# j-min/HiREST

Hardware: AMD Instinct MI355X
Metric: encoded frames/sec (EVA-CLIP-g/14 224^2) (higher is better)
Workload: dtype bf16

## Files before the change

hirest_amd/_lib.py:

```python
from __future__ import annotations

import ctypes as C
import os

HERE = os.path.dirname(os.path.abspath(__file__))
LIB_PATH = os.path.join(HERE, "lib", "libhirest_hip.so")
if os.environ.get("HIREST_LIB_VARIANT"):
    LIB_PATH = os.path.join(HERE, "lib", f"libhirest_hip.{os.environ['HIREST_LIB_VARIANT']}.so")

(EPI_BIAS_BF16, EPI_BIAS_GELU_BF16, EPI_BIAS_QGELU_BF16, EPI_BIAS_RESID_F32, EPI_BIAS_F32, EPI_PATCH_POS_F32,
 EPI_BIAS_RESID_LNSTATS_F32, EPI_LNFOLD_BF16, EPI_LNFOLD_GELU_BF16, EPI_BIAS_GELU_SPLIT2, EPI_BIAS_RESID2_LNSTATS) = range(11)

TOWER_NO_LNFOLD = 1
TOWER_NO_PRUNE = 2
TOWER_F32_RESIDUAL = 4
GEMM_REVERSE = 1
GEMM_X3 = 2
GEMM_X3_T128 = 4
ABI_VERSION = 4

ERRORS = {-1: "HIREST_E_BADARG", -2: "HIREST_E_SHAPE (unsupported shape)", -3: "HIREST_E_WORKSPACE (workspace too small)"}


class GemmArgs(C.Structure):
    _fields_ = [("struct_size", C.c_uint64),
                ("A", C.c_void_p), ("lda", C.c_int64), ("W", C.c_void_p), ("ldw", C.c_int64),
                ("bias", C.c_void_p), ("out", C.c_void_p), ("ldo", C.c_int64),
                ("M", C.c_int32), ("N", C.c_int32), ("K", C.c_int32), ("epilogue", C.c_int32),
                ("pos", C.c_void_p), ("patches_per_frame", C.c_int32), ("aux0", C.c_void_p), ("aux1", C.c_void_p), ("flags", C.c_int32)]

    @classmethod
    def make(cls, *fields):
        return cls(C.sizeof(cls), *fields)


F32_ENTRY = {"gemm": 0, "ws": 1, "layouts": 2, "ln": 3, "ln_colmax": 4, "rows_colmax": 5}


class GemmF32Query(C.Structure):
    _fields_ = [("struct_size", C.c_uint32)] + \
               [(n, C.c_int32) for n in ("entry", "M", "N", "K", "has_resid", "has_periodic", "has_ids", "has_ln_out", "has_workspace",
                                         "a_kmajor", "w_kmajor", "select_kernel", "ring_mode", "rows_ln_mode", "cus")]

    @classmethod
    def make(cls, entry, M, N, K, **fields):
        q = cls(C.sizeof(cls), F32_ENTRY[entry], M, N, K, select_kernel=-1, ring_mode=-1, rows_ln_mode=-1)
        for k, v in fields.items():
            setattr(q, k, int(v))
        return q


class BlockWeights(C.Structure):
    _fields_ = [(n, C.c_void_p) for n in ("ln1_g", "ln1_b", "qkv_w", "qkv_b", "proj_w", "proj_b",
                                          "ln2_g", "ln2_b", "fc1_w", "fc1_b", "fc2_w", "fc2_b",
                                          "qkv_wf", "qkv_bf", "qkv_s", "fc1_wf", "fc1_bf", "fc1_s")]


class VisionTower(C.Structure):
    _fields_ = [(n, C.c_int32) for n in ("image_size", "patch", "width", "heads", "head_dim", "mlp_dim",
                                         "layers", "embed_dim", "kpad", "act")] + \
               [("ln_eps", C.c_float)] + \
               [("patch_w", C.c_void_p), ("patch_b", C.c_void_p), ("cls", C.c_void_p), ("pos", C.c_void_p),
                ("blocks", C.POINTER(BlockWeights)),
                ("norm_g", C.c_void_p), ("norm_b", C.c_void_p), ("head_w", C.c_void_p), ("head_b", C.c_void_p),
                ("image_mean", C.c_void_p), ("image_std", C.c_void_p),
                ("ln_pre_g", C.c_void_p), ("ln_pre_b", C.c_void_p), ("out_all_tokens", C.c_int32)]


class TextTower(C.Structure):
    _fields_ = [(n, C.c_int32) for n in ("context", "vocab", "width", "heads", "layers", "embed_dim", "act")] + \
               [("ln_eps", C.c_float)] + \
               [("tok_emb", C.c_void_p), ("pos", C.c_void_p), ("blocks", C.POINTER(BlockWeights)),
                ("lnf_g", C.c_void_p), ("lnf_b", C.c_void_p), ("proj_w", C.c_void_p)]


class BlockWeightsF32(C.Structure):
    _fields_ = [(n, C.c_void_p) for n in ("ln1_g", "ln1_b", "qkv_w", "qkv_b", "proj_w", "proj_b",
                                          "ln2_g", "ln2_b", "fc1_w", "fc1_b", "fc2_w", "fc2_b")]


class VisionTowerF32(C.Structure):
    _fields_ = [(n, t) if n != "blocks" else (n, C.POINTER(BlockWeightsF32)) for n, t in VisionTower._fields_]


class TextTowerF32(C.Structure):
    _fields_ = [(n, t) if n != "blocks" else (n, C.POINTER(BlockWeightsF32)) for n, t in TextTower._fields_]


class BlockWeightsX3(C.Structure):
    _fields_ = [(n, C.c_void_p) for n in ("qkv_w2", "proj_w2", "fc1_w2", "fc2_w2")]


class VisionTowerX3(C.Structure):
    _fields_ = [("base", C.POINTER(VisionTowerF32)), ("blocks", C.POINTER(BlockWeightsX3))]


class CaptionLayer(C.Structure):
    _fields_ = [(n, C.c_void_p) for n in ("qkv_w", "qkv_b", "so_w", "so_b", "so_ln_g", "so_ln_b", "cq_w", "cq_b",
                                          "co_w", "co_b", "co_ln_g", "co_ln_b", "ff1_w", "ff1_b", "ff2_w", "ff2_b", "ff_ln_g", "ff_ln_b")]


class CaptionDecoder(C.Structure):
    _fields_ = [(n, C.c_int32) for n in ("layers", "heads", "hidden", "inter", "vocab_padded", "max_pos")] + \
               [(n, C.c_void_p) for n in ("word_emb", "pos_emb", "emb_ln_g", "emb_ln_b")] + \
               [("layer", C.POINTER(CaptionLayer))] + \
               [(n, C.c_void_p) for n in ("tr_w", "tr_b", "tr_ln_g", "tr_ln_b", "lm_w", "lm_b", "lm_w2")]


class WhisperLayer(C.Structure):
    _fields_ = [(n, C.c_void_p) for n in ("attn_ln_g", "attn_ln_b", "qkv_w", "qkv_b", "so_w", "so_b", "cross_ln_g", "cross_ln_b", "cq_w", "cq_b",
                                          "co_w", "co_b", "mlp_ln_g", "mlp_ln_b", "fc1_w", "fc1_b", "fc2_w", "fc2_b")]


class WhisperDecoder(C.Structure):
    _fields_ = [(n, C.c_int32) for n in ("layers", "heads", "hidden", "inter", "vocab_padded", "max_pos")] + \
               [(n, C.c_void_p) for n in ("tok_emb", "pos_emb")] + [("layer", C.POINTER(WhisperLayer))] + \
               [(n, C.c_void_p) for n in ("ln_g", "ln_b", "lm_b")]


class WhisperTailParams(C.Structure):
    _fields_ = [(n, C.c_int32) for n in ("n_vocab", "eot", "no_speech", "no_timestamps", "timestamp_begin", "max_initial_timestamp_index",
                                         "sample_begin", "blank", "suppress_blank", "timestamp_rules", "monotonic")] + \
               [("temperature", C.c_float), ("seed", C.c_uint32), ("serial", C.c_uint32), ("suppress_mask", C.c_void_p)]


WHISPER_ROW_STATE_WORDS = 8


class JointLayerX3(C.Structure):
    _fields_ = [(n, C.c_void_p) for n in ("qkv_w2", "qkv_b", "ao_w2", "ao_b", "ln1_g", "ln1_b", "fc1_w2", "fc1_b", "fc2_w2", "fc2_b", "ln2_g", "ln2_b")]


class JointEncoderX3(C.Structure):
    _fields_ = [("struct_size", C.c_uint64)] + [(n, C.c_int32) for n in ("layers", "heads", "width", "mlp_dim", "in_dim", "max_pos")] + \
               [("ln_eps", C.c_float), ("attn_shift", C.c_float)] + \
               [(n, C.c_void_p) for n in ("emb_w2", "emb_b", "pos", "emb_ln_g", "emb_ln_b")] + [("layer", C.POINTER(JointLayerX3))]


class ColsumItem(C.Structure):
    _fields_ = [("x", C.c_void_p), ("row_weight", C.c_void_p), ("row_select", C.c_void_p), ("out", C.c_void_p), ("ldx", C.c_int64),
                ("R", C.c_int32), ("C", C.c_int32), ("select_value", C.c_int32), ("reserved", C.c_int32)]


COLSUM_GROUP_MAX = 40


class SplitItem(C.Structure):
    _fields_ = [("x", C.c_void_p), ("out", C.c_void_p), ("ldx", C.c_int64), ("ldo", C.c_int64), ("rows", C.c_int32), ("cols", C.c_int32),
                ("transposed", C.c_int32), ("reserved", C.c_int32)]


class OptimItem(C.Structure):
    _fields_ = [("p", C.c_void_p), ("g", C.c_void_p), ("m", C.c_void_p), ("v", C.c_void_p), ("n", C.c_int64)]


OPTIM_GROUP_MAX = 64
OPTIM_CHUNK = 8192


class TrainBlock(C.Structure):
    _fields_ = [("struct_size", C.c_uint64)] + [(n, C.c_int32) for n in ("B", "T", "heads", "width", "mlp", "precision")] + \
               [("ln_eps", C.c_float), ("drop", C.c_float)] + [(n, C.c_uint32) for n in ("seed_attn", "seed_ao", "seed_out", "reserved")] + \
               [(n, C.c_void_p) for n in ("wqkv", "bqkv", "wo", "bo", "ln1_g", "ln1_b", "w1", "b1", "w2", "b2", "ln2_g", "ln2_b", "x",
                                          "qkv", "P", "cx", "a_pre", "aa", "hpre", "hh", "x_pre", "out", "x2", "out2",
                                          "wqkv2", "wo2", "w12", "w22", "wqkvT2", "woT2", "w1T2", "w2T2", "ws")] + [("ws_bytes", C.c_size_t)]


class TrainFusionBwd(C.Structure):
    _fields_ = [("struct_size", C.c_uint64)] + \
               [(n, C.c_int32) for n in ("B", "T", "E", "W", "vis_dim", "text_dim", "asr_dim", "boundary", "max_pos", "reserved")] + \
               [("drop", C.c_float), ("seed_emb", C.c_uint32)] + \
               [(n, C.c_void_p) for n in ("w_emb", "emb_ln_g", "t2_w", "asr1_w", "asr0_g", "norm_g",
                                          "x0", "f", "v", "tn", "tin", "a0", "asr2", "v0", "vis2", "t", "text", "mm32", "bm32", "n_valid", "dx",
                                          "g_emb_ln_g", "g_emb_ln_b", "g_pos", "g_w_emb", "g_b_emb", "g_mask", "g_bound", "g_t2_w", "g_t2_b", "g_t0_w", "g_t0_b",
                                          "g_asr1_w", "g_asr1_b", "g_asr0_g", "g_asr0_b", "g_norm_g", "g_norm_b", "g_vis_w", "g_vis_b", "g_text_w", "g_text_b")] + \
               [("items", C.POINTER(ColsumItem)), ("n_items", C.POINTER(C.c_int32)), ("max_items", C.c_int32), ("reserved2", C.c_int32),
                ("ws", C.c_void_p), ("ws_bytes", C.c_size_t), ("side_stream", C.c_void_p), ("side_ws", C.c_void_p), ("side_ws_bytes", C.c_size_t),
                ("scratch", C.c_void_p), ("scratch_bytes", C.c_size_t)]


class TrainBlockGrads(C.Structure):
    _fields_ = [("struct_size", C.c_uint64)] + \
               [(n, C.c_void_p) for n in ("dout", "dx", "g_wqkv", "g_wo", "g_w1", "g_w2", "g_bqkv", "g_bo", "g_b1", "g_b2", "g_ln1_g", "g_ln1_b",
                                          "g_ln2_g", "g_ln2_b")] + \
               [("items", C.POINTER(ColsumItem)), ("n_items", C.POINTER(C.c_int32)), ("max_items", C.c_int32), ("reserved", C.c_int32),
                ("side_stream", C.c_void_p), ("side_ws", C.c_void_p), ("side_ws_bytes", C.c_size_t), ("scratch", C.c_void_p),
                ("scratch_bytes", C.c_size_t)]


class JpegImage(C.Structure):
    _fields_ = [(n, C.c_int32) for n in ("width", "height", "ncomp", "hs", "vs", "restart_interval", "mcux", "mcuy", "supported",
                                         "reason")] + \
               [("scan_begin", C.c_int64), ("scan_end", C.c_int64), ("table_set", C.c_int32), ("reserved", C.c_int32),
                ("data_offset", C.c_int64), ("out_offset", C.c_int64), ("ws_offset", C.c_int64),
                ("plane_offset", C.c_int64)]


class JpegTables(C.Structure):
    _fields_ = [("qt", (C.c_uint16 * 64) * 3), ("huff_bits", (C.c_uint8 * 16) * 6), ("huff_vals", (C.c_uint8 * 256) * 6)]


JPEG_REASONS = {0: "ok", 1: "not a JPEG / malformed markers", 2: "progressive", 3: "arithmetic coding", 4: "lossless / hierarchical",
                5: "not 8-bit", 6: "colour space (CMYK / YCCK / RGB / component count)", 7: "sampling factors", 8: "multi-scan",
                9: "truncated (no EOI after the scan)", 10: "bad or missing tables", 11: "image size"}
JPEG_STATUS = {1: "bad Huffman code", 2: "more than 64 coefficients in a block", 4: "out of data", 8: "RSTn out of sequence",
               16: "unsupported"}


BATCH_GATHER_MAX = 8


class BatchGather(C.Structure):
    _fields_ = [("src", C.c_void_p), ("dst", C.c_void_p), ("row_of_example", C.c_void_p), ("words", C.c_int32), ("reserved", C.c_int32)]


class BatchArgs(C.Structure):
    _fields_ = [("struct_size", C.c_uint64), ("index", C.c_void_p)] + \
               [(n, C.c_int32) for n in ("B", "T", "D", "Da", "n_examples", "n_model_frames", "n_gather", "reserved")] + \
               [(n, C.c_void_p) for n in ("frames", "frame_off", "asr_rows", "sub_off", "sub_span", "ex_video", "ex_len", "ex_range",
                                          "bound_off", "bound_val", "vis", "asr", "vis_mask", "moment_mask", "prev_boundary_mask")] + \
               [("gather", BatchGather * BATCH_GATHER_MAX)]


class ProfRecord(C.Structure):
    _fields_ = [("kind", C.c_int32), ("tag", C.c_int32), ("d0", C.c_int64), ("d1", C.c_int64), ("d2", C.c_int64),
                ("ms", C.c_float)]


_SIGNATURES = {
    "hirest_profile_enable": (C.c_int, [C.c_int32]),
    "hirest_attention_debug_mode": (C.c_int, [C.c_int32]),
    "hirest_profile_collect": (C.c_int, [C.POINTER(ProfRecord), C.c_int32]),
    "hirest_abi_version": (C.c_int, []),
    "hirest_build_info": (C.c_char_p, []),
    "hirest_gemm_bf16": (C.c_int, [C.POINTER(GemmArgs), C.c_void_p]),
    "hirest_gemm_select_kernel": (C.c_int, [C.c_int32]),
    "hirest_gemm_debug_mode": (C.c_int, [C.c_int32]),
    "hirest_gemm_dispatch_name": (C.c_int, [C.POINTER(GemmArgs), C.c_char_p, C.c_int32]),
    "hirest_attention_select_kernel": (C.c_int, [C.c_int32]),
    "hirest_attention_set_skew": (C.c_int, [C.c_int32]),
    "hirest_attention_set_mapping": (C.c_int, [C.c_int32]),
    "hirest_attention_set_pace": (C.c_int, [C.c_int32]),
    "hirest_attention_x3_select_waves": (C.c_int, [C.c_int32]),
    "hirest_attention_x3_debug_trace": (C.c_int, [C.c_void_p]),
    "hirest_attention_set_stagger": (C.c_int, [C.c_int32]),
    "hirest_attention_debug_trace_read": (C.c_int, [C.c_void_p, C.c_int32]),
    "hirest_layernorm": (C.c_int, [C.c_void_p, C.c_int64, C.c_void_p, C.c_void_p, C.c_void_p, C.c_float,
                                   C.c_void_p, C.c_int64, C.c_int32, C.c_int32, C.c_int32, C.c_void_p]),
    "hirest_attention_bf16": (C.c_int, [C.c_void_p, C.c_void_p, C.c_int32, C.c_int32, C.c_int32, C.c_int32,
                                        C.c_float, C.c_int32, C.c_void_p]),
    "hirest_attention_bf16_rows": (C.c_int, [C.c_void_p, C.c_void_p, C.c_int32, C.c_int32, C.c_int32, C.c_int32,
                                             C.c_float, C.c_int32, C.c_int32, C.c_void_p]),
    "hirest_fold_layernorm": (C.c_int, [C.c_void_p, C.c_void_p, C.c_void_p, C.c_void_p, C.c_void_p, C.c_void_p, C.c_void_p, C.c_int32,
                                        C.c_int32, C.c_void_p]),
    "hirest_patchify": (C.c_int, [C.c_void_p, C.c_int32, C.c_int32, C.c_int32, C.c_int32, C.c_void_p, C.c_void_p,
                                  C.c_void_p, C.c_int32, C.c_void_p]),
    "hirest_rowstats_bf16": (C.c_int, [C.c_void_p, C.c_int64, C.c_void_p, C.c_void_p, C.c_float, C.c_int32, C.c_int32, C.c_void_p, C.c_void_p]),
    "hirest_rowstats_split_bf16": (C.c_int, [C.c_void_p, C.c_int64, C.c_void_p, C.c_void_p, C.c_void_p, C.c_float, C.c_int32, C.c_int32, C.c_void_p,
                                             C.c_void_p]),
    "hirest_combine_hi_lo_f32": (C.c_int, [C.c_void_p, C.c_void_p, C.c_int64, C.c_void_p, C.c_int64, C.c_int32, C.c_int32, C.c_void_p]),
    "hirest_ln_stats_finalize": (C.c_int, [C.c_void_p, C.c_int32, C.c_void_p, C.c_float, C.c_int32, C.c_int32, C.c_void_p, C.c_void_p]),
    "hirest_write_cls_rows": (C.c_int, [C.c_void_p, C.c_int64, C.c_void_p, C.c_void_p, C.c_int32, C.c_int32,
                                        C.c_int32, C.c_void_p]),
    "hirest_embed_tokens": (C.c_int, [C.c_void_p, C.c_void_p, C.c_void_p, C.c_void_p, C.c_void_p, C.c_int32,
                                      C.c_int32, C.c_int32, C.c_int32, C.c_void_p]),
    "hirest_f32_to_bf16": (C.c_int, [C.c_void_p, C.c_void_p, C.c_int64, C.c_void_p]),
    "hirest_pool_l2norm": (C.c_int, [C.c_void_p, C.c_void_p, C.c_int32, C.c_int32, C.c_int32, C.c_int32, C.c_void_p]),
    "hirest_pool_l2norm_varlen": (C.c_int, [C.c_void_p, C.c_void_p, C.c_void_p, C.c_int32, C.c_int32, C.c_void_p]),
    "hirest_similarity_f32": (C.c_int, [C.c_void_p, C.c_void_p, C.c_void_p, C.c_int32, C.c_int32, C.c_int32, C.c_void_p]),
    "hirest_topk_workspace_bytes": (C.c_int64, [C.c_int32, C.c_int32, C.c_int32]),
    "hirest_topk_f32_ws": (C.c_int, [C.c_void_p, C.c_void_p, C.c_int32, C.c_int32, C.c_int32, C.c_void_p, C.c_void_p, C.c_void_p,
                                     C.c_int64, C.c_void_p]),
    "hirest_topk_f32": (C.c_int, [C.c_void_p, C.c_void_p, C.c_int32, C.c_int32, C.c_int32, C.c_void_p, C.c_void_p,
                                  C.c_void_p]),
    "hirest_clip_score": (C.c_int, [C.c_void_p, C.c_int32, C.c_int32, C.c_void_p, C.c_int32, C.c_void_p, C.c_int32, C.c_int32,
                                    C.c_int32, C.c_void_p, C.c_void_p]),
    "hirest_bertscore_greedy": (C.c_int, [C.c_void_p, C.c_int64, C.c_int32, C.c_void_p, C.c_int32, C.c_void_p, C.c_void_p, C.c_void_p,
                                          C.c_int32, C.c_void_p, C.c_void_p]),
    "hirest_gemm_f32": (C.c_int, [C.c_void_p, C.c_int64, C.c_void_p, C.c_int64, C.c_void_p, C.c_void_p, C.c_int64, C.c_void_p,
                                  C.c_int32, C.c_void_p, C.c_int64, C.c_int32, C.c_int32, C.c_int32, C.c_int32, C.c_void_p]),
    "hirest_attention_f32": (C.c_int, [C.c_void_p, C.c_void_p, C.c_int32, C.c_int32, C.c_int32, C.c_int32, C.c_float,
                                       C.c_float, C.c_void_p]),
    "hirest_attention_f32_qkv": (C.c_int, [C.c_void_p, C.c_int64, C.c_void_p, C.c_void_p, C.c_int64, C.c_void_p, C.c_int32, C.c_int32,
                                           C.c_int32, C.c_int32, C.c_int32, C.c_float, C.c_float, C.c_float, C.c_void_p]),
    "hirest_gemm_f32_select_kernel": (C.c_int, [C.c_int32]),
    "hirest_gemm_f32_workspace_bytes": (C.c_size_t, [C.c_int32, C.c_int32, C.c_int32]),
    "hirest_gemm_f32_layouts_workspace_bytes": (C.c_size_t, [C.c_int32, C.c_int32, C.c_int32]),
    "hirest_gemm_f32_layouts": (C.c_int, [C.c_void_p, C.c_int64, C.c_int32, C.c_void_p, C.c_int64, C.c_int32, C.c_void_p, C.c_void_p, C.c_int64,
                                          C.c_void_p, C.c_int64, C.c_int32, C.c_int32, C.c_int32, C.c_int32, C.c_void_p, C.c_size_t, C.c_void_p]),
    "hirest_gemm_f32_ws": (C.c_int, [C.c_void_p, C.c_int64, C.c_void_p, C.c_int64, C.c_void_p, C.c_void_p, C.c_int64, C.c_void_p,
                                     C.c_int32, C.c_void_p, C.c_int64, C.c_int32, C.c_int32, C.c_int32, C.c_int32, C.c_void_p, C.c_size_t,
                                     C.c_void_p]),
    "hirest_attention_f32_decode": (C.c_int, [C.c_void_p, C.c_int64, C.c_void_p, C.c_void_p, C.c_int64, C.c_void_p, C.c_int32, C.c_void_p,
                                              C.c_void_p, C.c_int64, C.c_void_p, C.c_void_p, C.c_void_p, C.c_int32, C.c_int32, C.c_float,
                                              C.c_float, C.c_float, C.c_void_p]),
    "hirest_gemm_f32_ln": (C.c_int, [C.c_void_p, C.c_int64, C.c_void_p, C.c_void_p, C.c_void_p, C.c_void_p, C.c_void_p, C.c_float,
                                     C.c_void_p, C.c_int64, C.c_void_p, C.c_int64, C.c_void_p, C.c_void_p, C.c_int64, C.c_void_p,
                                     C.c_int64, C.c_int32, C.c_int32, C.c_int32, C.c_int32, C.c_void_p]),
    "hirest_caption_step_workspace_bytes": (C.c_size_t, [C.POINTER(CaptionDecoder), C.c_int32]),
    "hirest_beam_backtrack": (C.c_int, [C.c_void_p, C.c_void_p, C.c_void_p, C.c_void_p, C.c_int32, C.c_int32, C.c_int32, C.c_void_p, C.c_void_p]),
    "hirest_beam_advance": (C.c_int, [C.c_void_p, C.c_void_p, C.c_int32, C.c_int32, C.c_int32, C.c_int32, C.c_int32, C.c_int32,
                                      C.c_void_p, C.c_void_p, C.c_void_p, C.c_void_p, C.c_void_p, C.c_void_p, C.c_void_p, C.c_void_p,
                                      C.c_void_p]),
    "hirest_caption_decode_step": (C.c_int, [C.POINTER(CaptionDecoder), C.c_int32, C.c_int32, C.c_void_p, C.c_void_p,
                                             C.POINTER(C.c_void_p), C.POINTER(C.c_void_p), C.POINTER(C.c_void_p), C.c_int32,
                                             C.c_void_p, C.c_void_p, C.c_void_p, C.c_size_t, C.c_void_p]),
    "hirest_caption_decode_logits": (C.c_int, [C.POINTER(CaptionDecoder), C.c_int32, C.c_int32, C.c_void_p, C.c_void_p,
                                               C.POINTER(C.c_void_p), C.POINTER(C.c_void_p), C.POINTER(C.c_void_p), C.c_int32,
                                               C.c_void_p, C.c_void_p, C.c_size_t, C.c_void_p]),
    "hirest_caption_select": (C.c_int, [C.c_int32]),
    "hirest_gemm_f32_ln_colmax": (C.c_int, [C.c_void_p, C.c_int64, C.c_void_p, C.c_void_p, C.c_float, C.c_void_p, C.c_int64, C.c_void_p,
                                            C.c_void_p, C.c_int64, C.c_void_p, C.c_int32, C.c_int32, C.c_int32, C.c_void_p]),
    "hirest_gemm_f32_dispatch_name": (C.c_int, [C.POINTER(GemmF32Query), C.c_char_p, C.c_int32]),
    "hirest_gemm_f32_rows_ln_mode": (C.c_int, [C.c_int32]),
    "hirest_gemm_f32_ring_mode": (C.c_int, [C.c_int32]),
    "hirest_gemm_f32_rows_preferred": (C.c_int, [C.c_int32]),
    "hirest_gemm_f32_rows_colmax": (C.c_int, [C.c_void_p, C.c_int64, C.c_void_p, C.c_int64, C.c_void_p, C.c_void_p, C.c_int64, C.c_void_p,
                                              C.c_int32, C.c_int32, C.c_int32, C.c_void_p]),
    "hirest_caption_beam_step": (C.c_int, [C.POINTER(CaptionDecoder), C.c_int32, C.c_int32, C.c_int32, C.c_void_p, C.c_void_p,
                                           C.POINTER(C.c_void_p), C.POINTER(C.c_void_p), C.POINTER(C.c_void_p), C.c_int32, C.c_void_p,
                                           C.c_void_p, C.c_int32, C.c_int32, C.c_void_p, C.c_void_p, C.c_void_p, C.c_void_p, C.c_void_p,
                                           C.c_void_p, C.c_void_p, C.c_size_t, C.c_void_p, C.c_size_t, C.c_void_p]),
    "hirest_caption_beam_tail_workspace_bytes": (C.c_size_t, [C.c_int32, C.c_int32, C.c_int32]),
    "hirest_caption_beam_tail": (C.c_int, [C.c_void_p, C.c_int64, C.c_void_p, C.c_int32, C.c_int32, C.c_int32, C.c_int32, C.c_int32,
                                           C.c_int32, C.c_void_p, C.c_void_p, C.c_void_p, C.c_void_p, C.c_void_p, C.c_void_p,
                                           C.c_void_p, C.c_void_p, C.c_void_p, C.c_void_p, C.c_size_t, C.c_void_p]),
    "hirest_attention_f32_varlen": (C.c_int, [C.c_void_p, C.c_void_p, C.c_void_p, C.c_int32, C.c_int32, C.c_int32, C.c_int32, C.c_float,
                                              C.c_float, C.c_void_p]),
    "hirest_log_softmax_f32": (C.c_int, [C.c_void_p, C.c_int64, C.c_void_p, C.c_void_p, C.c_int64, C.c_int32, C.c_int32, C.c_void_p]),
    "hirest_joint_time_grid_f32": (C.c_int, [C.c_void_p, C.c_int32, C.c_int32, C.c_void_p, C.c_void_p]),
    "hirest_joint_time_features": (C.c_int, [C.c_void_p, C.c_void_p, C.c_void_p, C.c_void_p, C.c_int32, C.c_int32, C.c_int32,
                                             C.c_void_p]),
    "hirest_joint_base": (C.c_int, [C.c_void_p, C.c_void_p, C.c_void_p, C.c_void_p, C.c_void_p, C.c_int32, C.c_int32, C.c_int32,
                                    C.c_void_p]),
    "hirest_joint_mask_add": (C.c_int, [C.c_void_p, C.c_void_p, C.c_void_p, C.c_void_p, C.c_void_p, C.c_void_p, C.c_int64,
                                        C.c_int32, C.c_void_p]),
    "hirest_transpose_pad_f32": (C.c_int, [C.c_void_p, C.c_int64, C.c_int32, C.c_int32, C.c_void_p, C.c_int32, C.c_void_p]),
    "hirest_weighted_colsum_grouped_f32": (C.c_int, [C.c_void_p, C.c_int32, C.c_void_p]),
    "hirest_train_fusion_backward_scratch_bytes": (C.c_size_t, [C.POINTER(TrainFusionBwd)]),
    "hirest_train_fusion_backward": (C.c_int, [C.POINTER(TrainFusionBwd), C.c_void_p]),
    "hirest_train_block_forward_scratch_bytes": (C.c_size_t, [C.POINTER(TrainBlock)]),
    "hirest_train_block_forward": (C.c_int, [C.POINTER(TrainBlock), C.c_void_p, C.c_size_t, C.c_void_p]),
    "hirest_train_block_backward_scratch_bytes": (C.c_size_t, [C.POINTER(TrainBlock)]),
    "hirest_train_block_backward": (C.c_int, [C.POINTER(TrainBlock), C.POINTER(TrainBlockGrads), C.c_void_p]),
    "hirest_optim_partials_count": (C.c_int64, [C.c_void_p, C.c_int32]),
    "hirest_grad_sqnorm_grouped_f32": (C.c_int, [C.c_void_p, C.c_int32, C.c_void_p, C.c_void_p]),
    "hirest_clip_coef_f32": (C.c_int, [C.c_void_p, C.c_int64, C.c_float, C.c_void_p, C.c_void_p]),
    "hirest_adamw_grouped_f32": (C.c_int, [C.c_void_p, C.c_int32, C.c_void_p, C.c_float, C.c_float, C.c_float, C.c_float, C.c_float,
                                           C.c_float, C.c_float, C.c_void_p]),
    "hirest_grad_sqnorm_scaled_grouped_f32": (C.c_int, [C.c_void_p, C.c_int32, C.c_void_p, C.c_void_p, C.c_void_p]),
    "hirest_clip_coef_dev_f32": (C.c_int, [C.c_void_p, C.c_int64, C.c_void_p, C.c_void_p, C.c_void_p]),
    "hirest_optim_step_advance_f32": (C.c_int, [C.c_void_p, C.c_int32, C.c_void_p, C.c_void_p]),
    "hirest_adamw_capturable_grouped_f32": (C.c_int, [C.c_void_p, C.c_void_p, C.c_int32, C.c_void_p, C.c_void_p, C.c_double, C.c_void_p,
                                                      C.c_void_p, C.c_double, C.c_double, C.c_float, C.c_double, C.c_void_p]),
    "hirest_weighted_colsum_f32": (C.c_int, [C.c_void_p, C.c_int64, C.c_void_p, C.c_void_p, C.c_int32, C.c_int32, C.c_int32, C.c_void_p, C.c_void_p]),
    "hirest_scale_by_device_scalar_f32": (C.c_int, [C.c_void_p, C.c_void_p, C.c_int64, C.c_void_p]),
    "hirest_act_f32": (C.c_int, [C.c_void_p, C.c_void_p, C.c_int64, C.c_int32, C.c_void_p]),
    "hirest_act_bwd_f32": (C.c_int, [C.c_void_p, C.c_void_p, C.c_void_p, C.c_int64, C.c_int32, C.c_void_p]),
    "hirest_dropout_add_f32": (C.c_int, [C.c_void_p, C.c_void_p, C.c_void_p, C.c_int64, C.c_float, C.c_uint32, C.c_void_p]),
    "hirest_layernorm_bwd_f32": (C.c_int, [C.c_void_p, C.c_void_p, C.c_void_p, C.c_float, C.c_void_p, C.c_void_p, C.c_int32, C.c_int32, C.c_void_p]),
    "hirest_attention_train_select": (C.c_int, [C.c_int32]),
    "hirest_gemm_f32_strided": (C.c_int, [C.c_void_p, C.c_int64, C.c_int64, C.c_void_p, C.c_int64, C.c_int64, C.c_void_p, C.c_int64,
                                          C.c_int32, C.c_int32, C.c_int32, C.c_float, C.c_void_p]),
    "hirest_attention_train_fwd_f32": (C.c_int, [C.c_void_p, C.c_void_p, C.c_void_p, C.c_int32, C.c_int32, C.c_int32, C.c_int32, C.c_float,
                                                 C.c_float, C.c_float, C.c_uint32, C.c_void_p]),
    "hirest_attention_train_bwd_f32": (C.c_int, [C.c_void_p, C.c_void_p, C.c_void_p, C.c_void_p, C.c_void_p, C.c_int32, C.c_int32, C.c_int32,
                                                 C.c_int32, C.c_float, C.c_float, C.c_uint32, C.c_void_p]),
    "hirest_attention_train_fwd_qkv_f32": (C.c_int, [C.c_void_p, C.c_int64, C.c_void_p, C.c_void_p, C.c_int64, C.c_void_p, C.c_void_p, C.c_void_p,
                                                     C.c_int64, C.c_int32, C.c_int32, C.c_int32, C.c_int32, C.c_int32, C.c_float, C.c_float,
                                                     C.c_float, C.c_uint32, C.c_void_p]),
    "hirest_attention_train_bwd_qkv_f32": (C.c_int, [C.c_void_p, C.c_int64, C.c_void_p, C.c_void_p, C.c_int64, C.c_void_p, C.c_void_p, C.c_int64,
                                                     C.c_void_p, C.c_void_p, C.c_int64, C.c_void_p, C.c_void_p, C.c_int64, C.c_int32, C.c_int32,
                                                     C.c_int32, C.c_int32, C.c_int32, C.c_float, C.c_float, C.c_uint32, C.c_void_p]),
    "hirest_embedding_fwd_f32": (C.c_int, [C.c_void_p, C.c_void_p, C.c_void_p, C.c_void_p, C.c_int64, C.c_int32, C.c_int32, C.c_void_p]),
    "hirest_embedding_pos_fwd_f32": (C.c_int, [C.c_void_p, C.c_void_p, C.c_void_p, C.c_void_p, C.c_void_p, C.c_int64, C.c_int32, C.c_void_p]),
    "hirest_embedding_bwd_f32": (C.c_int, [C.c_void_p, C.c_void_p, C.c_void_p, C.c_int64, C.c_int32, C.c_void_p]),
    "hirest_ce_rows_f32": (C.c_int, [C.c_void_p, C.c_int64, C.c_void_p, C.c_int32, C.c_int32, C.c_float, C.c_int32, C.c_void_p, C.c_void_p, C.c_void_p]),
    "hirest_bce_masked_f32": (C.c_int, [C.c_void_p, C.c_void_p, C.c_void_p, C.c_int32, C.c_int32, C.c_float, C.c_void_p, C.c_void_p, C.c_void_p]),
    "hirest_joint_base_bwd_f32": (C.c_int, [C.c_void_p, C.c_void_p, C.c_void_p, C.c_void_p, C.c_void_p, C.c_int32, C.c_int32, C.c_int32, C.c_void_p]),
    "hirest_l2norm_bwd_f32": (C.c_int, [C.c_void_p, C.c_void_p, C.c_void_p, C.c_int32, C.c_int32, C.c_void_p]),
    "hirest_ce_masked_f32": (C.c_int, [C.c_void_p, C.c_void_p, C.c_void_p, C.c_int32, C.c_int32, C.c_float, C.c_void_p, C.c_void_p, C.c_void_p]),
    "hirest_heads_bwd_f32": (C.c_int, [C.c_void_p, C.c_int64, C.c_int32, C.c_int32, C.c_void_p, C.c_void_p, C.c_void_p, C.c_void_p, C.c_void_p]),
    "hirest_linear_heads": (C.c_int, [C.c_void_p, C.c_int64, C.c_int32, C.c_int32, C.c_void_p, C.c_void_p, C.c_void_p, C.c_void_p,
                                      C.c_void_p, C.c_void_p]),
    "hirest_masked_argmax": (C.c_int, [C.c_void_p, C.c_void_p, C.c_float, C.c_int32, C.c_int32, C.c_void_p, C.c_void_p]),
    "hirest_moment_valid_f32": (C.c_int, [C.c_void_p, C.c_void_p, C.c_void_p, C.c_void_p, C.c_void_p, C.c_int32, C.c_int32, C.c_float,
                                          C.c_void_p, C.c_void_p, C.c_void_p]),
    "hirest_lm_head_ce_workspace_bytes": (C.c_size_t, [C.c_int32, C.c_int32]),
    "hirest_lm_head_ce_f32": (C.c_int, [C.c_void_p, C.c_int64, C.c_void_p, C.c_int64, C.c_void_p, C.c_void_p, C.c_int32, C.c_int32,
                                        C.c_int32, C.c_int32, C.c_void_p, C.c_void_p, C.c_void_p, C.c_size_t, C.c_void_p]),
    "hirest_segmentation_step": (C.c_int, [C.c_void_p, C.c_void_p, C.c_void_p, C.c_int32, C.c_int32, C.c_double, C.c_void_p,
                                           C.c_void_p, C.c_int32, C.c_void_p, C.c_void_p]),
    "hirest_preprocess_plan_bytes": (C.c_int64, [C.c_int32, C.c_int32, C.c_int32]),
    "hirest_preprocess_plan": (C.c_int, [C.c_int32, C.c_int32, C.c_int32, C.c_void_p, C.c_int64]),
    "hirest_preprocess_workspace_bytes": (C.c_int64, [C.c_int32, C.c_int32, C.c_int32, C.c_int32]),
    "hirest_preprocess_u8": (C.c_int, [C.c_void_p, C.c_int32, C.c_int32, C.c_int32, C.c_int32, C.c_void_p, C.c_void_p,
                                       C.c_int32, C.c_void_p, C.c_void_p, C.c_void_p, C.c_int64, C.c_void_p]),
    "hirest_jpeg_parse": (C.c_int, [C.c_void_p, C.c_int64, C.POINTER(JpegImage), C.POINTER(JpegTables)]),
    "hirest_jpeg_workspace_bytes": (C.c_int64, [C.POINTER(JpegImage), C.c_int32]),
    "hirest_jpeg_decode": (C.c_int, [C.c_void_p, C.c_void_p, C.c_int32, C.c_void_p, C.c_void_p, C.c_void_p, C.c_void_p, C.c_void_p,
                                     C.c_int64, C.c_void_p]),
    "hirest_jpeg_decode_host": (C.c_int, [C.POINTER(JpegImage), C.POINTER(JpegTables), C.c_void_p, C.c_void_p, C.POINTER(C.c_int32)]),
    "hirest_jpeg_chunked_workspace_bytes": (C.c_int64, [C.c_int32]),
    "hirest_jpeg_decode_chunked": (C.c_int, [C.c_void_p, C.c_void_p, C.c_int32, C.c_void_p, C.c_void_p, C.c_void_p, C.c_void_p, C.c_void_p,
                                             C.c_int64, C.c_int64, C.c_void_p, C.c_int64, C.c_void_p]),
    "hirest_jpeg_decode_host_chunked": (C.c_int, [C.POINTER(JpegImage), C.POINTER(JpegTables), C.c_void_p, C.c_int64, C.c_void_p,
                                                  C.POINTER(C.c_int32), C.POINTER(C.c_int32)]),
    "hirest_interval_iou_f64": (C.c_int, [C.c_void_p, C.c_void_p, C.c_int64, C.c_void_p, C.c_void_p]),
    "hirest_step_bound_pr": (C.c_int, [C.c_void_p, C.c_void_p, C.c_void_p, C.c_void_p, C.c_int32, C.c_double, C.c_void_p,
                                       C.c_void_p, C.c_void_p, C.c_void_p]),
    "hirest_frame_to_timestamp": (C.c_int, [C.c_void_p, C.c_void_p, C.c_void_p, C.c_int32, C.c_int64, C.c_int64, C.c_void_p, C.c_void_p]),
    "hirest_timestamp_to_frame": (C.c_int, [C.c_void_p, C.c_void_p, C.c_void_p, C.c_int32, C.c_int64, C.c_int64, C.c_void_p, C.c_void_p]),
    "hirest_preprocess_moment_bounds": (C.c_int, [C.c_void_p, C.c_void_p, C.c_void_p, C.c_int32, C.c_void_p, C.c_void_p,
                                                  C.c_int32, C.c_void_p]),
    "hirest_cascade_moment_bounds": (C.c_int, [C.c_void_p, C.c_void_p, C.c_void_p, C.c_int32, C.c_int32, C.c_int32, C.c_void_p, C.c_void_p,
                                               C.c_void_p, C.c_void_p, C.c_void_p]),
    "hirest_cascade_boundaries": (C.c_int, [C.c_void_p, C.c_void_p, C.c_void_p, C.c_void_p, C.c_void_p, C.c_int32, C.c_int32, C.c_int32,
                                            C.c_void_p, C.c_void_p, C.c_void_p, C.c_void_p, C.c_void_p, C.c_void_p, C.c_void_p]),
    "hirest_cascade_trim_gather": (C.c_int, [C.c_void_p, C.c_void_p, C.c_void_p, C.c_void_p, C.c_int32, C.c_int32, C.c_int32, C.c_int32,
                                             C.c_int32, C.c_int32, C.c_void_p, C.c_void_p, C.c_void_p]),
    "hirest_batch_assemble": (C.c_int, [C.POINTER(BatchArgs), C.c_void_p]),
    "hirest_log_mel_workspace_bytes": (C.c_size_t, [C.c_int64, C.c_int64]),
    "hirest_log_mel": (C.c_int, [C.c_void_p, C.c_int64, C.c_int64, C.c_void_p, C.c_int32, C.c_void_p, C.c_void_p, C.c_void_p, C.c_size_t,
                                 C.c_void_p]),
    "hirest_mel_to_rows": (C.c_int, [C.c_void_p, C.c_void_p, C.c_int32, C.c_int32, C.c_int32, C.c_void_p]),
    "hirest_attention_f32_decode_inplace": (C.c_int, [C.c_void_p, C.c_int64, C.c_void_p, C.c_void_p, C.c_int64, C.c_int64, C.c_int32, C.c_int32,
                                                      C.c_void_p, C.c_void_p, C.c_int64, C.c_void_p, C.c_int32, C.c_int32, C.c_float, C.c_float,
                                                      C.c_float, C.c_void_p]),
    "hirest_attention_f32_cross_decode_workspace_bytes": (C.c_size_t, [C.c_int32, C.c_int32, C.c_int32]),
    "hirest_attention_f32_cross_decode": (C.c_int, [C.c_void_p, C.c_int64, C.c_void_p, C.c_int64, C.c_int64, C.c_int32, C.c_int32, C.c_void_p,
                                                    C.c_void_p, C.c_int64, C.c_int32, C.c_int32, C.c_float, C.c_void_p, C.c_size_t, C.c_void_p]),
    "hirest_whisper_step_tail": (C.c_int, [C.c_void_p, C.c_int64, C.c_int32, C.c_int32, C.c_int32, C.c_int32, C.POINTER(WhisperTailParams),
                                           C.c_void_p, C.c_void_p, C.c_void_p, C.c_void_p, C.c_void_p, C.c_void_p]),
    "hirest_whisper_gumbel_bits": (C.c_int, [C.c_uint32, C.c_uint32, C.c_int32, C.c_int32, C.c_void_p, C.c_void_p]),
    "hirest_whisper_step_workspace_bytes": (C.c_size_t, [C.POINTER(WhisperDecoder), C.c_int32, C.c_int32]),
    "hirest_whisper_decode_step": (C.c_int, [C.POINTER(WhisperDecoder), C.c_int32, C.c_int32, C.c_void_p, C.POINTER(C.c_void_p),
                                             C.POINTER(C.c_void_p), C.c_int32, C.POINTER(C.c_void_p), C.c_int32, C.c_int32, C.c_void_p,
                                             C.c_void_p, C.c_void_p, C.c_size_t, C.c_void_p]),
    "hirest_vision_workspace_bytes": (C.c_size_t, [C.POINTER(VisionTower), C.c_int32]),
    "hirest_vision_forward": (C.c_int, [C.POINTER(VisionTower), C.c_void_p, C.c_int32, C.c_int32, C.c_void_p,
                                        C.c_void_p, C.c_size_t, C.c_int32, C.c_void_p]),
    "hirest_vision_guard_offset": (C.c_size_t, [C.POINTER(VisionTower), C.c_int32]),
    "hirest_vision_workspace_bytes_f32": (C.c_size_t, [C.POINTER(VisionTowerF32), C.c_int32]),
    "hirest_vision_embed_f32": (C.c_int, [C.POINTER(VisionTowerF32), C.c_void_p, C.c_int32, C.c_int32, C.c_void_p, C.c_void_p, C.c_void_p]),
    "hirest_joint_encoder_x3_workspace_bytes": (C.c_size_t, [C.POINTER(JointEncoderX3), C.c_int32, C.c_int32]),
    "hirest_joint_encoder_x3_forward": (C.c_int, [C.POINTER(JointEncoderX3), C.c_void_p, C.c_int32, C.c_int32, C.c_void_p, C.c_void_p, C.c_size_t,
                                                  C.c_void_p]),
    "hirest_layernorm_f32_split2": (C.c_int, [C.c_void_p, C.c_int64, C.c_void_p, C.c_int32, C.c_void_p, C.c_void_p, C.c_float, C.c_void_p, C.c_int64,
                                              C.c_void_p, C.c_int64, C.c_int32, C.c_int32, C.c_void_p]),
    "hirest_split2_bf16": (C.c_int, [C.c_void_p, C.c_int64, C.c_void_p, C.c_int64, C.c_int64, C.c_int32, C.c_int32, C.c_void_p]),
    "hirest_split2_grouped_bf16": (C.c_int, [C.c_void_p, C.c_int32, C.c_void_p]),
    "hirest_split2_transposed_bf16": (C.c_int, [C.c_void_p, C.c_int64, C.c_void_p, C.c_int64, C.c_int32, C.c_int32, C.c_void_p]),
    "hirest_layernorm_split2": (C.c_int, [C.c_void_p, C.c_int64, C.c_void_p, C.c_void_p, C.c_float, C.c_void_p, C.c_int64, C.c_int32,
                                          C.c_int32, C.c_void_p]),
    "hirest_attention_x3_qkv": (C.c_int, [C.c_void_p, C.c_int64, C.c_void_p, C.c_void_p, C.c_int64, C.c_void_p, C.c_int32, C.c_int32, C.c_int32,
                                          C.c_int32, C.c_int32, C.c_float, C.c_void_p]),
    "hirest_attention_x3_qkv_split2": (C.c_int, [C.c_void_p, C.c_int64, C.c_void_p, C.c_void_p, C.c_int64, C.c_void_p, C.c_int32, C.c_int32,
                                                 C.c_int32, C.c_int32, C.c_int32, C.c_float, C.c_void_p]),
    "hirest_vision_x3_select_attention": (C.c_int, [C.c_int32]),
    "hirest_vision_workspace_bytes_x3": (C.c_size_t, [C.POINTER(VisionTowerX3), C.c_int32]),
    "hirest_vision_forward_x3": (C.c_int, [C.POINTER(VisionTowerX3), C.c_void_p, C.c_int32, C.c_int32, C.c_void_p, C.c_void_p, C.c_size_t,
                                           C.c_void_p]),
    "hirest_vision_forward_f32": (C.c_int, [C.POINTER(VisionTowerF32), C.c_void_p, C.c_int32, C.c_int32, C.c_void_p,
                                            C.c_void_p, C.c_size_t, C.c_void_p]),
    "hirest_text_workspace_bytes_f32": (C.c_size_t, [C.POINTER(TextTowerF32), C.c_int32]),
    "hirest_text_forward_f32": (C.c_int, [C.POINTER(TextTowerF32), C.c_void_p, C.c_int32, C.c_void_p, C.c_void_p,
                                          C.c_size_t, C.c_void_p]),
    "hirest_text_workspace_bytes": (C.c_size_t, [C.POINTER(TextTower), C.c_int32]),
    "hirest_text_forward": (C.c_int, [C.POINTER(TextTower), C.c_void_p, C.c_int32, C.c_void_p, C.c_void_p,
                                      C.c_size_t, C.c_void_p]),
}

EXPORTS = tuple(_SIGNATURES)
_lib = None


def load():
    global _lib
    if _lib is not None:
        return _lib
    if not os.path.isfile(LIB_PATH):
        raise RuntimeError(f"{LIB_PATH} is missing: build it with `python -m hirest_amd.build` "
                           "(hipcc --offload-arch=gfx950). There is no CPU fallback.")
    lib = C.CDLL(LIB_PATH)
    lib.hirest_abi_version.restype, lib.hirest_abi_version.argtypes = C.c_int, []
    if lib.hirest_abi_version() != ABI_VERSION:
        raise RuntimeError(f"libhirest_hip.so ABI version {lib.hirest_abi_version()} != binding {ABI_VERSION}: rebuild with "
                           "`python -m hirest_amd.build --force`")
    for name, (res, args) in _SIGNATURES.items():
        fn = getattr(lib, name)
        fn.restype, fn.argtypes = res, args
    if os.environ.get("HIREST_ATTENTION_KERNEL"):
        check(lib.hirest_attention_select_kernel(int(os.environ["HIREST_ATTENTION_KERNEL"])), "HIREST_ATTENTION_KERNEL")
    _lib = lib
    return lib


def check(code: int, what: str):
    if code == 0:
        return
    if code < 0:
        raise RuntimeError(f"{what}: {ERRORS.get(code, code)}")
    raise RuntimeError(f"{what}: HIP error {code}")
```

hirest_amd/csrc/attention.hip:

```cpp
#include "common.h"
#include <atomic>
#include "profile.h"

namespace {

template <int DH, int DP, int NT>
struct AttnCfg {
    static constexpr int NPAD = 16 * NT;
    static constexpr int KS = (NT + 1) / 2;
    static constexpr int KP = 32 * KS;
    static constexpr int KRS = DP * 2 + 16;
    static constexpr int VRS = KP * 2 + 16;
    static constexpr int LDS_BYTES = NPAD * KRS + DP * VRS;
};

template <int DH, int DP, int NT>
__global__ __launch_bounds__(512) void attention_kernel(const bf16_t* __restrict__ qkv, bf16_t* __restrict__ out,
                                                       int N, int H, float scale_log2e, int causal, int nq) {
    using C = AttnCfg<DH, DP, NT>;
    extern __shared__ __attribute__((aligned(16))) char smem[];
    char* Ks = smem;
    char* Vt = smem + C::NPAD * C::KRS;
    const int tid = threadIdx.x, lane = tid & 63, wave = tid >> 6;
    const int b = blockIdx.x / H, h = blockIdx.x - b * H;
    const int D = H * DH;
    const int64_t ld = 3 * (int64_t)D;
    const bf16_t* base = qkv + (int64_t)b * N * ld + h * DH;

    constexpr int KCH = DP / 8;
    for (int idx = tid; idx < C::NPAD * KCH; idx += 512) {
        const int key = idx / KCH, ch = idx - key * KCH;
        bf16x8 v = {0, 0, 0, 0, 0, 0, 0, 0};
        if (key < N && ch * 8 < DH) v = *reinterpret_cast<const bf16x8*>(base + (int64_t)key * ld + D + ch * 8);
        *reinterpret_cast<bf16x8*>(Ks + key * C::KRS + ch * 16) = v;
    }
    constexpr int VCH = DH / 8;
    for (int idx = tid; idx < C::KP * VCH; idx += 512) {
        const int ch = idx / C::KP, key = idx - ch * C::KP;
        bf16x8 v = {0, 0, 0, 0, 0, 0, 0, 0};
        if (key < N) v = *reinterpret_cast<const bf16x8*>(base + (int64_t)key * ld + 2 * D + ch * 8);
#pragma unroll
        for (int e = 0; e < 8; ++e) *reinterpret_cast<bf16_t*>(Vt + (ch * 8 + e) * C::VRS + key * 2) = v[e];
    }
    __syncthreads();

    const int g = lane >> 4, c16 = lane & 15;
    const int nqt = (nq + 15) >> 4;
    for (int qt = wave; qt < nqt; qt += 8) {
        const int q = qt * 16 + c16;
        const bool qvalid = q < N;
        bf16x8 qf[DP / 32];
#pragma unroll
        for (int kk = 0; kk < DP / 32; ++kk) {
            const int d = (kk * 4 + g) * 8;
            bf16x8 v = {0, 0, 0, 0, 0, 0, 0, 0};
            if (qvalid && d < DH) v = *reinterpret_cast<const bf16x8*>(base + (int64_t)q * ld + d);
            qf[kk] = v;
        }
        f32x4 st[NT];
#pragma unroll
        for (int t = 0; t < NT; ++t) {
            f32x4 acc = {0.f, 0.f, 0.f, 0.f};
#pragma unroll
            for (int kk = 0; kk < DP / 32; ++kk) {
                const bf16x8 kf = *reinterpret_cast<const bf16x8*>(Ks + (t * 16 + c16) * C::KRS + (kk * 4 + g) * 16);
                acc = __builtin_amdgcn_mfma_f32_16x16x32_bf16(kf, qf[kk], acc, 0, 0, 0);
            }
            st[t] = acc;
            if ((t & 1) == 1) __builtin_amdgcn_sched_barrier(0);
        }
        const int klimit = causal ? (q < N - 1 ? q : N - 1) : N - 1;
        float mx = -3.0e38f;
#pragma unroll
        for (int t = 0; t < NT; ++t)
#pragma unroll
            for (int i = 0; i < 4; ++i) {
                const int key = t * 16 + 4 * g + i;
                const float s = key <= klimit ? st[t][i] : -3.0e38f;
                st[t][i] = s;
                mx = fmaxf(mx, s);
            }
        mx = fmaxf(mx, __shfl_xor(mx, 16, 64));
        mx = fmaxf(mx, __shfl_xor(mx, 32, 64));
        float sum = 0.f;
#pragma unroll
        for (int t = 0; t < NT; ++t)
#pragma unroll
            for (int i = 0; i < 4; ++i) {
                const float pz = exp2f((st[t][i] - mx) * scale_log2e);
                st[t][i] = pz;
                sum += pz;
            }
        sum += __shfl_xor(sum, 16, 64);
        sum += __shfl_xor(sum, 32, 64);
        const float inv = 1.0f / sum;
        bf16x8 pf[C::KS];
#pragma unroll
        for (int s = 0; s < C::KS; ++s) {
#pragma unroll
            for (int i = 0; i < 4; ++i) {
                pf[s][i] = (bf16_t)st[2 * s][i];
                if (2 * s + 1 < NT) pf[s][4 + i] = (bf16_t)st[2 * s + 1][i];
                else pf[s][4 + i] = (bf16_t)0.f;
            }
        }
#pragma unroll 1
        for (int dt = 0; dt < DP / 16; ++dt) {
            f32x4 acc = {0.f, 0.f, 0.f, 0.f};
            const char* vrow = Vt + (dt * 16 + c16) * C::VRS + 8 * g;
#pragma unroll
            for (int s = 0; s < C::KS; ++s) {
                const bf16x4 lo = *reinterpret_cast<const bf16x4*>(vrow + s * 64);
                const bf16x4 hi = *reinterpret_cast<const bf16x4*>(vrow + s * 64 + 32);
                const bf16x8 vf = {lo[0], lo[1], lo[2], lo[3], hi[0], hi[1], hi[2], hi[3]};
                acc = __builtin_amdgcn_mfma_f32_16x16x32_bf16(vf, pf[s], acc, 0, 0, 0);
            }
            const int d = dt * 16 + 4 * g;
            if (q < nq && d < DH) {
                bf16x4 o;
#pragma unroll
                for (int i = 0; i < 4; ++i) o[i] = (bf16_t)(acc[i] * inv);
                *reinterpret_cast<bf16x4*>(out + ((int64_t)b * N + q) * D + h * DH + d) = o;
            }
        }
    }
}

template <int DH, int DP, int NT>
int launch(const bf16_t* qkv, bf16_t* out, int B, int N, int H, float scale, int causal, int nq, hipStream_t s) {
    using C = AttnCfg<DH, DP, NT>;
    static HirestDevCfg cfg;
    auto kern = attention_kernel<DH, DP, NT>;
    if (int e = hirest_configure(kern, C::LDS_BYTES, cfg)) return e;
    hipLaunchKernelGGL(kern, dim3(B * H), dim3(512), C::LDS_BYTES, s, qkv, out, N, H, scale * 1.44269504088896340736f, causal, nq);
    return hirest_launch_status();
}


template <int DH, int DP, int NT>
struct AttnCfg2 {
    static constexpr int NPAD = 16 * NT;
    static constexpr int KS = (NT + 1) / 2;
    static constexpr int KP = 32 * KS;
    static constexpr int RS = DP * 2;
    static constexpr int CPR = DP / 8;
    static constexpr int NK_INSTR = NPAD * CPR / 64;
    static constexpr int NV_INSTR = KP * CPR / 64;
    static constexpr int LDS_BYTES = (NPAD + KP) * RS;
};

__device__ __forceinline__ void wait_vm_le(int n) {
    switch (n) {
        case 0: asm volatile("s_waitcnt vmcnt(0)" ::: "memory"); break;
        case 1: asm volatile("s_waitcnt vmcnt(1)" ::: "memory"); break;
        case 2: asm volatile("s_waitcnt vmcnt(2)" ::: "memory"); break;
        case 3: asm volatile("s_waitcnt vmcnt(3)" ::: "memory"); break;
        case 4: asm volatile("s_waitcnt vmcnt(4)" ::: "memory"); break;
        case 5: asm volatile("s_waitcnt vmcnt(5)" ::: "memory"); break;
        case 6: asm volatile("s_waitcnt vmcnt(6)" ::: "memory"); break;
        case 7: asm volatile("s_waitcnt vmcnt(7)" ::: "memory"); break;
        default: asm volatile("s_waitcnt vmcnt(8)" ::: "memory"); break;
    }
}

template <int DH, int DP, int NT>
__global__ __launch_bounds__(512) void attention_kernel_v2(const bf16_t* __restrict__ qkv, bf16_t* __restrict__ out,
                                                          int N, int H, float scale_log2e, int causal, int nq) {
    using C = AttnCfg2<DH, DP, NT>;
    extern __shared__ __attribute__((aligned(16))) char smem[];
    char* Ks = smem;
    char* Vs = smem + C::NPAD * C::RS;
    const int tid = threadIdx.x, lane = tid & 63;
    const int wave = __builtin_amdgcn_readfirstlane(tid >> 6);
    const int b = blockIdx.x / H, h = blockIdx.x - b * H;
    const int D = H * DH;
    const int64_t ld = 3 * (int64_t)D;
    const bf16_t* base = qkv + (int64_t)b * N * ld + h * DH;

    int nv_mine = 0;
    for (int i = wave; i < C::NK_INSTR; i += 8) {
        const int ci = i * 64 + lane;
        int row = ci / C::CPR, c = ci - row * C::CPR;
        c = (c & ~3) | ((c & 3) ^ ((-(row >> 2)) & 3));
        row = row < N ? row : N - 1;
        c = c * 8 < DH ? c : DH / 8 - 1;
        glds16(base + (int64_t)row * ld + D + c * 8, Ks + i * 1024);
    }
    for (int i = wave; i < C::NV_INSTR; i += 8) {
        const int ci = i * 64 + lane;
        int row = ci / C::CPR, c = ci - row * C::CPR;
        row = row < N ? row : N - 1;
        c = c * 8 < DH ? c : DH / 8 - 1;
        glds16(base + (int64_t)row * ld + 2 * D + c * 8, Vs + i * 1024);
        ++nv_mine;
    }
    wait_vm_le(nv_mine);
    __builtin_amdgcn_s_barrier();

    const int g = lane >> 4, c16 = lane & 15;
    const int gk = g ^ ((-(c16 >> 2)) & 3);
    const int nqt = (nq + 15) >> 4;
    bool v_ready = false;
    for (int qt = wave; qt < nqt; qt += 8) {
        const int q = qt * 16 + c16;
        const bool qvalid = q < N;
        bf16x8 qf[DP / 32];
#pragma unroll
        for (int kk = 0; kk < DP / 32; ++kk) {
            const int d = (kk * 4 + g) * 8;
            bf16x8 v = {0, 0, 0, 0, 0, 0, 0, 0};
            if (qvalid && d < DH) v = *reinterpret_cast<const bf16x8*>(base + (int64_t)q * ld + d);
            qf[kk] = v;
        }
        f32x4 st[NT];
#pragma unroll
        for (int t = 0; t < NT; ++t) {
            f32x4 acc = {0.f, 0.f, 0.f, 0.f};
#pragma unroll
            for (int kk = 0; kk < DP / 32; ++kk) {
                const bf16x8 kf = *reinterpret_cast<const bf16x8*>(Ks + (t * 16 + c16) * C::RS + (kk * 4 + gk) * 16);
                acc = __builtin_amdgcn_mfma_f32_16x16x32_bf16(kf, qf[kk], acc, 0, 0, 0);
            }
            st[t] = acc;
            if ((t & 1) == 1) __builtin_amdgcn_sched_barrier(0);
        }
        const int klimit = causal ? (q < N - 1 ? q : N - 1) : N - 1;
        float mx = -3.0e38f;
#pragma unroll
        for (int t = 0; t < NT; ++t)
#pragma unroll
            for (int i = 0; i < 4; ++i) {
                const int key = t * 16 + 4 * g + i;
                const float sv = key <= klimit ? st[t][i] : -3.0e38f;
                st[t][i] = sv;
                mx = fmaxf(mx, sv);
            }
        mx = fmaxf(mx, __shfl_xor(mx, 16, 64));
        mx = fmaxf(mx, __shfl_xor(mx, 32, 64));
        float sum = 0.f;
#pragma unroll
        for (int t = 0; t < NT; ++t)
#pragma unroll
            for (int i = 0; i < 4; ++i) {
                const float pz = exp2f((st[t][i] - mx) * scale_log2e);
                st[t][i] = pz;
                sum += pz;
            }
        sum += __shfl_xor(sum, 16, 64);
        sum += __shfl_xor(sum, 32, 64);
        const float inv = 1.0f / sum;
        bf16x8 pf[C::KS];
#pragma unroll
        for (int s = 0; s < C::KS; ++s) {
#pragma unroll
            for (int i = 0; i < 4; ++i) {
                pf[s][i] = (bf16_t)st[2 * s][i];
                if (2 * s + 1 < NT) pf[s][4 + i] = (bf16_t)st[2 * s + 1][i];
                else pf[s][4 + i] = (bf16_t)0.f;
            }
        }
        if (!v_ready) {
            asm volatile("s_waitcnt vmcnt(0)" ::: "memory");
            __builtin_amdgcn_s_barrier();
            v_ready = true;
        }
        const char* vlane = Vs + (4 * g + (c16 >> 2)) * C::RS + (c16 & 3) * 8;
#pragma unroll 1
        for (int dt = 0; dt < DP / 16; ++dt) {
            f32x4 acc = {0.f, 0.f, 0.f, 0.f};
            const char* vrow = vlane + dt * 32;
#pragma unroll
            for (int s = 0; s < C::KS; ++s) {
                const bf16x4 lo = __builtin_amdgcn_ds_read_tr16_b64_v4bf16(
                    (__attribute__((address_space(3))) bf16x4*)(vrow + s * 32 * C::RS));
                const bf16x4 hi = __builtin_amdgcn_ds_read_tr16_b64_v4bf16(
                    (__attribute__((address_space(3))) bf16x4*)(vrow + (s * 32 + 16) * C::RS));
                const bf16x8 vf = {lo[0], lo[1], lo[2], lo[3], hi[0], hi[1], hi[2], hi[3]};
                acc = __builtin_amdgcn_mfma_f32_16x16x32_bf16(vf, pf[s], acc, 0, 0, 0);
            }
            const int d = dt * 16 + 4 * g;
            if (q < nq && d < DH) {
                bf16x4 o;
#pragma unroll
                for (int i = 0; i < 4; ++i) o[i] = (bf16_t)(acc[i] * inv);
                *reinterpret_cast<bf16x4*>(out + ((int64_t)b * N + q) * D + h * DH + d) = o;
            }
        }
    }
    if (!v_ready) {
        asm volatile("s_waitcnt vmcnt(0)" ::: "memory");
        __builtin_amdgcn_s_barrier();
    }
}


__device__ __forceinline__ void sleep_n(int n) {
    for (int i = 0; i < n; ++i) __builtin_amdgcn_s_sleep(1);
}
template <int NW, int CPR> struct ROWS_PER_PIECE_OK { static constexpr bool value = (NW * 64 % CPR == 0) && ((NW * 64 / CPR) % 8 == 0); };
__device__ __attribute__((aligned(16))) const unsigned short g_attn_ones[8] = {0x3F80, 0x3F80, 0x3F80, 0x3F80, 0x3F80, 0x3F80, 0x3F80, 0x3F80};
__device__ __attribute__((aligned(16))) const unsigned short g_attn_zeros[8] = {0, 0, 0, 0, 0, 0, 0, 0};
constexpr int ATTN_TRACE_STEPS = 64, ATTN_TRACE_WAVES = 12, ATTN_TRACE_SLOTS = 12;
__device__ long long g_attn_trace[ATTN_TRACE_STEPS * ATTN_TRACE_WAVES * ATTN_TRACE_SLOTS];
__device__ __forceinline__ float max3_raw(float a, float b, float c) {
    float r;
    asm("v_max3_f32 %0, %1, %2, %3" : "=v"(r) : "v"(a), "v"(b), "v"(c));
    return r;
}
typedef float f32x2_t __attribute__((ext_vector_type(2)));
template <int DH, int DP, int NT, bool FAST, bool DBG, int NW = 9, bool LEAN = false, bool PROD = false>
__global__ __launch_bounds__((NW + (PROD ? 1 : 0)) * 64) void attention_kernel_v3(const bf16_t* __restrict__ qkv, bf16_t* __restrict__ out,
                                                          int N, int H, float scale_log2e, int causal, int dbg_bits, int nq, int skew,
                                                          int B, int map, int pace, int stagger) {
    const int dbg = DBG ? dbg_bits : 0;
    using C = AttnCfg2<DH, DP, NT>;
    extern __shared__ __attribute__((aligned(16))) char smem[];
    char* Vs = smem + 2 * C::NPAD * C::RS;
    const int tid = threadIdx.x, lane = tid & 63;
    const int wave = __builtin_amdgcn_readfirstlane(tid >> 6);
    const int D = H * DH;
    const int64_t ld = 3 * (int64_t)D;
    int b0, bstep, h0, hstep, nsteps;
    if (map == 0) { b0 = blockIdx.x; bstep = 0; h0 = 0; hstep = 1; nsteps = H; }
    else {
        const int xcd = blockIdx.x & 7, slot = blockIdx.x >> 3, FL = (gridDim.x >> 3) / H;
        h0 = slot % H; hstep = 0; b0 = xcd * FL + slot / H; bstep = 8 * FL;
        nsteps = b0 < B ? (B - b0 + bstep - 1) / bstep : 0;
    }
    if (nsteps == 0) return;
    if (stagger > 0 && blockIdx.x < 256) sleep_n(((blockIdx.x >> 3) & 15) * stagger);
    auto sbase = [&](int st) { return qkv + (int64_t)(b0 + st * bstep) * N * ld + (h0 + st * hstep) * DH; };
    const int g = lane >> 4, c16 = lane & 15;
    const int gk = g ^ ((-(c16 >> 2)) & 3);
    const int nqt = (nq + 15) >> 4;

    const int ci0 = wave * 64 + lane;
    const int row0 = ci0 / C::CPR, col0 = ci0 - row0 * C::CPR;
    constexpr bool VSWAP = C::RS == 192;
    const int vlog = VSWAP ? ((((col0 >> 1) ^ ((row0 >> 2) & 1)) << 1) | (col0 & 1)) : col0;
    const int vc = vlog * 8 < DH ? vlog : DH / 8 - 1;
    static_assert(ROWS_PER_PIECE_OK<NW, C::CPR>::value, "a lane's rows must keep (row >> 2) & 1 from piece to piece");
    static_assert((NW * 64) % C::CPR == 0, "piece stride must be whole rows");
    constexpr int ROWS_PER_PIECE = NW * 64 / C::CPR;
    auto dma_k = [&](int h, char* dst) -> int {
        int n = 0;
        const bf16_t* src = sbase(h) + D;
        for (int i = wave, row = row0; i < C::NK_INSTR; i += NW, row += ROWS_PER_PIECE) {
            int kc = (col0 & ~3) | ((col0 & 3) ^ ((-(row >> 2)) & 3));
            const bool kpad = kc * 8 >= DH;
            kc = kpad ? DH / 8 - 1 : kc;
            const int r = row < N ? row : N - 1;
            const void* from = src + (int64_t)r * ld + kc * 8;
            if (LEAN && DP > DH) from = kpad ? (const void*)g_attn_zeros : from;
            glds16(from, dst + i * 1024);
            ++n;
        }
        return n;
    };
    constexpr bool SUM_IN_MFMA = LEAN && DP > DH;
    const bool vpad = SUM_IN_MFMA && vlog * 8 >= DH;
    auto dma_v = [&](int h) {
        const bf16_t* src = sbase(h) + 2 * D + vc * 8;
        for (int i = wave, row = row0; i < C::NV_INSTR; i += NW, row += ROWS_PER_PIECE) {
            const int r = row < N ? row : N - 1;
            const void* from = src + (int64_t)r * ld;
            if (SUM_IN_MFMA) from = vpad ? (const void*)g_attn_ones : from;
            glds16(from, Vs + i * 1024);
        }
    };
    auto load_q = [&](int h, int qtile, bf16x8 (&dst)[DP / 32]) {
        const int q = qtile * 16 + c16;
        const bf16_t* base = sbase(h);
        if (LEAN && DP > DH) {
            const bf16_t* row = base + (int64_t)(q < N ? q : N - 1) * ld;
#pragma unroll
            for (int kk = 0; kk < DP / 32; ++kk) {
                const int d = (kk * 4 + g) * 8;
                dst[kk] = *reinterpret_cast<const bf16x8*>(row + (d < DH ? d : DH - 8));
            }
            return;
        }
#pragma unroll
        for (int kk = 0; kk < DP / 32; ++kk) {
            const int d = (kk * 4 + g) * 8;
            bf16x8 v = {0, 0, 0, 0, 0, 0, 0, 0};
            if (qtile < nqt && q < N && d < DH) v = *reinterpret_cast<const bf16x8*>(base + (int64_t)q * ld + d);
            dst[kk] = v;
        }
    };

    if (PROD && wave == NW) {
        constexpr int PER = C::CPR / 4;
        static_assert(C::NK_INSTR % PER == 0 && C::NV_INSTR % PER == 0, "whole 16-row groups");
        int prow[PER], pkoff[PER], pvoff[PER];
        bool pkpad[PER], pvpad[PER];
#pragma unroll
        for (int j = 0; j < PER; ++j) {
            const int ci = j * 64 + lane, r = ci / C::CPR, c = ci - r * C::CPR;
            prow[j] = r;
            int kc = (c & ~3) | ((c & 3) ^ ((-(r >> 2)) & 3));
            pkpad[j] = kc * 8 >= DH;
            pkoff[j] = (pkpad[j] ? DH / 8 - 1 : kc) * 8;
            const int vl = VSWAP ? ((((c >> 1) ^ ((r >> 2) & 1)) << 1) | (c & 1)) : c;
            pvpad[j] = SUM_IN_MFMA && vl * 8 >= DH;
            pvoff[j] = (vl * 8 < DH ? vl : DH / 8 - 1) * 8;
        }
        auto issue_k = [&](int st, char* dst, int pace_units) {
            const bf16_t* src = sbase(st) + D;
            for (int it0 = 0; it0 < C::NK_INSTR / PER; ++it0) {
                const int it = map ? (it0 + h0) % (C::NK_INSTR / PER) : it0;
#pragma unroll
                for (int j = 0; j < PER; ++j) {
                    const int row = prow[j] + 16 * it, r = row < N ? row : N - 1;
                    const void* from = src + (int64_t)r * ld + pkoff[j];
                    if (LEAN && DP > DH) from = pkpad[j] ? (const void*)g_attn_zeros : from;
                    glds16(from, dst + (it * PER + j) * 1024);
                    if (pace_units > 0) sleep_n(pace_units);
                }
            }
        };
        auto issue_v = [&](int st) {
            const bf16_t* src = sbase(st) + 2 * D;
            for (int it0 = 0; it0 < C::NV_INSTR / PER; ++it0) {
                const int it = map ? (it0 + h0) % (C::NV_INSTR / PER) : it0;
#pragma unroll
                for (int j = 0; j < PER; ++j) {
                    const int row = prow[j] + 16 * it, r = row < N ? row : N - 1;
                    const void* from = src + (int64_t)r * ld + pvoff[j];
                    if (SUM_IN_MFMA) from = pvpad[j] ? (const void*)g_attn_ones : from;
                    glds16(from, Vs + (it * PER + j) * 1024);
                }
            }
        };
        issue_k(0, smem, 0);
        for (int h = 0; h < nsteps; ++h) {
            asm volatile("s_waitcnt vmcnt(0)" ::: "memory");
            __builtin_amdgcn_s_barrier();
            issue_v(h);
            asm volatile("s_waitcnt vmcnt(0)" ::: "memory");
            __builtin_amdgcn_s_barrier();
            if (h + 1 < nsteps) issue_k(h + 1, smem + ((h + 1) & 1) * (C::NPAD * C::RS), pace);
        }
        asm volatile("s_waitcnt vmcnt(0)" ::: "memory");
        return;
    }

    bf16x8 qa[DP / 32], qb[DP / 32];
    load_q(0, wave, qa);
    load_q(0, wave + NW, qb);
    if (!(dbg & 8) && !PROD) dma_k(0, smem);
    for (int h = 0; h < nsteps; ++h) {
        const char* Ks = smem + (h & 1) * (C::NPAD * C::RS);
        auto stamp = [&](int slot) {
            if (DBG && (dbg & 256) && blockIdx.x == 0 && h < ATTN_TRACE_STEPS) {
                const long long t = __builtin_readcyclecounter();
                if (lane == 0) g_attn_trace[(h * ATTN_TRACE_WAVES + wave) * ATTN_TRACE_SLOTS + slot] = t;
            }
        };
        stamp(10);
        asm volatile("s_waitcnt vmcnt(0)" ::: "memory");
#pragma unroll
        for (int kk = 0; kk < DP / 32; ++kk) { asm volatile("" : "+v"(qa[kk])); asm volatile("" : "+v"(qb[kk])); }
        if (!(dbg & 128)) __builtin_amdgcn_s_barrier();
        stamp(0);
        if (!(dbg & 8) && !PROD) dma_v(h);
        const int nk_next = (h + 1 < nsteps && !(dbg & 8) && !PROD) ? dma_k(h + 1, smem + ((h + 1) & 1) * (C::NPAD * C::RS)) : 0;
        bool v_ready = false;
        auto tile = [&](int qt, bf16x8 (&qf)[DP / 32], int ord) {
            stamp(1 + 4 * ord);
            const int q = qt * 16 + c16;
            const bool qvalid = q < N;
            f32x4 st[NT];
#pragma unroll
            for (int t = 0; t < NT; t += 2) {
                f32x4 a0 = {0.f, 0.f, 0.f, 0.f}, a1 = {0.f, 0.f, 0.f, 0.f};
                if (!(dbg & 1))
#pragma unroll
                for (int kk = 0; kk < DP / 32; ++kk) {
                    const bf16x8 k0 = *reinterpret_cast<const bf16x8*>(Ks + (t * 16 + c16) * C::RS + (kk * 4 + gk) * 16);
                    a0 = __builtin_amdgcn_mfma_f32_16x16x32_bf16(k0, qf[kk], a0, 0, 0, 0);
                    if (t + 1 < NT) {
                        const bf16x8 k1 = *reinterpret_cast<const bf16x8*>(Ks + ((t + 1) * 16 + c16) * C::RS + (kk * 4 + gk) * 16);
                        a1 = __builtin_amdgcn_mfma_f32_16x16x32_bf16(k1, qf[kk], a1, 0, 0, 0);
                    }
                }
                st[t] = a0;
                if (t + 1 < NT) st[t + 1] = a1;
                if ((t & 2) || !FAST) __builtin_amdgcn_sched_barrier(0);
            }
            if (h + 1 < nsteps && !(dbg & 32)) load_q(h + 1, qt, qf);
            stamp(2 + 4 * ord);
            const int klimit = causal ? (q < N - 1 ? q : N - 1) : N - 1;
            float mx = -3.0e38f;
            float sum = 0.f;
            bf16x8 pf[C::KS];
            if (LEAN) {
                float mxb = -3.0e38f;
#pragma unroll
                for (int t = 0; t < NT; ++t) {
                    if (!FAST || t == NT - 1) {
#pragma unroll
                        for (int i = 0; i < 4; ++i) st[t][i] = (t * 16 + 4 * g + i) <= klimit ? st[t][i] : -3.0e38f;
                    }
                    if (t & 1) { mxb = max3_raw(mxb, st[t][0], st[t][1]); mxb = max3_raw(mxb, st[t][2], st[t][3]); }
                    else { mx = max3_raw(mx, st[t][0], st[t][1]); mx = max3_raw(mx, st[t][2], st[t][3]); }
                }
                float pa = max3_raw(mx, mxb, mxb), pb = pa;
                lane_swap16(pa, pb); pa = max3_raw(pa, pb, pb); pb = pa; lane_swap32(pa, pb); mx = max3_raw(pa, pb, pb);
                const float nmc = -mx * scale_log2e;
                const f32x2_t sc2 = {scale_log2e, scale_log2e}, nm2 = {nmc, nmc};
                f32x2_t sum2 = {0.f, 0.f};
#pragma unroll
                for (int s2 = 0; s2 < C::KS; ++s2) {
#pragma unroll
                    for (int u = 0; u < 2; ++u) {
                        if (2 * s2 + u < NT) {
#pragma unroll
                            for (int ip = 0; ip < 2; ++ip) {
                                const f32x2_t sv = {st[2 * s2 + u][2 * ip], st[2 * s2 + u][2 * ip + 1]};
                                const f32x2_t e = __builtin_elementwise_fma(sv, sc2, nm2);
                                const f32x2_t p2 = (dbg & 2) ? e : f32x2_t{__builtin_amdgcn_exp2f(e[0]), __builtin_amdgcn_exp2f(e[1])};
                                if (!SUM_IN_MFMA) sum2 += p2;
                                pf[s2][4 * u + 2 * ip] = (bf16_t)p2[0];
                                pf[s2][4 * u + 2 * ip + 1] = (bf16_t)p2[1];
                            }
                        } else {
#pragma unroll
                            for (int i = 0; i < 4; ++i) pf[s2][4 + i] = (bf16_t)0.f;
                        }
                    }
                }
                if (!SUM_IN_MFMA) {
                    sum = sum2[0] + sum2[1];
                    float sa = sum, sb = sum; lane_swap16(sa, sb); sum = sa + sb; sa = sum; sb = sum; lane_swap32(sa, sb); sum = sa + sb;
                }
            } else {
#pragma unroll
            for (int t = 0; t < NT; ++t) {
                if (!FAST || t == NT - 1) {
#pragma unroll
                    for (int i = 0; i < 4; ++i) st[t][i] = (t * 16 + 4 * g + i) <= klimit ? st[t][i] : -3.0e38f;
                }
                mx = fmaxf(fmaxf(mx, fmaxf(st[t][0], st[t][1])), fmaxf(st[t][2], st[t][3]));
            }
            { float pa = mx, pb = mx; lane_swap16(pa, pb); mx = fmaxf(pa, pb); pa = mx; pb = mx; lane_swap32(pa, pb); mx = fmaxf(pa, pb); }
            const float nmc = -mx * scale_log2e;
#pragma unroll
            for (int s2 = 0; s2 < C::KS; ++s2) {
#pragma unroll
                for (int i = 0; i < 4; ++i) {
                    const float e0 = fmaf(st[2 * s2][i], scale_log2e, nmc);
                    const float p0 = (dbg & 2) ? e0 : __builtin_amdgcn_exp2f(e0);
                    sum += p0;
                    pf[s2][i] = (bf16_t)p0;
                    if (2 * s2 + 1 < NT) {
                        const float e1 = fmaf(st[2 * s2 + 1][i], scale_log2e, nmc);
                        const float p1 = (dbg & 2) ? e1 : __builtin_amdgcn_exp2f(e1);
                        sum += p1;
                        pf[s2][4 + i] = (bf16_t)p1;
                    } else {
                        pf[s2][4 + i] = (bf16_t)0.f;
                    }
                }
            }
            { float pa = sum, pb = sum; lane_swap16(pa, pb); sum = pa + pb; pa = sum; pb = sum; lane_swap32(pa, pb); sum = pa + pb; }
            }
            stamp(3 + 4 * ord);
            if (!v_ready) {
                if (!PROD) wait_vm_le(nk_next);
                if (!(dbg & 64)) __builtin_amdgcn_s_barrier();
                v_ready = true;
            }
            stamp(4 + 4 * ord);
            const char* vlane = Vs + (4 * g + (c16 >> 2)) * C::RS + (c16 & 3) * 8;
            const char* vl_e = vlane + ((VSWAP && (g & 1)) ? 32 : 0);
            const char* vl_o = vlane - ((VSWAP && (g & 1)) ? 32 : 0);
            f32x4 oacc[DP / 16];
#pragma unroll
            for (int dt = 0; dt < DP / 16; ++dt) oacc[dt] = f32x4{0.f, 0.f, 0.f, 0.f};
            if (!(dbg & 4))
#pragma unroll
            for (int s2 = 0; s2 < C::KS; ++s2) {
#pragma unroll
                for (int dt = 0; dt < DP / 16; ++dt) {
                    const char* vrow = ((dt & 1) ? vl_o : vl_e) + dt * 32 + s2 * 32 * C::RS;
                    const bf16x4 lo = __builtin_amdgcn_ds_read_tr16_b64_v4bf16((__attribute__((address_space(3))) bf16x4*)(vrow));
                    const bf16x4 hi = __builtin_amdgcn_ds_read_tr16_b64_v4bf16((__attribute__((address_space(3))) bf16x4*)(vrow + 16 * C::RS));
                    const bf16x8 vf = {lo[0], lo[1], lo[2], lo[3], hi[0], hi[1], hi[2], hi[3]};
                    oacc[dt] = __builtin_amdgcn_mfma_f32_16x16x32_bf16(vf, pf[s2], oacc[dt], 0, 0, 0);
                }
                if ((s2 & 1) || !FAST) __builtin_amdgcn_sched_barrier(0);
            }
            if (SUM_IN_MFMA) {
                float sa = oacc[DP / 16 - 1][0], sb = sa;
                lane_swap32(sa, sb);
                sum = sb;
            }
            const float inv = 1.0f / sum;
            static_assert((DP / 16) % 2 == 0 && DH % 8 == 0, "paired d tiles");
#pragma unroll
            for (int dp = 0; dp < DP / 32; ++dp) {
                union { bf16x4 v; unsigned u[2]; } e, o;
#pragma unroll
                for (int i = 0; i < 4; ++i) { e.v[i] = (bf16_t)(oacc[2 * dp][i] * inv); o.v[i] = (bf16_t)(oacc[2 * dp + 1][i] * inv); }
                const auto s0 = __builtin_amdgcn_permlane16_swap(e.u[0], o.u[0], false, false);
                const auto s1 = __builtin_amdgcn_permlane16_swap(e.u[1], o.u[1], false, false);
                union { bf16x8 v; unsigned u[4]; } w;
                w.u[0] = s0[0]; w.u[1] = s1[0]; w.u[2] = s0[1]; w.u[3] = s1[1];
                const int d = (2 * dp + (g & 1)) * 16 + (g >> 1) * 8;
                if (qvalid && q < nq && d < DH && !(dbg & 16)) *reinterpret_cast<bf16x8*>(out + ((int64_t)(b0 + h * bstep) * N + q) * D + (h0 + h * hstep) * DH + d) = w.v;
            }
        };
        if (skew > 0 && wave >= 4 && wave < 8) sleep_n(skew);
        if (wave < nqt) tile(wave, qa, 0);
        if (wave + NW < nqt) tile(wave + NW, qb, 1);
        stamp(9);
        if (!v_ready) {
            if (!PROD) wait_vm_le(nk_next);
            __builtin_amdgcn_s_barrier();
        }
    }
    asm volatile("s_waitcnt vmcnt(0)" ::: "memory");
}

std::atomic<int> g_attn_dbg{0};
std::atomic<int> g_attn_skew{12};
std::atomic<int> g_attn_stagger{16};
std::atomic<int> g_attn_pace{0};
std::atomic<int> g_attn_map{2};
std::atomic<int> g_attn_variant{7};

template <int DH, int DP, int NT, bool FAST, bool DBG, int NW = 9, bool LEAN = false, bool PROD = false>
int launch3_impl(const bf16_t* qkv, bf16_t* out, int B, int N, int H, float scale, int causal, int nq, hipStream_t s) {
    using C = AttnCfg2<DH, DP, NT>;
    constexpr int LDS = (2 * C::NPAD + C::KP) * C::RS;
    static_assert(LDS <= 163840, "K x2 + V must fit the CU's LDS");
    static HirestDevCfg cfg;
    auto kern = attention_kernel_v3<DH, DP, NT, FAST, DBG, NW, LEAN, PROD>;
    if (int e = hirest_configure(kern, LDS, cfg)) return e;
    const bool by_head = (g_attn_map == 1 || (g_attn_map == 2 && B < 256)) && H <= 32 && 32 % H == 0 && B >= 8 * (32 / H) * 4;
    const int grid = by_head ? 256 : B;
    hipLaunchKernelGGL(kern, dim3(grid), dim3((NW + (PROD ? 1 : 0)) * 64), LDS, s, qkv, out, N, H, scale * 1.44269504088896340736f, causal, g_attn_dbg, nq,
                       g_attn_skew, B, by_head ? 1 : 0, g_attn_pace, g_attn_stagger);
    return hirest_launch_status();
}

template <int DH, int DP, int NT, bool FAST>
int launch3(const bf16_t* qkv, bf16_t* out, int B, int N, int H, float scale, int causal, int nq, hipStream_t s) {
    if (g_attn_dbg && FAST && g_attn_variant == 6) return launch3_impl<DH, DP, NT, FAST, true, 9, true, true>(qkv, out, B, N, H, scale, causal, nq, s);
    if (g_attn_variant == 6) return launch3_impl<DH, DP, NT, FAST, false, 9, true, true>(qkv, out, B, N, H, scale, causal, nq, s);
    if (g_attn_dbg && FAST && g_attn_variant == 7) return launch3_impl<DH, DP, NT, FAST, true, 9, false, true>(qkv, out, B, N, H, scale, causal, nq, s);
    if (g_attn_variant == 7) return launch3_impl<DH, DP, NT, FAST, false, 9, false, true>(qkv, out, B, N, H, scale, causal, nq, s);
    if (g_attn_dbg && FAST && g_attn_variant == 5) return launch3_impl<DH, DP, NT, FAST, true, 9, true>(qkv, out, B, N, H, scale, causal, nq, s);
    if (g_attn_dbg && FAST) return launch3_impl<DH, DP, NT, FAST, true>(qkv, out, B, N, H, scale, causal, nq, s);
    if (g_attn_variant == 4) return launch3_impl<DH, DP, NT, FAST, false, 12>(qkv, out, B, N, H, scale, causal, nq, s);
    if (g_attn_variant == 5) return launch3_impl<DH, DP, NT, FAST, false, 9, true>(qkv, out, B, N, H, scale, causal, nq, s);
    return launch3_impl<DH, DP, NT, FAST, false>(qkv, out, B, N, H, scale, causal, nq, s);
}


template <int DH, int DP, int NT>
int launch2(const bf16_t* qkv, bf16_t* out, int B, int N, int H, float scale, int causal, int nq, hipStream_t s) {
    using C = AttnCfg2<DH, DP, NT>;
    static HirestDevCfg cfg;
    auto kern = attention_kernel_v2<DH, DP, NT>;
    if (int e = hirest_configure(kern, C::LDS_BYTES, cfg)) return e;
    hipLaunchKernelGGL(kern, dim3(B * H), dim3(512), C::LDS_BYTES, s, qkv, out, N, H, scale * 1.44269504088896340736f, causal, nq);
    return hirest_launch_status();
}

}

extern "C" int hirest_attention_debug_mode(int32_t bits) { g_attn_dbg = bits; return 0; }

extern "C" int hirest_attention_set_skew(int32_t units) {
    if (units < 0 || units > 64) return HIREST_E_BADARG;
    g_attn_skew = units;
    return 0;
}

extern "C" int hirest_attention_debug_trace_read(int64_t* dst, int32_t n) {
    if (!dst || n <= 0 || n > ATTN_TRACE_STEPS * ATTN_TRACE_WAVES * ATTN_TRACE_SLOTS) return HIREST_E_BADARG;
    return (int)hipMemcpyFromSymbol(dst, HIP_SYMBOL(g_attn_trace), sizeof(long long) * n);
}

extern "C" int hirest_attention_set_stagger(int32_t units) {
    if (units < 0 || units > 64) return HIREST_E_BADARG;
    g_attn_stagger = units;
    return 0;
}

extern "C" int hirest_attention_set_pace(int32_t units) {
    if (units < 0 || units > 64) return HIREST_E_BADARG;
    g_attn_pace = units;
    return 0;
}

extern "C" int hirest_attention_set_mapping(int32_t by_head) {
    if (by_head < 0 || by_head > 2) return HIREST_E_BADARG;
    g_attn_map = by_head;
    return 0;
}

extern "C" int hirest_attention_select_kernel(int32_t which) {
    if (which < 1 || which > 7) return HIREST_E_BADARG;
    g_attn_variant = which;
    return 0;
}

extern "C" int hirest_attention_bf16(const hirest_bf16* qkv, hirest_bf16* out, int32_t B, int32_t N, int32_t H,
                                     int32_t dh, float scale, int32_t causal, void* stream) {
    return hirest_attention_bf16_rows(qkv, out, B, N, H, dh, scale, causal, N, stream);
}

extern "C" int hirest_attention_bf16_rows(const hirest_bf16* qkv, hirest_bf16* out, int32_t B, int32_t N, int32_t H,
                                          int32_t dh, float scale, int32_t causal, int32_t q_rows, void* stream) {
    if (!qkv || !out || B <= 0 || N <= 0 || H <= 0 || q_rows <= 0 || q_rows > N) return HIREST_E_BADARG;
    const int nq = q_rows;
    hipStream_t s = reinterpret_cast<hipStream_t>(stream);
    const bf16_t* q = reinterpret_cast<const bf16_t*>(qkv);
    bf16_t* o = reinterpret_cast<bf16_t*>(out);
    HirestProfScope prof(HIREST_PROF_ATTENTION, causal, (int64_t)B * H, N, dh, s);
    if (g_attn_variant >= 3 && N > 80 && N <= 272 && B >= 64) {
        const bool fast = !causal && N > 256;
        if (dh == 88) return fast ? launch3<88, 96, 17, true>(q, o, B, N, H, scale, causal, nq, s)
                                  : launch3<88, 96, 17, false>(q, o, B, N, H, scale, causal, nq, s);
        if (dh == 64) return fast ? launch3<64, 64, 17, true>(q, o, B, N, H, scale, causal, nq, s)
                                  : launch3<64, 64, 17, false>(q, o, B, N, H, scale, causal, nq, s);
    }
    if (g_attn_variant >= 2) {
        if (dh == 88) {
            if (N <= 80) return launch2<88, 96, 5>(q, o, B, N, H, scale, causal, nq, s);
            if (N <= 272) return launch2<88, 96, 17>(q, o, B, N, H, scale, causal, nq, s);
        } else if (dh == 64) {
            if (N <= 80) return launch2<64, 64, 5>(q, o, B, N, H, scale, causal, nq, s);
            if (N <= 272) return launch2<64, 64, 17>(q, o, B, N, H, scale, causal, nq, s);
        }
        return HIREST_E_SHAPE;
    }
    if (dh == 88) {
        if (N <= 80) return launch<88, 96, 5>(q, o, B, N, H, scale, causal, nq, s);
        if (N <= 272) return launch<88, 96, 17>(q, o, B, N, H, scale, causal, nq, s);
    } else if (dh == 64) {
        if (N <= 80) return launch<64, 64, 5>(q, o, B, N, H, scale, causal, nq, s);
        if (N <= 272) return launch<64, 64, 17>(q, o, B, N, H, scale, causal, nq, s);
    }
    return HIREST_E_SHAPE;
}
```

hirest_amd/csrc/tower.hip:

```cpp
#include "common.h"

namespace {

inline size_t align256(size_t v) { return (v + 255) & ~(size_t)255; }

struct Regions {
    size_t x, h, big, eot, xb, xl, cls, part, stats, guard, total;
};

Regions plan(int64_t M, int D, int wide, int B, bool lnfold = false) {
    Regions r;
    size_t off = 0;
    r.x = off; off += align256((size_t)M * D * 4);
    r.h = off; off += align256((size_t)M * D * 2);
    r.big = off; off += align256((size_t)M * wide * 2);
    r.eot = off; off += align256((size_t)B * 4);
    r.xb = r.xl = r.cls = r.part = r.stats = r.guard = off;
    if (lnfold) {
        r.xb = off; off += align256((size_t)M * D * 2);
        r.xl = off; off += align256((size_t)M * D * 2);
        r.cls = off; off += 2 * align256((size_t)B * D * 2);
        r.part = off; off += align256((size_t)M * ((D + 63) / 64) * 8);
        r.stats = off; off += align256((size_t)M * 8);
        r.guard = off; off += 256;
    }
    r.total = off;
    return r;
}

inline bool vision_lnfold(const hirest_vision_tower* t, int B) {
    if (!t->blocks || !t->blocks[0].qkv_wf || t->act != 0 || t->ln_pre_g || B < 64) return false;
    const int T = (t->image_size / t->patch) * (t->image_size / t->patch) + 1;
    const int64_t M = (int64_t)B * T;
    return t->width >= 256 && t->width <= 1536 && t->width % 8 == 0 && M * t->width >= (int64_t)2048 * 1024;
}

inline int vision_wide(const hirest_vision_tower* t) {
    int w = 3 * t->width;
    if (t->mlp_dim > w) w = t->mlp_dim;
    if (t->kpad > w) w = t->kpad;
    return w;
}

#define CHECK(expr) do { int _e = (expr); if (_e != 0) return _e; } while (0)

int gemm(const void* A, int64_t lda, const void* W, int64_t ldw, const float* bias, void* out, int64_t ldo, int M, int N,
         int K, int epi, void* stream, const float* pos = nullptr, int P = 0, void* aux0 = nullptr, void* aux1 = nullptr,
         int flags = 0) {
    hirest_gemm_args a;
    a.struct_size = sizeof(a);
    a.A = reinterpret_cast<const hirest_bf16*>(A); a.lda = lda;
    a.W = reinterpret_cast<const hirest_bf16*>(W); a.ldw = ldw;
    a.bias = bias; a.out = out; a.ldo = ldo; a.M = M; a.N = N; a.K = K; a.epilogue = epi;
    a.pos = pos; a.patches_per_frame = P; a.aux0 = aux0; a.aux1 = aux1; a.flags = flags;
    return hirest_gemm_bf16(&a, stream);
}

int run_block(const hirest_block_weights& w, float* x, hirest_bf16* h, hirest_bf16* big, int B, int T, int D, int heads,
              int dh, int Dm, float eps, int act, int causal, void* stream) {
    const int M = B * T;
    CHECK(hirest_layernorm(x, D, nullptr, w.ln1_g, w.ln1_b, eps, h, D, 0, M, D, stream));
    CHECK(gemm(h, D, w.qkv_w, D, w.qkv_b, big, 3 * D, M, 3 * D, D, HIREST_EPI_BIAS_BF16, stream));
    CHECK(hirest_attention_bf16(big, h, B, T, heads, dh, 1.0f / sqrtf((float)dh), causal, stream));
    CHECK(gemm(h, D, w.proj_w, D, w.proj_b, x, D, M, D, D, HIREST_EPI_BIAS_RESID_F32, stream));
    CHECK(hirest_layernorm(x, D, nullptr, w.ln2_g, w.ln2_b, eps, h, D, 0, M, D, stream));
    CHECK(gemm(h, D, w.fc1_w, D, w.fc1_b, big, Dm, M, Dm, D,
               act == 1 ? HIREST_EPI_BIAS_QGELU_BF16 : HIREST_EPI_BIAS_GELU_BF16, stream));
    CHECK(gemm(big, Dm, w.fc2_w, Dm, w.fc2_b, x, D, M, D, Dm, HIREST_EPI_BIAS_RESID_F32, stream));
    return 0;
}

int run_block_lnfold(const hirest_block_weights& w, float* x, hirest_bf16* h, hirest_bf16* big, hirest_bf16* xb, float* part,
                     float* stats, float* guard, int B, int T, int D, int heads, int dh, int Dm, float eps, void* stream,
                     hirest_bf16* xl = nullptr) {
    const int M = B * T, G = (D + 63) / 64;
    void* res = xl ? static_cast<void*>(xl) : static_cast<void*>(x);
    const int epi_res = xl ? HIREST_EPI_BIAS_RESID2_LNSTATS : HIREST_EPI_BIAS_RESID_LNSTATS_F32;
    CHECK(gemm(xb, D, w.qkv_wf, D, w.qkv_bf, big, 3 * D, M, 3 * D, D, HIREST_EPI_LNFOLD_BF16, stream, nullptr, 0, stats,
               const_cast<float*>(w.qkv_s)));
    CHECK(hirest_attention_bf16(big, h, B, T, heads, dh, 1.0f / sqrtf((float)dh), 0, stream));
    CHECK(gemm(h, D, w.proj_w, D, w.proj_b, res, D, M, D, D, epi_res, stream, nullptr, 0, xb, part));
    CHECK(hirest_ln_stats_finalize(part, G, stats, eps, M, D, guard, stream));
    CHECK(gemm(xb, D, w.fc1_wf, D, w.fc1_bf, big, Dm, M, Dm, D, HIREST_EPI_LNFOLD_GELU_BF16, stream, nullptr, 0, stats,
               const_cast<float*>(w.fc1_s)));
    CHECK(gemm(big, Dm, w.fc2_w, Dm, w.fc2_b, res, D, M, D, Dm, epi_res, stream, nullptr, 0, xb, part, HIREST_GEMM_REVERSE));
    CHECK(hirest_ln_stats_finalize(part, G, stats, eps, M, D, guard, stream));
    return 0;
}

int run_block_lnfold_cls(const hirest_block_weights& w, float* x, hirest_bf16* h, hirest_bf16* big, hirest_bf16* xb, float* part,
                         float* stats, float* guard, int B, int T, int D, int heads, int dh, int Dm, float eps, void* stream,
                         hirest_bf16* xl = nullptr, hirest_bf16* cls_hi = nullptr, hirest_bf16* cls_lo = nullptr) {
    const int M = B * T, G = (D + 63) / 64;
    const int64_t TD = (int64_t)T * D;
    CHECK(gemm(xb, D, w.qkv_wf, D, w.qkv_bf, big, 3 * D, M, 3 * D, D, HIREST_EPI_LNFOLD_BF16, stream, nullptr, 0, stats,
               const_cast<float*>(w.qkv_s)));
    CHECK(hirest_attention_bf16_rows(big, h, B, T, heads, dh, 1.0f / sqrtf((float)dh), 0, 1, stream));
    if (xl) {
        hipStream_t s = reinterpret_cast<hipStream_t>(stream);
        if (hipMemcpy2DAsync(cls_hi, (size_t)D * 2, xb, (size_t)TD * 2, (size_t)D * 2, B, hipMemcpyDeviceToDevice, s) != hipSuccess ||
            hipMemcpy2DAsync(cls_lo, (size_t)D * 2, xl, (size_t)TD * 2, (size_t)D * 2, B, hipMemcpyDeviceToDevice, s) != hipSuccess)
            return hirest_launch_status();
        CHECK(gemm(h, TD, w.proj_w, D, w.proj_b, cls_lo, D, B, D, D, HIREST_EPI_BIAS_RESID2_LNSTATS, stream, nullptr, 0, cls_hi, part));
        CHECK(hirest_ln_stats_finalize(part, G, stats, eps, B, D, guard, stream));
        CHECK(gemm(cls_hi, D, w.fc1_wf, D, w.fc1_bf, big, Dm, B, Dm, D, HIREST_EPI_LNFOLD_GELU_BF16, stream, nullptr, 0, stats,
                   const_cast<float*>(w.fc1_s)));
        CHECK(gemm(big, Dm, w.fc2_w, Dm, w.fc2_b, cls_lo, D, B, D, Dm, HIREST_EPI_BIAS_RESID2_LNSTATS, stream, nullptr, 0, cls_hi, part));
        return 0;
    }
    CHECK(gemm(h, TD, w.proj_w, D, w.proj_b, x, TD, B, D, D, HIREST_EPI_BIAS_RESID_LNSTATS_F32, stream, nullptr, 0, xb, part));
    CHECK(hirest_ln_stats_finalize(part, G, stats, eps, B, D, guard, stream));
    CHECK(gemm(xb, D, w.fc1_wf, D, w.fc1_bf, big, Dm, B, Dm, D, HIREST_EPI_LNFOLD_GELU_BF16, stream, nullptr, 0, stats,
               const_cast<float*>(w.fc1_s)));
    CHECK(gemm(big, Dm, w.fc2_w, Dm, w.fc2_b, x, TD, B, D, Dm, HIREST_EPI_BIAS_RESID_LNSTATS_F32, stream, nullptr, 0, xb, part));
    return 0;
}

}

extern "C" int hirest_abi_version(void) { return HIREST_ABI_VERSION; }

extern "C" const char* hirest_build_info(void) {
    return "hirest_hip gfx950 (CDNA4) | gemm pq256 (persistent ping-pong, 2 phases per K step, 16x16x32 bf16 MFMA) / p256 / t128 + LDS-DMA | "
           "bf16x3 split-operand GEMM + attention | attention 16x16x32 bf16 MFMA + tr16 reads | " __VERSION__;
}

extern "C" size_t hirest_vision_workspace_bytes(const hirest_vision_tower* t, int32_t B) {
    if (!t || B <= 0) return 0;
    const int T = (t->image_size / t->patch) * (t->image_size / t->patch) + 1;
    return plan((int64_t)B * T, t->width, vision_wide(t), B, vision_lnfold(t, B)).total;
}

extern "C" size_t hirest_vision_guard_offset(const hirest_vision_tower* t, int32_t B) {
    if (!t || B <= 0 || !vision_lnfold(t, B)) return (size_t)-1;
    const int T = (t->image_size / t->patch) * (t->image_size / t->patch) + 1;
    return plan((int64_t)B * T, t->width, vision_wide(t), B, true).guard;
}

extern "C" int hirest_vision_forward(const hirest_vision_tower* t, const void* frames, int32_t in_dtype, int32_t B,
                                     float* out, void* workspace, size_t workspace_bytes, int32_t flags, void* stream) {
    if (!t || !frames || !out || !workspace || B <= 0 || !t->blocks) return HIREST_E_BADARG;
    if (t->width != t->heads * t->head_dim || t->image_size % t->patch != 0) return HIREST_E_SHAPE;
    const int G = t->image_size / t->patch, P = G * G, T = P + 1, D = t->width;
    const bool can_fold = vision_lnfold(t, B), lnfold = can_fold && !(flags & HIREST_TOWER_NO_LNFOLD);
    const Regions r = plan((int64_t)B * T, D, vision_wide(t), B, can_fold);
    if (workspace_bytes < r.total) return HIREST_E_WORKSPACE;
    char* ws = reinterpret_cast<char*>(workspace);
    float* x = reinterpret_cast<float*>(ws + r.x);
    hirest_bf16* h = reinterpret_cast<hirest_bf16*>(ws + r.h);
    hirest_bf16* big = reinterpret_cast<hirest_bf16*>(ws + r.big);

    CHECK(hirest_patchify(frames, in_dtype, B, t->image_size, t->patch, t->image_mean, t->image_std, big, t->kpad, stream));
    CHECK(gemm(big, t->kpad, t->patch_w, t->kpad, t->patch_b, x, D, B * P, D, t->kpad, HIREST_EPI_PATCH_POS_F32, stream,
               t->pos, P));
    CHECK(hirest_write_cls_rows(x, D, t->cls, t->pos, B, T, D, stream));
    if (t->ln_pre_g)
        CHECK(hirest_layernorm(x, D, nullptr, t->ln_pre_g, t->ln_pre_b, t->ln_eps, x, D, 1, B * T, D, stream));
    int64_t cls_ldx = (int64_t)T * D;
    if (lnfold) {
        hirest_bf16* xb = reinterpret_cast<hirest_bf16*>(ws + r.xb);
        float* part = reinterpret_cast<float*>(ws + r.part);
        float* stats = reinterpret_cast<float*>(ws + r.stats);
        float* guard = reinterpret_cast<float*>(ws + r.guard);
        if (hipMemsetAsync(guard, 0, 256, reinterpret_cast<hipStream_t>(stream)) != hipSuccess) return hirest_launch_status();
        const bool prune = !t->out_all_tokens && !(flags & HIREST_TOWER_NO_PRUNE);
        hirest_bf16* xl = ((flags & HIREST_TOWER_F32_RESIDUAL) || (prune && t->layers == 1)) ? nullptr : reinterpret_cast<hirest_bf16*>(ws + r.xl);
        hirest_bf16* cls_hi = reinterpret_cast<hirest_bf16*>(ws + r.cls);
        hirest_bf16* cls_lo = reinterpret_cast<hirest_bf16*>(ws + r.cls + align256((size_t)B * D * 2));
        CHECK(hirest_rowstats_split_bf16(x, D, xb, xl, stats, t->ln_eps, B * T, D, guard, stream));
        for (int l = 0; l < t->layers; ++l) {
            if (prune && l == t->layers - 1) {
                CHECK(run_block_lnfold_cls(t->blocks[l], x, h, big, xb, part, stats, guard, B, T, D, t->heads, t->head_dim, t->mlp_dim,
                                           t->ln_eps, stream, xl, cls_hi, cls_lo));
            } else {
                CHECK(run_block_lnfold(t->blocks[l], x, h, big, xb, part, stats, guard, B, T, D, t->heads, t->head_dim, t->mlp_dim,
                                       t->ln_eps, stream, xl));
            }
        }
        if (xl && !prune) CHECK(hirest_combine_hi_lo_f32(xb, xl, D, x, D, B * T, D, stream));
        if (xl && prune) {
            CHECK(hirest_combine_hi_lo_f32(cls_hi, cls_lo, D, x, D, B, D, stream));
            cls_ldx = D;
        }
    } else {
        for (int l = 0; l < t->layers; ++l)
            CHECK(run_block(t->blocks[l], x, h, big, B, T, D, t->heads, t->head_dim, t->mlp_dim, t->ln_eps, t->act, 0, stream));
    }
    if (t->out_all_tokens) {
        CHECK(hirest_layernorm(x, D, nullptr, t->norm_g, t->norm_b, t->ln_eps, h, D, 0, B * T, D, stream));
        CHECK(gemm(h, D, t->head_w, D, t->head_b, out, t->embed_dim, B * T, t->embed_dim, D, HIREST_EPI_BIAS_F32, stream));
        return 0;
    }
    CHECK(hirest_layernorm(x, cls_ldx, nullptr, t->norm_g, t->norm_b, t->ln_eps, h, D, 0, B, D, stream));
    CHECK(gemm(h, D, t->head_w, D, t->head_b, out, t->embed_dim, B, t->embed_dim, D, HIREST_EPI_BIAS_F32, stream));
    return 0;
}

extern "C" size_t hirest_text_workspace_bytes(const hirest_text_tower* t, int32_t B) {
    if (!t || B <= 0) return 0;
    return plan((int64_t)B * t->context, t->width, 4 * t->width, B).total;
}

extern "C" int hirest_text_forward(const hirest_text_tower* t, const int64_t* tokens, int32_t B, float* out,
                                   void* workspace, size_t workspace_bytes, void* stream) {
    if (!t || !tokens || !out || !workspace || B <= 0 || !t->blocks) return HIREST_E_BADARG;
    if (t->width % t->heads != 0) return HIREST_E_SHAPE;
    const int L = t->context, D = t->width, dh = D / t->heads;
    const Regions r = plan((int64_t)B * L, D, 4 * D, B);
    if (workspace_bytes < r.total) return HIREST_E_WORKSPACE;
    char* ws = reinterpret_cast<char*>(workspace);
    float* x = reinterpret_cast<float*>(ws + r.x);
    hirest_bf16* h = reinterpret_cast<hirest_bf16*>(ws + r.h);
    hirest_bf16* big = reinterpret_cast<hirest_bf16*>(ws + r.big);
    int32_t* eot = reinterpret_cast<int32_t*>(ws + r.eot);

    CHECK(hirest_embed_tokens(tokens, t->tok_emb, t->pos, x, eot, B, L, D, t->vocab, stream));
    for (int l = 0; l < t->layers; ++l)
        CHECK(run_block(t->blocks[l], x, h, big, B, L, D, t->heads, dh, 4 * D, t->ln_eps, t->act, 1, stream));
    CHECK(hirest_layernorm(x, D, eot, t->lnf_g, t->lnf_b, t->ln_eps, h, D, 0, B, D, stream));
    CHECK(gemm(h, D, t->proj_w, D, nullptr, out, t->embed_dim, B, t->embed_dim, D, HIREST_EPI_BIAS_F32, stream));
    return 0;
}
```

hirest_amd/eva_clip.py:

```python
from __future__ import annotations

import ctypes as C
import json
import math
import os
from contextlib import contextmanager
from copy import deepcopy
from operator import attrgetter
from typing import Dict, Optional, Tuple

import numpy as np
import torch
from torch import nn

from . import _lib, ops, synth

OPENAI_DATASET_MEAN = (0.48145466, 0.4578275, 0.40821073)
OPENAI_DATASET_STD = (0.26862954, 0.26130258, 0.27577711)

TOWER_PRECISIONS = ("fp32", "bf16x3", "bf16")
_NO_GUARD = (1 << 64) - 1

_MODEL_CONFIGS: Dict[str, dict] = {"EVA_CLIP_g_14": synth.EVA_CLIP_G_14, "EVA_CLIP_tiny_test": synth.EVA_CLIP_TINY,
                                   "EVA_CLIP_tiny_e1024_test": dict(synth.EVA_CLIP_TINY, embed_dim=1024)}


def list_models():
    return list(_MODEL_CONFIGS.keys())


def add_model_config(path):
    paths = [os.path.join(path, f) for f in os.listdir(path)] if os.path.isdir(path) else [path]
    for p in paths:
        if p.endswith(".json"):
            cfg = json.load(open(p))
            if all(k in cfg for k in ("embed_dim", "vision_cfg", "text_cfg")):
                _MODEL_CONFIGS[os.path.splitext(os.path.basename(p))[0]] = cfg


def get_model_config(model_name):
    return deepcopy(_MODEL_CONFIGS[model_name]) if model_name in _MODEL_CONFIGS else None


class _Leaf(nn.Module):

    def __init__(self, **shapes):
        super().__init__()
        for name, shape in shapes.items():
            self.register_parameter(name, nn.Parameter(torch.zeros(shape), requires_grad=True))


def _linear(out_f, in_f, bias=True):
    return _Leaf(weight=(out_f, in_f), bias=(out_f,)) if bias else _Leaf(weight=(out_f, in_f))


def _norm(d):
    return _Leaf(weight=(d,), bias=(d,))


def _struct(struct, /, **fields):
    names = [n for n, _ in struct._fields_]
    if sorted(fields) != sorted(names):
        raise TypeError(f"{struct.__name__}: fields {sorted(set(fields) ^ set(names))} missing or unknown")
    return struct(**fields)


@contextmanager
def _precision_scope(towers):
    old = [t.precision for t, _ in towers]
    try:
        for t, p in towers:
            if p is not None:
                t.precision = p
        yield
    finally:
        for (t, _), p in zip(towers, old):
            t.precision = p


def _fold_rows(lin, weight, norm):
    return tuple((f"{lin}_{out}", f"fold{i}", (weight, f"{lin}_b", norm)) for i, out in enumerate(("wf", "bf", "s")))


_NO_FOLD = tuple((f, None, None) for f in ("qkv_wf", "qkv_bf", "qkv_s", "fc1_wf", "fc1_bf", "fc1_s"))
_RESBLOCK = (("ln1_g", "f32", "ln_1.weight"), ("ln1_b", "f32", "ln_1.bias"),
             ("qkv_w", "w", "attn.in_proj_weight"), ("qkv_b", "f32", "attn.in_proj_bias"),
             ("proj_w", "w", "attn.out_proj.weight"), ("proj_b", "f32", "attn.out_proj.bias"),
             ("ln2_g", "f32", "ln_2.weight"), ("ln2_b", "f32", "ln_2.bias"),
             ("fc1_w", "w", "mlp.c_fc.weight"), ("fc1_b", "f32", "mlp.c_fc.bias"),
             ("fc2_w", "w", "mlp.c_proj.weight"), ("fc2_b", "f32", "mlp.c_proj.bias"))


class _Tower(nn.Module):
    _TABLES: Dict[str, tuple] = {}
    _what = "tower"
    fold_layernorm = False

    def __init__(self):
        super().__init__()
        self._prepared = None
        self._workspace = None
        self.precision = "bf16"

    def _apply(self, fn, *a, **k):
        self._prepared = None
        self._workspace = None
        return super()._apply(fn, *a, **k)

    def _load_from_state_dict(self, *a, **k):
        self._prepared = None
        return super()._load_from_state_dict(*a, **k)

    def invalidate(self):
        self._prepared = None

    def _ws(self, nbytes: int, device) -> torch.Tensor:
        if self._workspace is None or self._workspace.numel() < nbytes or self._workspace.device != device:
            self._workspace = torch.empty(nbytes, dtype=torch.uint8, device=device)
        return self._workspace

    @staticmethod
    def _f32(p: torch.Tensor) -> torch.Tensor:
        return p.detach().float().contiguous()

    def _prepared_for(self, kind: str, device) -> dict:
        cache = self._prepared
        if cache is None or any(p["device"] != device for p in cache.values()):
            cache = self._prepared = {}
        if kind not in cache:
            if device.type != "cuda":
                raise RuntimeError(f"hirest_amd: the {self._what} runs on MI355X only (no CPU fallback); move the model to a GPU")
            desc_cls, rows, block_cls, block_rows = self._TABLES[kind]
            keep = []
            blocks = (block_cls * self.layers)()
            for i, b in enumerate(self._blocks()):
                blocks[i] = _struct(block_cls, **self._pointers(b, block_rows, kind, device, keep))
            if kind == "x3":
                base = self._prepared_for("fp32", device)
                keep.append(base)
                scalars = {"base": C.pointer(base["desc"])}
            else:
                scalars = self._scalars()
            desc = _struct(desc_cls, blocks=blocks, **scalars, **self._pointers(self, rows, kind, device, keep))
            cache[kind] = {"device": device, "desc": desc, "blocks": blocks, "keep": keep}
        return cache[kind]

    def _pointers(self, owner, rows, kind, device, keep) -> dict:
        cast = ops.to_bf16 if kind == "bf16" else (lambda t: t)
        fold = self.fold_layernorm and not self.quick_gelu
        done, folded = {}, {}
        for field, form, src in rows:
            if form is None or (form.startswith("fold") and not fold):
                t = None
            elif form == "const":
                t = torch.tensor(getattr(self, src), dtype=torch.float32, device=device)
            elif form.startswith("fold"):
                if src not in folded:
                    weight, bias, norm = src
                    folded[src] = self._fold(self._f32(attrgetter(weight)(owner)), done[bias], attrgetter(norm)(owner), device)
                t = folded[src][int(form[4:])]
            else:
                p = attrgetter(src)(owner)
                if form == "qkv_bias":
                    t = torch.cat([p.q_bias.detach().float(), torch.zeros(self.width, device=device), p.v_bias.detach().float()])
                elif form == "patch":
                    K = p[0].numel()
                    t = torch.zeros((self.width, self._scalars()["kpad"]), dtype=torch.float32, device=device)
                    t[:, :K] = p.detach().float().reshape(self.width, K)
                    t = cast(t)
                else:
                    t = self._f32(p.detach().float().t() if form == "wT" else p)
                    t = ops.split2(t) if form == "split" else t if form == "f32" else cast(t)
            done[field] = t
        keep.extend(t for t in done.values() if t is not None)
        return {f: None if t is None else t.data_ptr() for f, t in done.items()}

    def _fold(self, w32, bias, norm, device):
        N, K = w32.shape
        wf = torch.empty((N, K), dtype=torch.bfloat16, device=device)
        bf = torch.empty((N,), dtype=torch.float32, device=device)
        cs = torch.empty((N,), dtype=torch.float32, device=device)
        _lib.check(_lib.load().hirest_fold_layernorm(w32.data_ptr(), self._f32(norm.weight).data_ptr(), self._f32(norm.bias).data_ptr(),
                                                     bias.data_ptr(), wf.data_ptr(), bf.data_ptr(), cs.data_ptr(), N, K,
                                                     ops.stream_ptr()), "hirest_fold_layernorm")
        return wf, bf, cs

    @staticmethod
    def _call_size(B: int, limit, near_equal: bool) -> int:
        limit = max(1, int(limit))
        return -(-B // -(-B // limit)) if near_equal else min(B, limit)

    def _run_calls(self, B: int, limit, near_equal: bool, ws_bytes, call, device):
        if B <= 0:
            return []
        step = self._call_size(B, limit, near_equal)
        ws = self._ws(ws_bytes(step), device)
        spans = [(s, min(step, B - s)) for s in range(0, B, step)]
        for s, n in spans:
            call(s, n, ws)
        return spans


class VisionTower(_Tower):
    _what = "vision tower"
    _FIELDS = (("patch_w", "patch", "patch_embed.proj.weight"), ("patch_b", "f32", "patch_embed.proj.bias"),
               ("cls", "f32", "cls_token"), ("pos", "f32", "pos_embed"), ("norm_g", "f32", "norm.weight"), ("norm_b", "f32", "norm.bias"),
               ("head_w", "w", "head.weight"), ("head_b", "f32", "head.bias"),
               ("image_mean", "const", "image_mean"), ("image_std", "const", "image_std"), ("ln_pre_g", None, None), ("ln_pre_b", None, None))
    _BLOCK = (("ln1_g", "f32", "norm1.weight"), ("ln1_b", "f32", "norm1.bias"),
              ("qkv_w", "w", "attn.qkv.weight"), ("qkv_b", "qkv_bias", "attn"),
              ("proj_w", "w", "attn.proj.weight"), ("proj_b", "f32", "attn.proj.bias"),
              ("ln2_g", "f32", "norm2.weight"), ("ln2_b", "f32", "norm2.bias"),
              ("fc1_w", "w", "mlp.fc1.weight"), ("fc1_b", "f32", "mlp.fc1.bias"),
              ("fc2_w", "w", "mlp.fc2.weight"), ("fc2_b", "f32", "mlp.fc2.bias"))
    _TABLES = {"bf16": (_lib.VisionTower, _FIELDS, _lib.BlockWeights,
                        _BLOCK + _fold_rows("qkv", "attn.qkv.weight", "norm1") + _fold_rows("fc1", "mlp.fc1.weight", "norm2")),
               "fp32": (_lib.VisionTowerF32, _FIELDS, _lib.BlockWeightsF32, _BLOCK),
               "x3": (_lib.VisionTowerX3, (), _lib.BlockWeightsX3, tuple((f + "2", "split", src) for f, form, src in _BLOCK if form == "w"))}

    def __init__(self, image_size, patch_size, width, layers, heads, mlp_ratio, embed_dim, quick_gelu=False):
        super().__init__()
        self.image_size, self.patch_size, self.width, self.layers, self.heads = image_size, patch_size, width, layers, heads
        self.mlp_dim = int(width * mlp_ratio)
        self.embed_dim = self.num_classes = embed_dim
        self.quick_gelu = quick_gelu
        self.num_tokens = (image_size // patch_size) ** 2 + 1
        D, Dm = width, self.mlp_dim
        self.cls_token = nn.Parameter(torch.zeros(1, 1, D))
        self.pos_embed = nn.Parameter(torch.zeros(1, self.num_tokens, D))
        self.patch_embed = nn.Module()
        self.patch_embed.proj = _Leaf(weight=(D, 3, patch_size, patch_size), bias=(D,))
        blocks = []
        for _ in range(layers):
            b = nn.Module()
            b.norm1, b.norm2 = _norm(D), _norm(D)
            b.attn = _Leaf(q_bias=(D,), v_bias=(D,))
            b.attn.qkv = _linear(3 * D, D, bias=False)
            b.attn.proj = _linear(D, D)
            b.mlp = nn.Module()
            b.mlp.fc1, b.mlp.fc2 = _linear(Dm, D), _linear(D, Dm)
            blocks.append(b)
        self.blocks = nn.ModuleList(blocks)
        self.norm = _norm(D)
        self.head = _linear(embed_dim, D)
        self.image_mean, self.image_std = OPENAI_DATASET_MEAN, OPENAI_DATASET_STD
        self.max_frames_per_call = 1024
        self.max_frames_per_call_f32 = 256
        self.max_frames_per_call_x3 = 1024
        self.fold_layernorm = True
        self.fold_guard_ratio = 4.0
        self.last_fold_ratio = 0.0
        self.fold_fallbacks = 0
        self.prune_last_block = True
        self.f32_residual = os.environ.get("HIREST_F32_RESIDUAL", "0") == "1"

    def _blocks(self):
        return self.blocks

    def _scalars(self):
        P = self.patch_size
        return dict(image_size=self.image_size, patch=P, width=self.width, heads=self.heads, head_dim=self.width // self.heads,
                    mlp_dim=self.mlp_dim, layers=self.layers, embed_dim=self.embed_dim, kpad=(3 * P * P + 63) // 64 * 64,
                    act=1 if self.quick_gelu else 0, ln_eps=1e-6,
                    out_all_tokens=0)

    _EXACT = {"fp32": ("fp32", "hirest_vision_workspace_bytes_f32", "hirest_vision_forward_f32", "max_frames_per_call_f32", False),
              "bf16x3": ("x3", "hirest_vision_workspace_bytes_x3", "hirest_vision_forward_x3", "max_frames_per_call_x3", True)}

    def _forward_exact(self, image: torch.Tensor) -> torch.Tensor:
        kind, ws_bytes, fwd, limit, near_equal = self._EXACT[self.precision]
        desc = C.byref(self._prepared_for(kind, image.device)["desc"])
        lib = _lib.load()
        out = torch.empty((image.shape[0], self.embed_dim), dtype=torch.float32, device=image.device)
        code = ops._IN_DTYPES[image.dtype]

        def call(s, n, ws):
            _lib.check(getattr(lib, fwd)(desc, image[s:s + n].data_ptr(), code, n, out[s:s + n].data_ptr(), ws.data_ptr(), ws.numel(),
                                         ops.stream_ptr()), fwd)
        self._run_calls(image.shape[0], getattr(self, limit), near_equal, lambda n: getattr(lib, ws_bytes)(desc, n), call, image.device)
        return out

    @torch.no_grad()
    @ops.on_tensor_device
    def forward(self, image: torch.Tensor) -> torch.Tensor:
        if image.dtype == torch.uint8:
            H, W = image.shape[1], image.shape[2]
        else:
            H, W = image.shape[-2], image.shape[-1]
            if image.dtype not in (torch.float32, torch.bfloat16):
                image = image.float()
        assert H == self.image_size and W == self.image_size, \
            f"Input image size ({H}*{W}) doesn't match model ({self.image_size}*{self.image_size})."
        image = image.contiguous()
        if self.precision in self._EXACT:
            return self._forward_exact(image)
        desc = C.byref(self._prepared_for("bf16", image.device)["desc"])
        lib = _lib.load()
        B = image.shape[0]
        out = torch.empty((B, self.embed_dim), dtype=torch.float32, device=image.device)
        if B == 0:
            return out
        step = self._call_size(B, self.max_frames_per_call, True)
        code = ops._IN_DTYPES[image.dtype]
        self.last_fold_ratio = 0.0
        flags = (0 if self.prune_last_block else _lib.TOWER_NO_PRUNE) | (_lib.TOWER_F32_RESIDUAL if self.f32_residual else 0)
        goff = lib.hirest_vision_guard_offset(desc, step) if self.fold_guard_ratio is not None else _NO_GUARD
        guards = torch.zeros(-(-B // step), dtype=torch.float32, device=image.device) if goff != _NO_GUARD else None

        def call(s, n, ws, extra=0):
            _lib.check(lib.hirest_vision_forward(desc, image[s:s + n].data_ptr(), code, n, out[s:s + n].data_ptr(),
                                                 ws.data_ptr(), ws.numel(), flags | extra, ops.stream_ptr()), "hirest_vision_forward")

        def guarded(s, n, ws):
            call(s, n, ws)
            if guards is not None:
                g = lib.hirest_vision_guard_offset(desc, n)
                if g != _NO_GUARD:
                    guards[s // step:s // step + 1].copy_(ws[g:g + 4].view(torch.float32))
        spans = self._run_calls(B, self.max_frames_per_call, True, lambda n: lib.hirest_vision_workspace_bytes(desc, n), guarded, image.device)
        if guards is not None:
            ratios = guards.cpu().tolist()
            self.last_fold_ratio = max(ratios)
            for (s, n), ratio in zip(spans, ratios):
                if not ratio <= self.fold_guard_ratio:
                    self.fold_fallbacks += 1
                    call(s, n, self._workspace, _lib.TOWER_NO_LNFOLD)
        return out


class TextTower(_Tower):
    _what = "text tower"
    _FIELDS = (("tok_emb", "f32", "token_embedding.weight"), ("pos", "f32", "positional_embedding"),
               ("lnf_g", "f32", "ln_final.weight"), ("lnf_b", "f32", "ln_final.bias"), ("proj_w", "wT", "text_projection"))
    _TABLES = {"bf16": (_lib.TextTower, _FIELDS, _lib.BlockWeights, _RESBLOCK + _NO_FOLD),
               "fp32": (_lib.TextTowerF32, _FIELDS, _lib.BlockWeightsF32, _RESBLOCK)}

    def __init__(self, vocab_size, width, layers, heads, context_length, embed_dim, quick_gelu=False):
        super().__init__()
        self.vocab_size, self.width, self.layers, self.heads = vocab_size, width, layers, heads
        self.context_length, self.embed_dim, self.quick_gelu = context_length, embed_dim, quick_gelu
        D = width
        self.token_embedding = _Leaf(weight=(vocab_size, D))
        self.positional_embedding = nn.Parameter(torch.zeros(context_length, D))
        self.transformer = nn.Module()
        blocks = []
        for _ in range(layers):
            b = nn.Module()
            b.ln_1, b.ln_2 = _norm(D), _norm(D)
            b.attn = _Leaf(in_proj_weight=(3 * D, D), in_proj_bias=(3 * D,))
            b.attn.out_proj = _linear(D, D)
            b.mlp = nn.Module()
            b.mlp.c_fc, b.mlp.c_proj = _linear(4 * D, D), _linear(D, 4 * D)
            blocks.append(b)
        self.transformer.resblocks = nn.ModuleList(blocks)
        self.ln_final = _norm(D)
        self.text_projection = nn.Parameter(torch.zeros(D, embed_dim))
        self.logit_scale = nn.Parameter(torch.ones([]) * math.log(1 / 0.07))
        self.max_rows_per_call = 1024

    def _blocks(self):
        return self.transformer.resblocks

    def _scalars(self):
        return dict(context=self.context_length, vocab=self.vocab_size, width=self.width, heads=self.heads, layers=self.layers,
                    embed_dim=self.embed_dim, act=1 if self.quick_gelu else 0, ln_eps=1e-5)

    @torch.no_grad()
    @ops.on_tensor_device
    def forward(self, text: torch.Tensor) -> torch.Tensor:
        if text.dim() != 2 or text.shape[1] != self.context_length:
            raise RuntimeError(f"encode_text expects [B,{self.context_length}] token ids, got {tuple(text.shape)}")
        f32 = self.precision == "fp32"
        desc = C.byref(self._prepared_for("fp32" if f32 else "bf16", text.device)["desc"])
        lib = _lib.load()
        text = text.to(torch.int64).contiguous()
        out = torch.empty((text.shape[0], self.embed_dim), dtype=torch.float32, device=text.device)
        ws_bytes, fwd = (lib.hirest_text_workspace_bytes_f32, lib.hirest_text_forward_f32) if f32 else \
            (lib.hirest_text_workspace_bytes, lib.hirest_text_forward)

        def call(s, n, ws):
            _lib.check(fwd(desc, text[s:s + n].data_ptr(), n, out[s:s + n].data_ptr(), ws.data_ptr(), ws.numel(), ops.stream_ptr()),
                       "hirest_text_forward_f32" if f32 else "hirest_text_forward")
        self._run_calls(text.shape[0], self.max_rows_per_call, False, lambda n: ws_bytes(desc, n), call, text.device)
        return out


class EVA_CLIP(nn.Module):

    def __init__(self, embed_dim: int, vision_cfg: dict, text_cfg: dict, quick_gelu: bool = False):
        super().__init__()
        v, t = dict(vision_cfg), dict(text_cfg)
        self.visual = VisionTower(v.get("image_size", 224), v.get("patch_size", 16), v.get("width", 768),
                                  v.get("layers", 12), v.get("width", 768) // v.get("head_width", 64),
                                  v.get("mlp_ratio", 4.0), embed_dim)
        self.text = TextTower(t.get("vocab_size", 49408), t.get("width", 512), t.get("layers", 12), t.get("heads", 8),
                              t.get("context_length", 77), embed_dim, quick_gelu)
        self.output_dtype = torch.float32

    def set_precision(self, precision: str):
        if precision not in TOWER_PRECISIONS:
            raise ValueError(f"precision must be one of {TOWER_PRECISIONS}, got {precision!r}")
        self.visual.precision = precision
        self.text.precision = "fp32" if precision == "bf16x3" else precision
        return self

    def precision_scope(self, visual: Optional[str] = None, text: Optional[str] = None):
        for precision in (visual, text):
            if precision is not None and precision not in TOWER_PRECISIONS:
                raise ValueError(f"precision must be one of {TOWER_PRECISIONS}, got {precision!r}")
        return _precision_scope(((self.visual, visual), (self.text, "fp32" if text == "bf16x3" else text)))

    @torch.no_grad()
    def init_random_(self, seed: int = 0):
        gen = torch.Generator(device=next(self.parameters()).device)
        gen.manual_seed(seed)
        for name, p in self.named_parameters():
            std, mean = synth._init_rule(name, tuple(p.shape))
            if std == 0.0:
                p.fill_(mean)
            else:
                p.normal_(mean, std, generator=gen)
        self.visual.invalidate()
        self.text.invalidate()
        return self

    def encode_image(self, image):
        return self.visual(image).to(self.output_dtype)

    def encode_text(self, text):
        return self.text(text).to(self.output_dtype)

    def forward(self, image, text):
        if image is None:
            return self.encode_text(text)
        elif text is None:
            return self.encode_image(image)
        img = self.visual(image)
        txt = self.text(text)
        img_n = ops.pool_l2norm(img.unsqueeze(1)).to(self.output_dtype)
        txt_n = ops.pool_l2norm(txt.unsqueeze(1)).to(self.output_dtype)
        return img_n, txt_n, self.text.logit_scale.exp()


def load_state_dict(checkpoint_path: str, map_location: str = "cpu", model_key="model|module|state_dict"):
    if isinstance(checkpoint_path, str) and checkpoint_path.startswith("synth:"):
        raise RuntimeError("synthetic checkpoints are resolved in create_model")
    checkpoint = torch.load(checkpoint_path, map_location=map_location)
    state_dict = checkpoint
    for mk in model_key.split("|"):
        if isinstance(checkpoint, dict) and mk in checkpoint:
            state_dict = checkpoint[mk]
            break
    if next(iter(state_dict.items()))[0].startswith("module"):
        state_dict = {k[7:]: v for k, v in state_dict.items()}
    return state_dict


def load_checkpoint(model, checkpoint_path, model_key="model|module|state_dict", strict=True):
    sd = load_state_dict(checkpoint_path, model_key=model_key)
    return model.load_state_dict(sd, strict=strict)


def create_model(model_name: str, pretrained: str = "", precision: str = "fp32",
                 device: torch.device = torch.device("cpu"), force_quick_gelu: bool = False):
    model_name = model_name.replace("/", "-")
    if model_name not in _MODEL_CONFIGS:
        raise RuntimeError(f"Model config for {model_name} not found.")
    cfg = deepcopy(_MODEL_CONFIGS[model_name])
    if force_quick_gelu:
        cfg["quick_gelu"] = True
    synthetic = isinstance(pretrained, str) and pretrained.startswith("synth:")
    if not synthetic and not os.path.isfile(pretrained):
        raise FileNotFoundError(f"[Errno 2] No such file or directory: '{pretrained}'")
    model = EVA_CLIP(**cfg)
    if isinstance(pretrained, str) and pretrained.startswith("synth:"):
        model.load_state_dict(synth.eva_clip_state_dict(cfg, int(pretrained.split(":", 1)[1])), strict=True)
    else:
        load_checkpoint(model, pretrained)
    device = torch.device(device)
    model.to(device=device)
    env = os.environ.get("HIREST_PRECISION", "").strip().lower()
    if env and env not in TOWER_PRECISIONS:
        raise ValueError(f"HIREST_PRECISION={env!r}: expected one of {TOWER_PRECISIONS}")
    if env and precision != "fp32" and precision != env:
        import warnings
        warnings.warn(f"hirest_amd: HIREST_PRECISION={env} ignored: create_model was called with precision={precision!r}")
        env = ""
    if env:
        model.set_precision(env)
    elif precision == "fp32":
        model.set_precision("fp32")
    elif precision in TOWER_PRECISIONS:
        model.set_precision(precision)
    elif precision in ("bf16", "amp", "amp_bf16", "amp_bfloat16", "fp16"):
        model.set_precision("bf16")
    else:
        raise ValueError(f"unknown precision {precision!r} (fp32 | bf16 | amp | fp16)")
    if precision == "fp16":
        assert device.type != "cpu"
        model.output_dtype = torch.float16
    model.visual.image_mean = OPENAI_DATASET_MEAN
    model.visual.image_std = OPENAI_DATASET_STD
    return model


class ImageTransform:

    def __init__(self, image_size: int, mean=None, std=None):
        if isinstance(image_size, (list, tuple)):
            image_size = image_size[0]
        self.size = int(image_size)
        mean = mean or OPENAI_DATASET_MEAN
        std = std or OPENAI_DATASET_STD
        mean = (mean,) * 3 if not isinstance(mean, (list, tuple)) else mean
        std = (std,) * 3 if not isinstance(std, (list, tuple)) else std
        self.mean = np.asarray(mean, dtype=np.float32).reshape(3, 1, 1)
        self.std = np.asarray(std, dtype=np.float32).reshape(3, 1, 1)

    def __call__(self, img):
        from PIL import Image
        w, h = img.size
        s = self.size
        if not ((w <= h and w == s) or (h <= w and h == s)):
            if w < h:
                nw, nh = s, int(s * h / w)
            else:
                nh, nw = s, int(s * w / h)
            img = img.resize((nw, nh), Image.BICUBIC)
            w, h = nw, nh
        left, top = int(round((w - s) / 2.0)), int(round((h - s) / 2.0))
        img = img.crop((left, top, left + s, top + s)).convert("RGB")
        a = np.asarray(img, dtype=np.float32).transpose(2, 0, 1) / 255.0
        return torch.from_numpy((a - self.mean) / self.std)


def image_transform(image_size: int, mean: Optional[Tuple[float, ...]] = None, std: Optional[Tuple[float, ...]] = None):
    return ImageTransform(image_size, mean, std)


def build_eva_model_and_transforms(model_name: str, pretrained: str = "", precision: str = "fp32",
                                   device: torch.device = torch.device("cpu"), force_quick_gelu: bool = False,
                                   image_mean: Optional[Tuple[float, ...]] = None,
                                   image_std: Optional[Tuple[float, ...]] = None):
    model = create_model(model_name, pretrained, precision, device, force_quick_gelu=force_quick_gelu)
    image_mean = image_mean or getattr(model.visual, "image_mean", None)
    image_std = image_std or getattr(model.visual, "image_std", None)
    preprocess = image_transform(model.visual.image_size, mean=image_mean, std=image_std)
    return model, preprocess
```

include/hirest_hip.h:

```cpp
#ifndef HIREST_HIP_H
#define HIREST_HIP_H

#include <stddef.h>
#include <stdint.h>

#ifdef __cplusplus
extern "C" {
#endif

#define HIREST_ABI_VERSION 4

#define HIREST_E_BADARG   (-1)
#define HIREST_E_SHAPE    (-2)
#define HIREST_E_WORKSPACE (-3)

typedef uint16_t hirest_bf16;

int hirest_abi_version(void);
const char* hirest_build_info(void);

enum hirest_epilogue {
    HIREST_EPI_BIAS_BF16 = 0,
    HIREST_EPI_BIAS_GELU_BF16 = 1,
    HIREST_EPI_BIAS_QGELU_BF16 = 2,
    HIREST_EPI_BIAS_RESID_F32 = 3,
    HIREST_EPI_BIAS_F32 = 4,
    HIREST_EPI_PATCH_POS_F32 = 5,
    HIREST_EPI_BIAS_RESID_LNSTATS_F32 = 6,
    HIREST_EPI_LNFOLD_BF16 = 7,
    HIREST_EPI_LNFOLD_GELU_BF16 = 8,
    HIREST_EPI_BIAS_GELU_SPLIT2 = 9,
    HIREST_EPI_BIAS_RESID2_LNSTATS = 10
};

typedef struct hirest_gemm_args {
    uint64_t struct_size;
    const hirest_bf16* A;  int64_t lda;
    const hirest_bf16* W;  int64_t ldw;
    const float* bias;
    void* out;             int64_t ldo;
    int32_t M, N, K;
    int32_t epilogue;
    const float* pos;
    int32_t patches_per_frame;
    void* aux0;
    void* aux1;
    int32_t flags;
} hirest_gemm_args;
enum { HIREST_GEMM_REVERSE = 1,
       HIREST_GEMM_X3 = 2,
       HIREST_GEMM_X3_T128 = 4
     };

int hirest_gemm_bf16(const hirest_gemm_args* args, void* stream);
int hirest_gemm_select_kernel(int32_t which);
int hirest_gemm_debug_mode(int32_t bits);
int hirest_gemm_dispatch_name(const hirest_gemm_args* args, char* out, int32_t out_len);

int hirest_layernorm(const float* x, int64_t ldx, const int32_t* row_index,
                     const float* gamma, const float* beta, float eps,
                     void* out, int64_t ldo, int32_t out_is_f32,
                     int32_t rows, int32_t D, void* stream);

int hirest_attention_bf16(const hirest_bf16* qkv, hirest_bf16* out,
                          int32_t B, int32_t N, int32_t H, int32_t dh,
                          float scale, int32_t causal, void* stream);
int hirest_attention_bf16_rows(const hirest_bf16* qkv, hirest_bf16* out,
                               int32_t B, int32_t N, int32_t H, int32_t dh,
                               float scale, int32_t causal, int32_t q_rows, void* stream);
int hirest_attention_select_kernel(int32_t which);
int hirest_attention_set_mapping(int32_t by_head);
int hirest_attention_set_pace(int32_t units);
int hirest_attention_set_stagger(int32_t units);
int hirest_attention_set_skew(int32_t units);
int hirest_attention_debug_mode(int32_t bits);
int hirest_attention_debug_trace_read(int64_t* dst, int32_t n);

int hirest_patchify(const void* frames, int32_t in_dtype, int32_t B, int32_t S, int32_t P,
                    const float* mean3, const float* std3,
                    hirest_bf16* patches, int32_t Kpad, void* stream);

int hirest_fold_layernorm(const float* W, const float* gamma, const float* beta, const float* bias, hirest_bf16* Wf,
                          float* bias_out, float* colsum_out, int32_t N, int32_t K, void* stream);
int hirest_write_cls_rows(float* x, int64_t ldx, const float* cls, const float* pos0,
                          int32_t B, int32_t tokens_per_frame, int32_t D, void* stream);

int hirest_rowstats_bf16(const float* x, int64_t ldx, hirest_bf16* xb, float* stats, float eps, int32_t rows, int32_t D,
                         float* guard, void* stream);
int hirest_rowstats_split_bf16(const float* x, int64_t ldx, hirest_bf16* xb, hirest_bf16* xlo, float* stats, float eps, int32_t rows,
                               int32_t D, float* guard, void* stream);
int hirest_combine_hi_lo_f32(const hirest_bf16* hi, const hirest_bf16* lo, int64_t ld_in, float* out, int64_t ldo, int32_t rows,
                             int32_t D, void* stream);
int hirest_ln_stats_finalize(const float* partials, int32_t groups, float* stats, float eps, int32_t rows, int32_t D,
                             float* guard, void* stream);

int hirest_embed_tokens(const int64_t* tokens, const float* tok_emb, const float* pos,
                        float* x, int32_t* eot_row, int32_t B, int32_t L, int32_t D,
                        int32_t vocab, void* stream);

int hirest_f32_to_bf16(const float* in, hirest_bf16* out, int64_t n, void* stream);

int hirest_pool_l2norm(const float* frame_embeds, float* out, int32_t V, int32_t F, int32_t E,
                       int32_t normalize_frames_first, void* stream);
int hirest_pool_l2norm_varlen(const float* rows, const int32_t* seg_off, float* out, int32_t V, int32_t E, void* stream);

int hirest_similarity_f32(const float* text_n, const float* video_n, float* scores,
                          int32_t Q, int32_t V, int32_t E, void* stream);

int hirest_topk_f32(const float* scores, const int32_t* tie_rank, int32_t Q, int32_t V, int32_t k,
                    int32_t* out_index, float* out_score, void* stream);
int64_t hirest_topk_workspace_bytes(int32_t Q, int32_t V, int32_t k);
int hirest_topk_f32_ws(const float* scores, const int32_t* tie_rank, int32_t Q, int32_t V, int32_t k,
                       int32_t* out_index, float* out_score, void* workspace, int64_t workspace_bytes, void* stream);
int hirest_clip_score(const void* img_rows, int32_t img_dtype, int32_t U, const void* txt_rows, int32_t txt_dtype,
                      const int32_t* sel, int32_t C, int32_t K, int32_t E, float* out, void* stream);

#define HIREST_BERTSCORE_MAX_TOKENS 1024
int hirest_bertscore_greedy(const float* states, int64_t ld, int32_t D, const int32_t* seq_off, int32_t n_seq,
                            const float* tok_weight, const int32_t* cand_seq, const int32_t* ref_seq, int32_t n_pairs,
                            float* out , void* stream);

typedef struct hirest_block_weights {
    const float* ln1_g; const float* ln1_b;
    const hirest_bf16* qkv_w; const float* qkv_b;
    const hirest_bf16* proj_w; const float* proj_b;
    const float* ln2_g; const float* ln2_b;
    const hirest_bf16* fc1_w; const float* fc1_b;
    const hirest_bf16* fc2_w; const float* fc2_b;
    const hirest_bf16* qkv_wf; const float* qkv_bf; const float* qkv_s;
    const hirest_bf16* fc1_wf; const float* fc1_bf; const float* fc1_s;
} hirest_block_weights;

typedef struct hirest_vision_tower {
    int32_t image_size, patch, width, heads, head_dim, mlp_dim, layers, embed_dim;
    int32_t kpad;
    int32_t act;
    float ln_eps;
    const hirest_bf16* patch_w;
    const float* patch_b;
    const float* cls;
    const float* pos;
    const hirest_block_weights* blocks;
    const float* norm_g; const float* norm_b;
    const hirest_bf16* head_w;
    const float* head_b;
    const float* image_mean; const float* image_std;
    const float* ln_pre_g; const float* ln_pre_b;
    int32_t out_all_tokens;
} hirest_vision_tower;

size_t hirest_vision_workspace_bytes(const hirest_vision_tower* t, int32_t B);
enum { HIREST_TOWER_NO_LNFOLD = 1,
       HIREST_TOWER_NO_PRUNE = 2,
       HIREST_TOWER_F32_RESIDUAL = 4 };
int hirest_vision_forward(const hirest_vision_tower* t, const void* frames, int32_t in_dtype,
                          int32_t B, float* out, void* workspace, size_t workspace_bytes,
                          int32_t flags, void* stream);
size_t hirest_vision_guard_offset(const hirest_vision_tower* t, int32_t B);

typedef struct hirest_text_tower {
    int32_t context, vocab, width, heads, layers, embed_dim;
    int32_t act;
    float ln_eps;
    const float* tok_emb;
    const float* pos;
    const hirest_block_weights* blocks;
    const float* lnf_g; const float* lnf_b;
    const hirest_bf16* proj_w;
} hirest_text_tower;

size_t hirest_text_workspace_bytes(const hirest_text_tower* t, int32_t B);
int hirest_text_forward(const hirest_text_tower* t, const int64_t* tokens, int32_t B, float* out,
                        void* workspace, size_t workspace_bytes, void* stream);

typedef struct hirest_block_weights_f32 {
    const float* ln1_g; const float* ln1_b;
    const float* qkv_w; const float* qkv_b;
    const float* proj_w; const float* proj_b;
    const float* ln2_g; const float* ln2_b;
    const float* fc1_w; const float* fc1_b;
    const float* fc2_w; const float* fc2_b;
} hirest_block_weights_f32;

typedef struct hirest_vision_tower_f32 {
    int32_t image_size, patch, width, heads, head_dim, mlp_dim, layers, embed_dim;
    int32_t kpad;
    int32_t act;
    float ln_eps;
    const float* patch_w;
    const float* patch_b; const float* cls; const float* pos;
    const hirest_block_weights_f32* blocks;
    const float* norm_g; const float* norm_b;
    const float* head_w; const float* head_b;
    const float* image_mean; const float* image_std;
    const float* ln_pre_g; const float* ln_pre_b;
    int32_t out_all_tokens;
} hirest_vision_tower_f32;

typedef struct hirest_text_tower_f32 {
    int32_t context, vocab, width, heads, layers, embed_dim;
    int32_t act;
    float ln_eps;
    const float* tok_emb; const float* pos;
    const hirest_block_weights_f32* blocks;
    const float* lnf_g; const float* lnf_b;
    const float* proj_w;
} hirest_text_tower_f32;

size_t hirest_vision_workspace_bytes_f32(const hirest_vision_tower_f32* t, int32_t B);
int hirest_vision_forward_f32(const hirest_vision_tower_f32* t, const void* frames, int32_t in_dtype, int32_t B, float* out,
                              void* workspace, size_t workspace_bytes, void* stream);
int hirest_vision_embed_f32(const hirest_vision_tower_f32* t, const void* frames, int32_t in_dtype, int32_t B, float* x, float* rows,
                            void* stream);
size_t hirest_text_workspace_bytes_f32(const hirest_text_tower_f32* t, int32_t B);
int hirest_text_forward_f32(const hirest_text_tower_f32* t, const int64_t* tokens, int32_t B, float* out,
                            void* workspace, size_t workspace_bytes, void* stream);

typedef struct hirest_block_weights_x3 {
    const hirest_bf16* qkv_w2;
    const hirest_bf16* proj_w2;
    const hirest_bf16* fc1_w2;
    const hirest_bf16* fc2_w2;
} hirest_block_weights_x3;

typedef struct hirest_vision_tower_x3 {
    const hirest_vision_tower_f32* base;
    const hirest_block_weights_x3* blocks;
} hirest_vision_tower_x3;

int hirest_split2_bf16(const float* x, int64_t ldx, hirest_bf16* out, int64_t ldo, int64_t rows, int32_t D, int32_t act, void* stream);
int hirest_split2_transposed_bf16(const float* x, int64_t ldx, hirest_bf16* out, int64_t ldo, int32_t rows, int32_t cols, void* stream);
#define HIREST_SPLIT_GROUP_MAX 16
typedef struct hirest_split_item {
    const float* x; hirest_bf16* out;
    int64_t ldx, ldo;
    int32_t rows, cols, transposed, reserved;
} hirest_split_item;
int hirest_split2_grouped_bf16(const hirest_split_item* items, int32_t count, void* stream);
int hirest_layernorm_split2(const float* x, int64_t ldx, const float* gamma, const float* beta, float eps, hirest_bf16* out, int64_t ldo,
                            int32_t rows, int32_t D, void* stream);
int hirest_attention_x3_qkv(const float* q, int64_t ldq, const float* k, const float* v, int64_t ldkv, float* out, int32_t B, int32_t Tq,
                            int32_t Tk, int32_t H, int32_t dh, float scale, void* stream);
int hirest_attention_x3_qkv_split2(const float* q, int64_t ldq, const float* k, const float* v, int64_t ldkv, hirest_bf16* out2, int32_t B,
                                   int32_t Tq, int32_t Tk, int32_t H, int32_t dh, float scale, void* stream);
int hirest_attention_x3_select_waves(int32_t waves);
int hirest_attention_x3_debug_trace(int64_t* device_buffer);
int hirest_vision_x3_select_attention(int32_t which);
size_t hirest_vision_workspace_bytes_x3(const hirest_vision_tower_x3* t, int32_t B);
int hirest_vision_forward_x3(const hirest_vision_tower_x3* t, const void* frames, int32_t in_dtype, int32_t B, float* out,
                             void* workspace, size_t workspace_bytes, void* stream);

int hirest_gemm_f32(const float* A, int64_t lda, const float* W, int64_t ldw, const float* bias,
                    const float* resid, int64_t ldr, const float* periodic, int32_t period,
                    float* out, int64_t ldo, int32_t M, int32_t N, int32_t K, int32_t act, void* stream);
size_t hirest_gemm_f32_workspace_bytes(int32_t M, int32_t N, int32_t K);
int hirest_gemm_f32_ws(const float* A, int64_t lda, const float* W, int64_t ldw, const float* bias, const float* resid, int64_t ldr,
                       const float* periodic, int32_t period, float* out, int64_t ldo, int32_t M, int32_t N, int32_t K, int32_t act,
                       void* workspace, size_t workspace_bytes, void* stream);
size_t hirest_gemm_f32_layouts_workspace_bytes(int32_t M, int32_t N, int32_t K);
int hirest_gemm_f32_layouts(const float* A, int64_t lda, int32_t a_kmajor, const float* W, int64_t ldw, int32_t w_kmajor,
                            const float* bias, const float* resid, int64_t ldr, float* out, int64_t ldo, int32_t M, int32_t N,
                            int32_t K, int32_t act, void* workspace, size_t workspace_bytes, void* stream);
int hirest_gemm_f32_select_kernel(int32_t which);
int hirest_gemm_f32_ring_mode(int32_t mode);
int hirest_gemm_f32_ln(const float* X, int64_t ldx, const int32_t* ids, const float* table, const float* pos_row,
                       const float* gamma, const float* beta, float eps, float* ln_out, int64_t ldl, const float* W, int64_t ldw,
                       const float* bias, const float* resid, int64_t ldr, float* out, int64_t ldo, int32_t M, int32_t N, int32_t K,
                       int32_t act, void* stream);
int hirest_gemm_f32_ln_colmax(const float* X, int64_t ldx, const float* gamma, const float* beta, float eps, const float* W, int64_t ldw,
                              const float* bias, float* out, int64_t ldo, float* colmax, int32_t M, int32_t N, int32_t K, void* stream);
int hirest_gemm_f32_rows_ln_mode(int32_t mode);
int hirest_gemm_f32_rows_preferred(int32_t M);
int hirest_gemm_f32_rows_colmax(const float* A, int64_t lda, const float* W, int64_t ldw, const float* bias, float* out, int64_t ldo,
                                float* colmax, int32_t M, int32_t N, int32_t K, void* stream);
#define HIREST_F32_ENTRY_GEMM 0
#define HIREST_F32_ENTRY_WS 1
#define HIREST_F32_ENTRY_LAYOUTS 2
#define HIREST_F32_ENTRY_LN 3
#define HIREST_F32_ENTRY_LN_COLMAX 4
#define HIREST_F32_ENTRY_ROWS_COLMAX 5
typedef struct hirest_gemm_f32_query {
    uint32_t struct_size;
    int32_t entry;
    int32_t M, N, K;
    int32_t has_resid, has_periodic;
    int32_t has_ids, has_ln_out;
    int32_t has_workspace;
    int32_t a_kmajor, w_kmajor;
    int32_t select_kernel, ring_mode, rows_ln_mode;
    int32_t cus;
} hirest_gemm_f32_query;
int hirest_gemm_f32_dispatch_name(const hirest_gemm_f32_query* query, char* out, int32_t out_len);
int hirest_attention_f32(const float* qkv, float* out, int32_t B, int32_t T, int32_t H, int32_t dh,
                         float scale, float add_const, void* stream);
int hirest_attention_f32_qkv(const float* q, int64_t ldq, const float* k, const float* v, int64_t ldkv, float* out,
                             int32_t B, int32_t Tq, int32_t Tk, int32_t H, int32_t dh, float scale, float add_const,
                             float causal_penalty, void* stream);
int hirest_attention_f32_varlen(const float* qkv, float* out, const int32_t* seq_off, int32_t B, int32_t max_len, int32_t H,
                                int32_t dh, float scale, float add_const, void* stream);
int hirest_log_softmax_f32(const float* x, int64_t ldx, const float* row_add, float* out, int64_t ldo, int32_t rows,
                           int32_t V, void* stream);
int hirest_joint_time_features(const int32_t* n_valid, const float* w1, const float* b1, float* tin,
                               int32_t B, int32_t T, int32_t E, void* stream);
int hirest_joint_time_grid_f32(const int32_t* n_valid, int32_t B, int32_t T, float* grid, void* stream);
int hirest_joint_base(const float* v, const float* text_proj, const float* asr, const float* temporal, float* base,
                      int32_t B, int32_t T, int32_t E, void* stream);
int hirest_joint_mask_add(const float* base, const int32_t* moment_mask, const int32_t* boundary_mask,
                          const float* mask_embed, const float* boundary_embed, float* f, int64_t rows, int32_t E,
                          void* stream);
int hirest_linear_heads(const float* x, int64_t rows, int32_t D, int32_t nheads, const float* w0, const float* w1,
                        const float* w2, const float* bias3, float* logits, void* stream);
typedef struct hirest_caption_layer {
    const float* qkv_w; const float* qkv_b;
    const float* so_w; const float* so_b; const float* so_ln_g; const float* so_ln_b;
    const float* cq_w; const float* cq_b;
    const float* co_w; const float* co_b; const float* co_ln_g; const float* co_ln_b;
    const float* ff1_w; const float* ff1_b;
    const float* ff2_w; const float* ff2_b; const float* ff_ln_g; const float* ff_ln_b;
} hirest_caption_layer;
typedef struct hirest_caption_decoder {
    int32_t layers, heads, hidden, inter, vocab_padded, max_pos;
    const float* word_emb; const float* pos_emb; const float* emb_ln_g; const float* emb_ln_b;
    const hirest_caption_layer* layer;
    const float* tr_w; const float* tr_b; const float* tr_ln_g; const float* tr_ln_b;
    const float* lm_w; const float* lm_b;
    const hirest_bf16* lm_w2;
} hirest_caption_decoder;
size_t hirest_caption_step_workspace_bytes(const hirest_caption_decoder* d, int32_t R);
int hirest_caption_decode_step(const hirest_caption_decoder* d, int32_t R, int32_t position, const int32_t* last_ids,
                               const int32_t* parent_rows, const float* const* kv_in, float* const* kv_out,
                               const float* const* enc_kv, int32_t F, const float* row_add, float* logp,
                               void* workspace, size_t workspace_bytes, void* stream);

int hirest_attention_f32_decode(const float* q, int64_t ldq, const float* k_hist, const float* v_hist, int64_t ld_hist,
                                const int32_t* parent, int32_t t_hist, const float* k_new, const float* v_new, int64_t ld_new,
                                float* k_out, float* v_out, float* out, int32_t R, int32_t H, float scale, float add_const,
                                float causal_penalty, void* stream);
int hirest_caption_select(int32_t mode);
int hirest_caption_decode_logits(const hirest_caption_decoder* d, int32_t R, int32_t position, const int32_t* last_ids,
                                 const int32_t* parent_rows, const float* const* kv_in, float* const* kv_out,
                                 const float* const* enc_kv, int32_t F, float* logits, void* workspace, size_t workspace_bytes,
                                 void* stream);
size_t hirest_caption_beam_tail_workspace_bytes(int32_t B, int32_t beam, int32_t vocab);
int hirest_caption_beam_tail(const float* logits, int64_t ldx, const float* row_add, int32_t B, int32_t beam, int32_t vocab,
                             int32_t step, int32_t max_steps, int32_t eos_id, float* scores, int32_t* tokens, int32_t* backptr,
                             int32_t* n_steps, int32_t* done, int32_t* next_ids, int32_t* next_parents, float* next_add,
                             int32_t* done_host, void* workspace, size_t workspace_bytes, void* stream);

int hirest_caption_beam_step(const hirest_caption_decoder* d, int32_t B, int32_t beam, int32_t position, int32_t* ids, int32_t* parent_rows,
                             const float* const* kv_in, float* const* kv_out, const float* const* enc_kv, int32_t F, float* row_add,
                             float* logits, int32_t max_steps, int32_t eos_id, float* scores, int32_t* tokens, int32_t* backptr,
                             int32_t* n_steps, int32_t* done, int32_t* done_host, void* workspace, size_t workspace_bytes,
                             void* tail_workspace, size_t tail_workspace_bytes, void* stream);

int hirest_beam_advance(const float* val, const int32_t* idx, int32_t B, int32_t beam, int32_t vocab, int32_t step, int32_t max_steps,
                        int32_t eos_id, float* scores, int32_t* tokens, int32_t* backptr, int32_t* n_steps, int32_t* done,
                        int32_t* next_ids, int32_t* next_parents, float* next_add, void* stream);
int hirest_beam_backtrack(const float* scores, const int32_t* tokens, const int32_t* backptr, const int32_t* n_steps, int32_t B,
                          int32_t beam, int32_t max_steps, int32_t* out, void* stream);

int hirest_gemm_f32_strided(const float* A, int64_t sam, int64_t sak, const float* B, int64_t sbn, int64_t sbk, float* C, int64_t ldc,
                            int32_t M, int32_t N, int32_t K, float alpha, void* stream);
int hirest_transpose_pad_f32(const float* in, int64_t ld_in, int32_t R, int32_t C, float* out, int32_t Rp, void* stream);
int hirest_weighted_colsum_f32(const float* x, int64_t ldx, const float* row_weight, const int32_t* row_select,
                               int32_t select_value, int32_t R, int32_t C, float* out, void* stream);
#define HIREST_COLSUM_GROUP_MAX 40
typedef struct hirest_colsum_item {
    const float*   x;
    const float*   row_weight;
    const int32_t* row_select;
    float*         out;
    int64_t        ldx;
    int32_t        R, C, select_value, reserved;
} hirest_colsum_item;
int hirest_weighted_colsum_grouped_f32(const hirest_colsum_item* items, int32_t count, void* stream);
int hirest_act_f32(const float* pre, float* y, int64_t n, int32_t act, void* stream);
int hirest_scale_by_device_scalar_f32(float* x, const float* scalar, int64_t n, void* stream);
int hirest_act_bwd_f32(const float* pre, const float* dy, float* dx, int64_t n, int32_t act, void* stream);
int hirest_dropout_add_f32(const float* x, const float* resid, float* y, int64_t n, float p, uint32_t seed, void* stream);
int hirest_layernorm_bwd_f32(const float* x, const float* dy, const float* gamma, float eps, float* dx, float* dyxhat,
                             int32_t R, int32_t D, void* stream);
int hirest_attention_train_fwd_f32(const float* qkv, float* P, float* ctx, int32_t B, int32_t T, int32_t H, int32_t dh,
                                   float scale, float add_const, float drop_p, uint32_t seed, void* stream);
int hirest_attention_train_bwd_f32(const float* qkv, const float* P, const float* dctx, float* dS, float* dqkv, int32_t B,
                                   int32_t T, int32_t H, int32_t dh, float scale, float drop_p, uint32_t seed, void* stream);
int hirest_attention_train_select(int32_t which);
int hirest_attention_train_fwd_qkv_f32(const float* q, int64_t ldq, const float* k, const float* v, int64_t ldkv,
                                       const float* mask_add, float* P, float* ctx, int64_t ldctx, int32_t B, int32_t Tq, int32_t Tk,
                                       int32_t H, int32_t dh, float scale, float add_const, float drop_p, uint32_t seed, void* stream);
int hirest_attention_train_bwd_qkv_f32(const float* q, int64_t ldq, const float* k, const float* v, int64_t ldkv, const float* P,
                                       const float* dctx, int64_t ldctx, float* dS, float* dq, int64_t lddq, float* dk, float* dv,
                                       int64_t lddkv, int32_t B, int32_t Tq, int32_t Tk, int32_t H, int32_t dh, float scale,
                                       float drop_p, uint32_t seed, void* stream);
int hirest_embedding_fwd_f32(const int32_t* ids, const float* table, const float* pos, float* out, int64_t rows, int32_t T,
                             int32_t D, void* stream);
int hirest_embedding_pos_fwd_f32(const int32_t* ids, const int32_t* pos_ids, const float* table, const float* pos, float* out,
                                 int64_t rows, int32_t D, void* stream);
int hirest_embedding_bwd_f32(const int32_t* ids, const float* dx, float* dtable_accum, int64_t rows, int32_t D, void* stream);
int hirest_ce_rows_f32(const float* logits, int64_t ld, const int32_t* target, int32_t R, int32_t V, float weight, int32_t n_valid,
                       float* loss_accum, float* dlogits, void* stream);
int hirest_bce_masked_f32(const float* logits, const int32_t* target, const int32_t* mask, int32_t B, int32_t T, float weight,
                          float* loss_accum, float* dlogits, void* stream);
int hirest_joint_base_bwd_f32(const float* dbase, const float* v, const float* tn, float* dv, float* dtn, int32_t B, int32_t T,
                              int32_t E, void* stream);
int hirest_l2norm_bwd_f32(const float* t, const float* dtn, float* dt, int32_t B, int32_t E, void* stream);
int hirest_ce_masked_f32(const float* logits, const int32_t* mask, const int32_t* target, int32_t B, int32_t T, float weight,
                         float* loss_accum, float* dlogits, void* stream);
int hirest_heads_bwd_f32(const float* dlogits, int64_t rows, int32_t D, int32_t nheads, const float* w0, const float* w1,
                         const float* w2, float* dfeats, void* stream);

int hirest_masked_argmax(const float* logits, const int32_t* mask, float fill, int32_t B, int32_t T, int32_t* out,
                         void* stream);
int hirest_moment_valid_f32(const float* logits, const int32_t* vis_mask, const int32_t* moment_mask, const int32_t* start_target,
                            const int32_t* end_target, int32_t B, int32_t T, float fill, int32_t* pred , float* loss,
                            void* stream);
size_t hirest_lm_head_ce_workspace_bytes(int32_t R, int32_t V);
int hirest_lm_head_ce_f32(const float* h, int64_t ldh, const float* W, int64_t ldw, const float* bias, const int32_t* target, int32_t R,
                          int32_t V, int32_t K, int32_t n_valid, float* nll, float* loss, void* workspace, size_t workspace_bytes,
                          void* stream);
int hirest_segmentation_step(const float* logits, int32_t* moment_mask, int32_t* boundary_mask, int32_t B, int32_t T,
                             double threshold, int32_t* steps, int32_t* nsteps, int32_t max_steps, float* probs_out,
                             void* stream);

int64_t hirest_preprocess_plan_bytes(int32_t in_h, int32_t in_w, int32_t size);
int hirest_preprocess_plan(int32_t in_h, int32_t in_w, int32_t size, void* host_plan, int64_t plan_bytes);
int64_t hirest_preprocess_workspace_bytes(int32_t in_h, int32_t in_w, int32_t size, int32_t B);
int hirest_preprocess_u8(const uint8_t* frames, int32_t B, int32_t in_h, int32_t in_w, int32_t size,
                         const void* plan_dev, void* out, int32_t out_kind, const float* mean3, const float* std3,
                         void* workspace, int64_t workspace_bytes, void* stream);

enum hirest_jpeg_reason {
    HIREST_JPEG_OK = 0, HIREST_JPEG_NOT_JPEG = 1, HIREST_JPEG_PROGRESSIVE = 2, HIREST_JPEG_ARITHMETIC = 3,
    HIREST_JPEG_LOSSLESS = 4,
    HIREST_JPEG_PRECISION = 5,
    HIREST_JPEG_COLOR = 6,
    HIREST_JPEG_SAMPLING = 7, HIREST_JPEG_MULTI_SCAN = 8,
    HIREST_JPEG_TRUNCATED = 9,
    HIREST_JPEG_BAD_TABLES = 10, HIREST_JPEG_SIZE = 11
};
#define HIREST_JPEG_ST_BAD_CODE 1
#define HIREST_JPEG_ST_COEF_OVERRUN 2
#define HIREST_JPEG_ST_OUT_OF_DATA 4
#define HIREST_JPEG_ST_BAD_RESTART 8
#define HIREST_JPEG_ST_UNSUPPORTED 16

typedef struct {
    int32_t width, height, ncomp, hs, vs;
    int32_t restart_interval, mcux, mcuy;
    int32_t supported, reason;
    int64_t scan_begin, scan_end;
    int32_t table_set, reserved;
    int64_t data_offset, out_offset;
    int64_t ws_offset, plane_offset;
} hirest_jpeg_image;

typedef struct {
    uint16_t qt[3][64];
    uint8_t huff_bits[6][16];
    uint8_t huff_vals[6][256];
} hirest_jpeg_tables;

int hirest_jpeg_parse(const uint8_t* data, int64_t size, hirest_jpeg_image* img, hirest_jpeg_tables* tables);
int64_t hirest_jpeg_workspace_bytes(hirest_jpeg_image* imgs, int32_t n);
int hirest_jpeg_decode(const hirest_jpeg_image* imgs_host, const hirest_jpeg_image* imgs_dev, int32_t n,
                       const hirest_jpeg_tables* tables_dev, const uint8_t* data, uint8_t* out, int32_t* status,
                       void* workspace, int64_t workspace_bytes, void* stream);
int hirest_jpeg_decode_host(const hirest_jpeg_image* img, const hirest_jpeg_tables* tables, const uint8_t* data,
                            uint8_t* out, int32_t* status);
int64_t hirest_jpeg_chunked_workspace_bytes(int32_t n);
int hirest_jpeg_decode_chunked(const hirest_jpeg_image* imgs_host, const hirest_jpeg_image* imgs_dev, int32_t n,
                               const hirest_jpeg_tables* tables_dev, const uint8_t* data, uint8_t* out, int32_t* status,
                               void* workspace, int64_t workspace_bytes, int64_t chunk_bytes, void* chunk_workspace,
                               int64_t chunk_workspace_bytes, void* stream);
int hirest_jpeg_decode_host_chunked(const hirest_jpeg_image* img, const hirest_jpeg_tables* tables, const uint8_t* data,
                                    int64_t chunk_bytes, uint8_t* out, int32_t* status, int32_t* rounds_out);

int hirest_interval_iou_f64(const double* a, const double* b, int64_t n, double* iou, void* stream);
int hirest_step_bound_pr(const double* refs, const int32_t* ref_off, const double* preds, const int32_t* pred_off,
                         int32_t V, double tiou, double* recall, double* precision, double* best_iou, void* stream);
int hirest_preprocess_moment_bounds(const double* preds, const int32_t* pred_off, const double* gt_minmax, int32_t V,
                                    double* out, int32_t* out_count, int32_t max_out, void* stream);

int hirest_frame_to_timestamp(const int64_t* frame, const double* duration, const int32_t* n_frames, int32_t n_frames_all,
                              int64_t per_video, int64_t n, int64_t* timestamp, void* stream);
int hirest_timestamp_to_frame(const double* t, const double* duration, const int32_t* n_frames, int32_t n_frames_all,
                              int64_t per_video, int64_t n, int64_t* frame, void* stream);

int hirest_cascade_moment_bounds(const int32_t* pred_frames, const double* duration, const int32_t* n_frames, int32_t n_frames_all,
                                 int32_t B, int32_t T, int64_t* bounds_ts, int32_t* bound_frames, int32_t* moment_mask,
                                 int32_t* boundary_mask, void* stream);
int hirest_cascade_boundaries(const int32_t* steps, const int32_t* nsteps, const int32_t* bound_frames, const double* duration,
                              const int32_t* n_frames, int32_t n_frames_all, int32_t B, int32_t iters, int32_t* n_bounds,
                              int32_t* bounds, int64_t* step_ts, int32_t* step_frames, int32_t* step_sample, int32_t* offsets,
                              void* stream);
int hirest_cascade_trim_gather(const float* vis, const float* asr, const int32_t* step_frames, const int32_t* step_sample, int32_t S,
                               int32_t B, int32_t T, int32_t D, int32_t Da, int32_t F, float* out_vis, float* out_asr, void* stream);

enum hirest_prof_kind { HIREST_PROF_GEMM = 0, HIREST_PROF_ATTENTION = 1, HIREST_PROF_LAYERNORM = 2 };
typedef struct hirest_prof_record {
    int32_t kind;
    int32_t tag;
    int64_t d0, d1, d2;
    float ms;
} hirest_prof_record;
int hirest_profile_enable(int32_t on);
int hirest_profile_collect(hirest_prof_record* out, int32_t max_records);

typedef struct hirest_joint_layer_x3 {
    const hirest_bf16* qkv_w2; const float* qkv_b;
    const hirest_bf16* ao_w2;  const float* ao_b;
    const float* ln1_g; const float* ln1_b;
    const hirest_bf16* fc1_w2; const float* fc1_b;
    const hirest_bf16* fc2_w2; const float* fc2_b;
    const float* ln2_g; const float* ln2_b;
} hirest_joint_layer_x3;
typedef struct hirest_joint_encoder_x3 {
    uint64_t struct_size;
    int32_t layers, heads, width, mlp_dim, in_dim, max_pos;
    float ln_eps, attn_shift;
    const hirest_bf16* emb_w2; const float* emb_b;
    const float* pos;
    const float* emb_ln_g; const float* emb_ln_b;
    const hirest_joint_layer_x3* layer;
} hirest_joint_encoder_x3;
size_t hirest_joint_encoder_x3_workspace_bytes(const hirest_joint_encoder_x3* e, int32_t B, int32_t T);
int hirest_joint_encoder_x3_forward(const hirest_joint_encoder_x3* e, const float* f, int32_t B, int32_t T, float* out,
                                    void* workspace, size_t workspace_bytes, void* stream);
int hirest_layernorm_f32_split2(const float* x, int64_t ldx, const float* add, int32_t period, const float* gamma, const float* beta, float eps,
                                float* out32, int64_t ldo32, hirest_bf16* out2, int64_t ldo2, int32_t rows, int32_t D, void* stream);


typedef struct hirest_train_block {
    uint64_t struct_size;
    int32_t B, T, heads, width, mlp, precision;
    float ln_eps, drop;
    uint32_t seed_attn, seed_ao, seed_out, reserved;
    const float *wqkv, *bqkv;
    const float *wo, *bo, *ln1_g, *ln1_b;
    const float *w1, *b1, *w2, *b2, *ln2_g, *ln2_b;
    const float* x;
    float *qkv, *P, *cx, *a_pre, *aa, *hpre, *hh, *x_pre, *out;
    const hirest_bf16* x2; hirest_bf16* out2;
    const hirest_bf16 *wqkv2, *wo2, *w12, *w22;
    const hirest_bf16 *wqkvT2, *woT2, *w1T2, *w2T2;
    void* ws; size_t ws_bytes;
} hirest_train_block;
typedef struct hirest_train_block_grads {
    uint64_t struct_size;
    const float* dout;
    float* dx;
    float *g_wqkv, *g_wo, *g_w1, *g_w2;
    float *g_bqkv, *g_bo, *g_b1, *g_b2, *g_ln1_g, *g_ln1_b, *g_ln2_g, *g_ln2_b;
    hirest_colsum_item* items; int32_t* n_items; int32_t max_items, reserved;
    void* side_stream; void* side_ws; size_t side_ws_bytes;
    void* scratch; size_t scratch_bytes;
} hirest_train_block_grads;
typedef struct hirest_train_fusion_bwd {
    uint64_t struct_size;
    int32_t B, T, E, W, vis_dim, text_dim, asr_dim, boundary, max_pos, reserved;
    float drop; uint32_t seed_emb;
    const float *w_emb, *emb_ln_g, *t2_w, *asr1_w, *asr0_g, *norm_g;
    const float *x0, *f, *v, *tn, *tin, *a0, *asr2, *v0, *vis2, *t, *text;
    const int32_t *mm32, *bm32, *n_valid;
    const float* dx;
    float *g_emb_ln_g, *g_emb_ln_b, *g_pos, *g_w_emb, *g_b_emb, *g_mask, *g_bound, *g_t2_w, *g_t2_b, *g_t0_w, *g_t0_b,
          *g_asr1_w, *g_asr1_b, *g_asr0_g, *g_asr0_b, *g_norm_g, *g_norm_b, *g_vis_w, *g_vis_b, *g_text_w, *g_text_b;
    hirest_colsum_item* items; int32_t* n_items; int32_t max_items, reserved2;
    void* ws; size_t ws_bytes;
    void* side_stream; void* side_ws; size_t side_ws_bytes;
    void* scratch; size_t scratch_bytes;
} hirest_train_fusion_bwd;
size_t hirest_train_fusion_backward_scratch_bytes(const hirest_train_fusion_bwd* f);
int hirest_train_fusion_backward(const hirest_train_fusion_bwd* f, void* stream);
size_t hirest_train_block_forward_scratch_bytes(const hirest_train_block* b);
int hirest_train_block_forward(const hirest_train_block* b, void* scratch, size_t scratch_bytes, void* stream);
size_t hirest_train_block_backward_scratch_bytes(const hirest_train_block* b);
int hirest_train_block_backward(const hirest_train_block* b, const hirest_train_block_grads* g, void* stream);

#define HIREST_OPTIM_GROUP_MAX 64
#define HIREST_OPTIM_CHUNK 8192
typedef struct hirest_optim_item {
    float*       p;
    const float* g;
    float*       m;
    float*       v;
    int64_t      n;
} hirest_optim_item;
int64_t hirest_optim_partials_count(const hirest_optim_item* items, int32_t count);
int hirest_grad_sqnorm_grouped_f32(const hirest_optim_item* items, int32_t count, float* partials, void* stream);
int hirest_clip_coef_f32(const float* partials, int64_t count, float max_norm, float* norm_coef, void* stream);
int hirest_adamw_grouped_f32(const hirest_optim_item* items, int32_t count, const float* coef, float decay, float one_minus_beta1,
                             float beta2, float one_minus_beta2, float step_size, float bc2_sqrt, float eps, void* stream);
int hirest_grad_sqnorm_scaled_grouped_f32(const hirest_optim_item* items, int32_t count, const float* grad_scale, float* partials,
                                          void* stream);
int hirest_clip_coef_dev_f32(const float* partials, int64_t count, const float* max_norm, float* norm_coef, void* stream);
int hirest_optim_step_advance_f32(float* const* steps, int32_t count, const float* found_inf, void* stream);
int hirest_adamw_capturable_grouped_f32(const hirest_optim_item* items, float* const* steps, int32_t count, const float* coef,
                                        const float* lr_ptr, double lr, const float* grad_scale, const float* found_inf,
                                        double beta1, double beta2, float eps, double weight_decay, void* stream);

#define HIREST_BATCH_GATHER_MAX 8
typedef struct hirest_batch_gather {
    const void* src;
    void*       dst;
    const int32_t* row_of_example;
    int32_t words, reserved;
} hirest_batch_gather;
typedef struct hirest_batch_args {
    uint64_t struct_size;
    const int32_t* index;
    int32_t B, T, D, Da, n_examples, n_model_frames, n_gather, reserved;
    const float*   frames;
    const int64_t* frame_off;
    const float*   asr_rows;
    const int64_t* sub_off;
    const int32_t* sub_span;
    const int32_t* ex_video;
    const int32_t* ex_len;
    const int32_t* ex_range;
    const int32_t* bound_off;
    const int32_t* bound_val;
    float*   vis;
    float*   asr;
    int64_t *vis_mask, *moment_mask, *prev_boundary_mask;
    hirest_batch_gather gather[HIREST_BATCH_GATHER_MAX];
} hirest_batch_args;
int hirest_batch_assemble(const hirest_batch_args* a, void* stream);

size_t hirest_log_mel_workspace_bytes(int64_t n, int64_t padding);
int hirest_log_mel(const float* audio, int64_t n, int64_t padding, const float* filters, int32_t n_mels, const double* tables,
                   float* out, void* workspace, size_t workspace_bytes, void* stream);
int hirest_mel_to_rows(const float* mel, float* rows, int32_t B, int32_t n_mels, int32_t T, void* stream);

int hirest_attention_f32_decode_inplace(const float* q, int64_t ldq, float* k_cache, float* v_cache, int64_t ld_cache, int64_t row_stride,
                                        int32_t t, int32_t T_max, const float* k_new, const float* v_new, int64_t ld_new, float* out,
                                        int32_t R, int32_t H, float scale, float add_const, float causal_penalty, void* stream);
size_t hirest_attention_f32_cross_decode_workspace_bytes(int32_t R, int32_t H, int32_t Tk);
int hirest_attention_f32_cross_decode(const float* q, int64_t ldq, const float* kv, int64_t ldkv, int64_t window_stride, int32_t n_windows,
                                      int32_t Tk, const int32_t* row_window, float* out, int64_t ldo, int32_t R, int32_t H, float scale,
                                      void* workspace, size_t workspace_bytes, void* stream);

typedef struct hirest_whisper_row_state {
    int32_t n_sampled;
    int32_t last, penult;
    int32_t last_timestamp;
    int32_t completed;
    float   sum_logprobs;
    float   no_speech_prob;
    float   last_logprob;
} hirest_whisper_row_state;
typedef struct hirest_whisper_tail_params {
    int32_t n_vocab;
    int32_t eot, no_speech;
    int32_t no_timestamps, timestamp_begin, max_initial_timestamp_index;
    int32_t sample_begin;
    int32_t blank, suppress_blank;
    int32_t timestamp_rules;
    int32_t monotonic;
    float   temperature;
    uint32_t seed, serial;
    const uint32_t* suppress_mask;
} hirest_whisper_tail_params;
int hirest_whisper_step_tail(const float* logits, int64_t ldx, int32_t R, int32_t V, int32_t step, int32_t T_max,
                             const hirest_whisper_tail_params* params, hirest_whisper_row_state* state, int32_t* next_ids, int32_t* tokens,
                             float* logprobs, int32_t* done_host, void* stream);
int hirest_whisper_gumbel_bits(uint32_t seed, uint32_t serial, int32_t R, int32_t V, uint32_t* out, void* stream);

typedef struct hirest_whisper_layer {
    const float* attn_ln_g; const float* attn_ln_b;
    const float* qkv_w; const float* qkv_b;
    const float* so_w; const float* so_b;
    const float* cross_ln_g; const float* cross_ln_b;
    const float* cq_w; const float* cq_b;
    const float* co_w; const float* co_b;
    const float* mlp_ln_g; const float* mlp_ln_b;
    const float* fc1_w; const float* fc1_b; const float* fc2_w; const float* fc2_b;
} hirest_whisper_layer;
typedef struct hirest_whisper_decoder {
    int32_t layers, heads, hidden, inter, vocab_padded, max_pos;
    const float* tok_emb;
    const float* pos_emb;
    const hirest_whisper_layer* layer;
    const float* ln_g; const float* ln_b;
    const float* lm_b;
} hirest_whisper_decoder;
size_t hirest_whisper_step_workspace_bytes(const hirest_whisper_decoder* d, int32_t R, int32_t Tk);
int hirest_whisper_decode_step(const hirest_whisper_decoder* d, int32_t R, int32_t position, const int32_t* ids, float* const* self_k,
                               float* const* self_v, int32_t T_max, const float* const* cross_kv, int32_t n_windows, int32_t Tk,
                               const int32_t* row_window, float* logits, void* workspace, size_t workspace_bytes, void* stream);

#ifdef __cplusplus
}
#endif
#endif
```

Baseline: 2158.

## Permute QKV weight rows into per-head interleaved layout for attention

Reorders the rows of the QKV projection weights, biases and folded scales on the host so the QKV GEMM writes Q, K and V for each head next to each other. The attention kernels now take a layout descriptor (head stride plus K and V offsets) instead of assuming planar Q|K|V, and the tower forward passes a flag to select it. When this layout is active, the v3 kernel's auto mapping also picks the by-head block schedule regardless of batch size. The aim is better locality for the per-head K/V loads; the cost is an extra one-time weight permutation and a larger configuration surface.

```diff
diff --git a/hirest_amd/_lib.py b/hirest_amd/_lib.py
--- a/hirest_amd/_lib.py
+++ b/hirest_amd/_lib.py
@@ -14,6 +14,8 @@
 TOWER_NO_LNFOLD = 1
 TOWER_NO_PRUNE = 2
 TOWER_F32_RESIDUAL = 4
+TOWER_QKV_BY_HEAD = 8
+QKV_PLANAR, QKV_BY_HEAD = 0, 1
 GEMM_REVERSE = 1
 GEMM_X3 = 2
 GEMM_X3_T128 = 4
@@ -251,6 +253,8 @@
                                         C.c_float, C.c_int32, C.c_void_p]),
     "hirest_attention_bf16_rows": (C.c_int, [C.c_void_p, C.c_void_p, C.c_int32, C.c_int32, C.c_int32, C.c_int32,
                                              C.c_float, C.c_int32, C.c_int32, C.c_void_p]),
+    "hirest_attention_bf16_layout": (C.c_int, [C.c_void_p, C.c_void_p, C.c_int32, C.c_int32, C.c_int32, C.c_int32,
+                                               C.c_float, C.c_int32, C.c_int32, C.c_int32, C.c_void_p]),
     "hirest_fold_layernorm": (C.c_int, [C.c_void_p, C.c_void_p, C.c_void_p, C.c_void_p, C.c_void_p, C.c_void_p, C.c_void_p, C.c_int32,
                                         C.c_int32, C.c_void_p]),
     "hirest_patchify": (C.c_int, [C.c_void_p, C.c_int32, C.c_int32, C.c_int32, C.c_int32, C.c_void_p, C.c_void_p,
diff --git a/hirest_amd/csrc/attention.hip b/hirest_amd/csrc/attention.hip
--- a/hirest_amd/csrc/attention.hip
+++ b/hirest_amd/csrc/attention.hip
@@ -3,6 +3,8 @@
 #include "profile.h"
 
 namespace {
+
+struct QkvLayout { int hs, ko, vo; };
 
 template <int DH, int DP, int NT>
 struct AttnCfg {
@@ -16,7 +18,7 @@
 
 template <int DH, int DP, int NT>
 __global__ __launch_bounds__(512) void attention_kernel(const bf16_t* __restrict__ qkv, bf16_t* __restrict__ out,
-                                                       int N, int H, float scale_log2e, int causal, int nq) {
+                                                       int N, int H, float scale_log2e, int causal, int nq, QkvLayout lay) {
     using C = AttnCfg<DH, DP, NT>;
     extern __shared__ __attribute__((aligned(16))) char smem[];
     char* Ks = smem;
@@ -25,20 +27,20 @@
     const int b = blockIdx.x / H, h = blockIdx.x - b * H;
     const int D = H * DH;
     const int64_t ld = 3 * (int64_t)D;
-    const bf16_t* base = qkv + (int64_t)b * N * ld + h * DH;
+    const bf16_t* base = qkv + (int64_t)b * N * ld + h * lay.hs;
 
     constexpr int KCH = DP / 8;
     for (int idx = tid; idx < C::NPAD * KCH; idx += 512) {
         const int key = idx / KCH, ch = idx - key * KCH;
         bf16x8 v = {0, 0, 0, 0, 0, 0, 0, 0};
-        if (key < N && ch * 8 < DH) v = *reinterpret_cast<const bf16x8*>(base + (int64_t)key * ld + D + ch * 8);
+        if (key < N && ch * 8 < DH) v = *reinterpret_cast<const bf16x8*>(base + (int64_t)key * ld + lay.ko + ch * 8);
         *reinterpret_cast<bf16x8*>(Ks + key * C::KRS + ch * 16) = v;
     }
     constexpr int VCH = DH / 8;
     for (int idx = tid; idx < C::KP * VCH; idx += 512) {
         const int ch = idx / C::KP, key = idx - ch * C::KP;
         bf16x8 v = {0, 0, 0, 0, 0, 0, 0, 0};
-        if (key < N) v = *reinterpret_cast<const bf16x8*>(base + (int64_t)key * ld + 2 * D + ch * 8);
+        if (key < N) v = *reinterpret_cast<const bf16x8*>(base + (int64_t)key * ld + lay.vo + ch * 8);
 #pragma unroll
         for (int e = 0; e < 8; ++e) *reinterpret_cast<bf16_t*>(Vt + (ch * 8 + e) * C::VRS + key * 2) = v[e];
     }
@@ -127,12 +129,12 @@
 }
 
 template <int DH, int DP, int NT>
-int launch(const bf16_t* qkv, bf16_t* out, int B, int N, int H, float scale, int causal, int nq, hipStream_t s) {
+int launch(const bf16_t* qkv, bf16_t* out, int B, int N, int H, float scale, int causal, int nq, QkvLayout lay, hipStream_t s) {
     using C = AttnCfg<DH, DP, NT>;
     static HirestDevCfg cfg;
     auto kern = attention_kernel<DH, DP, NT>;
     if (int e = hirest_configure(kern, C::LDS_BYTES, cfg)) return e;
-    hipLaunchKernelGGL(kern, dim3(B * H), dim3(512), C::LDS_BYTES, s, qkv, out, N, H, scale * 1.44269504088896340736f, causal, nq);
+    hipLaunchKernelGGL(kern, dim3(B * H), dim3(512), C::LDS_BYTES, s, qkv, out, N, H, scale * 1.44269504088896340736f, causal, nq, lay);
     return hirest_launch_status();
 }
 
@@ -165,7 +167,7 @@
 
 template <int DH, int DP, int NT>
 __global__ __launch_bounds__(512) void attention_kernel_v2(const bf16_t* __restrict__ qkv, bf16_t* __restrict__ out,
-                                                          int N, int H, float scale_log2e, int causal, int nq) {
+                                                          int N, int H, float scale_log2e, int causal, int nq, QkvLayout lay) {
     using C = AttnCfg2<DH, DP, NT>;
     extern __shared__ __attribute__((aligned(16))) char smem[];
     char* Ks = smem;
@@ -175,7 +177,7 @@
     const int b = blockIdx.x / H, h = blockIdx.x - b * H;
     const int D = H * DH;
     const int64_t ld = 3 * (int64_t)D;
-    const bf16_t* base = qkv + (int64_t)b * N * ld + h * DH;
+    const bf16_t* base = qkv + (int64_t)b * N * ld + h * lay.hs;
 
     int nv_mine = 0;
     for (int i = wave; i < C::NK_INSTR; i += 8) {
@@ -184,14 +186,14 @@
         c = (c & ~3) | ((c & 3) ^ ((-(row >> 2)) & 3));
         row = row < N ? row : N - 1;
         c = c * 8 < DH ? c : DH / 8 - 1;
-        glds16(base + (int64_t)row * ld + D + c * 8, Ks + i * 1024);
+        glds16(base + (int64_t)row * ld + lay.ko + c * 8, Ks + i * 1024);
     }
     for (int i = wave; i < C::NV_INSTR; i += 8) {
         const int ci = i * 64 + lane;
         int row = ci / C::CPR, c = ci - row * C::CPR;
         row = row < N ? row : N - 1;
         c = c * 8 < DH ? c : DH / 8 - 1;
-        glds16(base + (int64_t)row * ld + 2 * D + c * 8, Vs + i * 1024);
+        glds16(base + (int64_t)row * ld + lay.vo + c * 8, Vs + i * 1024);
         ++nv_mine;
     }
     wait_vm_le(nv_mine);
@@ -311,7 +313,7 @@
 template <int DH, int DP, int NT, bool FAST, bool DBG, int NW = 9, bool LEAN = false, bool PROD = false>
 __global__ __launch_bounds__((NW + (PROD ? 1 : 0)) * 64) void attention_kernel_v3(const bf16_t* __restrict__ qkv, bf16_t* __restrict__ out,
                                                           int N, int H, float scale_log2e, int causal, int dbg_bits, int nq, int skew,
-                                                          int B, int map, int pace, int stagger) {
+                                                          int B, int map, int pace, int stagger, QkvLayout lay) {
     const int dbg = DBG ? dbg_bits : 0;
     using C = AttnCfg2<DH, DP, NT>;
     extern __shared__ __attribute__((aligned(16))) char smem[];
@@ -329,7 +331,7 @@
     }
     if (nsteps == 0) return;
     if (stagger > 0 && blockIdx.x < 256) sleep_n(((blockIdx.x >> 3) & 15) * stagger);
-    auto sbase = [&](int st) { return qkv + (int64_t)(b0 + st * bstep) * N * ld + (h0 + st * hstep) * DH; };
+    auto sbase = [&](int st) { return qkv + (int64_t)(b0 + st * bstep) * N * ld + (h0 + st * hstep) * lay.hs; };
     const int g = lane >> 4, c16 = lane & 15;
     const int gk = g ^ ((-(c16 >> 2)) & 3);
     const int nqt = (nq + 15) >> 4;
@@ -344,7 +346,7 @@
     constexpr int ROWS_PER_PIECE = NW * 64 / C::CPR;
     auto dma_k = [&](int h, char* dst) -> int {
         int n = 0;
-        const bf16_t* src = sbase(h) + D;
+        const bf16_t* src = sbase(h) + lay.ko;
         for (int i = wave, row = row0; i < C::NK_INSTR; i += NW, row += ROWS_PER_PIECE) {
             int kc = (col0 & ~3) | ((col0 & 3) ^ ((-(row >> 2)) & 3));
             const bool kpad = kc * 8 >= DH;
@@ -360,7 +362,7 @@
     constexpr bool SUM_IN_MFMA = LEAN && DP > DH;
     const bool vpad = SUM_IN_MFMA && vlog * 8 >= DH;
     auto dma_v = [&](int h) {
-        const bf16_t* src = sbase(h) + 2 * D + vc * 8;
+        const bf16_t* src = sbase(h) + lay.vo + vc * 8;
         for (int i = wave, row = row0; i < C::NV_INSTR; i += NW, row += ROWS_PER_PIECE) {
             const int r = row < N ? row : N - 1;
             const void* from = src + (int64_t)r * ld;
@@ -406,7 +408,7 @@
             pvoff[j] = (vl * 8 < DH ? vl : DH / 8 - 1) * 8;
         }
         auto issue_k = [&](int st, char* dst, int pace_units) {
-            const bf16_t* src = sbase(st) + D;
+            const bf16_t* src = sbase(st) + lay.ko;
             for (int it0 = 0; it0 < C::NK_INSTR / PER; ++it0) {
                 const int it = map ? (it0 + h0) % (C::NK_INSTR / PER) : it0;
 #pragma unroll
@@ -420,7 +422,7 @@
             }
         };
         auto issue_v = [&](int st) {
-            const bf16_t* src = sbase(st) + 2 * D;
+            const bf16_t* src = sbase(st) + lay.vo;
             for (int it0 = 0; it0 < C::NV_INSTR / PER; ++it0) {
                 const int it = map ? (it0 + h0) % (C::NV_INSTR / PER) : it0;
 #pragma unroll
@@ -630,42 +632,46 @@
 std::atomic<int> g_attn_map{2};
 std::atomic<int> g_attn_variant{7};
 
+#ifndef HIREST_ATTN_BY_HEAD_MAP1
+#define HIREST_ATTN_BY_HEAD_MAP1 1
+#endif
 template <int DH, int DP, int NT, bool FAST, bool DBG, int NW = 9, bool LEAN = false, bool PROD = false>
-int launch3_impl(const bf16_t* qkv, bf16_t* out, int B, int N, int H, float scale, int causal, int nq, hipStream_t s) {
+int launch3_impl(const bf16_t* qkv, bf16_t* out, int B, int N, int H, float scale, int causal, int nq, QkvLayout lay, hipStream_t s) {
     using C = AttnCfg2<DH, DP, NT>;
     constexpr int LDS = (2 * C::NPAD + C::KP) * C::RS;
     static_assert(LDS <= 163840, "K x2 + V must fit the CU's LDS");
     static HirestDevCfg cfg;
     auto kern = attention_kernel_v3<DH, DP, NT, FAST, DBG, NW, LEAN, PROD>;
     if (int e = hirest_configure(kern, LDS, cfg)) return e;
-    const bool by_head = (g_attn_map == 1 || (g_attn_map == 2 && B < 256)) && H <= 32 && 32 % H == 0 && B >= 8 * (32 / H) * 4;
+    const bool auto_by_head = B < 256 || (HIREST_ATTN_BY_HEAD_MAP1 && lay.hs != DH);
+    const bool by_head = (g_attn_map == 1 || (g_attn_map == 2 && auto_by_head)) && H <= 32 && 32 % H == 0 && B >= 8 * (32 / H) * 4;
     const int grid = by_head ? 256 : B;
     hipLaunchKernelGGL(kern, dim3(grid), dim3((NW + (PROD ? 1 : 0)) * 64), LDS, s, qkv, out, N, H, scale * 1.44269504088896340736f, causal, g_attn_dbg, nq,
-                       g_attn_skew, B, by_head ? 1 : 0, g_attn_pace, g_attn_stagger);
+                       g_attn_skew, B, by_head ? 1 : 0, g_attn_pace, g_attn_stagger, lay);
     return hirest_launch_status();
 }
 
 template <int DH, int DP, int NT, bool FAST>
-int launch3(const bf16_t* qkv, bf16_t* out, int B, int N, int H, float scale, int causal, int nq, hipStream_t s) {
-    if (g_attn_dbg && FAST && g_attn_variant == 6) return launch3_impl<DH, DP, NT, FAST, true, 9, true, true>(qkv, out, B, N, H, scale, causal, nq, s);
-    if (g_attn_variant == 6) return launch3_impl<DH, DP, NT, FAST, false, 9, true, true>(qkv, out, B, N, H, scale, causal, nq, s);
-    if (g_attn_dbg && FAST && g_attn_variant == 7) return launch3_impl<DH, DP, NT, FAST, true, 9, false, true>(qkv, out, B, N, H, scale, causal, nq, s);
-    if (g_attn_variant == 7) return launch3_impl<DH, DP, NT, FAST, false, 9, false, true>(qkv, out, B, N, H, scale, causal, nq, s);
-    if (g_attn_dbg && FAST && g_attn_variant == 5) return launch3_impl<DH, DP, NT, FAST, true, 9, true>(qkv, out, B, N, H, scale, causal, nq, s);
-    if (g_attn_dbg && FAST) return launch3_impl<DH, DP, NT, FAST, true>(qkv, out, B, N, H, scale, causal, nq, s);
-    if (g_attn_variant == 4) return launch3_impl<DH, DP, NT, FAST, false, 12>(qkv, out, B, N, H, scale, causal, nq, s);
-    if (g_attn_variant == 5) return launch3_impl<DH, DP, NT, FAST, false, 9, true>(qkv, out, B, N, H, scale, causal, nq, s);
-    return launch3_impl<DH, DP, NT, FAST, false>(qkv, out, B, N, H, scale, causal, nq, s);
+int launch3(const bf16_t* qkv, bf16_t* out, int B, int N, int H, float scale, int causal, int nq, QkvLayout lay, hipStream_t s) {
+    if (g_attn_dbg && FAST && g_attn_variant == 6) return launch3_impl<DH, DP, NT, FAST, true, 9, true, true>(qkv, out, B, N, H, scale, causal, nq, lay, s);
+    if (g_attn_variant == 6) return launch3_impl<DH, DP, NT, FAST, false, 9, true, true>(qkv, out, B, N, H, scale, causal, nq, lay, s);
+    if (g_attn_dbg && FAST && g_attn_variant == 7) return launch3_impl<DH, DP, NT, FAST, true, 9, false, true>(qkv, out, B, N, H, scale, causal, nq, lay, s);
+    if (g_attn_variant == 7) return launch3_impl<DH, DP, NT, FAST, false, 9, false, true>(qkv, out, B, N, H, scale, causal, nq, lay, s);
+    if (g_attn_dbg && FAST && g_attn_variant == 5) return launch3_impl<DH, DP, NT, FAST, true, 9, true>(qkv, out, B, N, H, scale, causal, nq, lay, s);
+    if (g_attn_dbg && FAST) return launch3_impl<DH, DP, NT, FAST, true>(qkv, out, B, N, H, scale, causal, nq, lay, s);
+    if (g_attn_variant == 4) return launch3_impl<DH, DP, NT, FAST, false, 12>(qkv, out, B, N, H, scale, causal, nq, lay, s);
+    if (g_attn_variant == 5) return launch3_impl<DH, DP, NT, FAST, false, 9, true>(qkv, out, B, N, H, scale, causal, nq, lay, s);
+    return launch3_impl<DH, DP, NT, FAST, false>(qkv, out, B, N, H, scale, causal, nq, lay, s);
 }
 
 
 template <int DH, int DP, int NT>
-int launch2(const bf16_t* qkv, bf16_t* out, int B, int N, int H, float scale, int causal, int nq, hipStream_t s) {
+int launch2(const bf16_t* qkv, bf16_t* out, int B, int N, int H, float scale, int causal, int nq, QkvLayout lay, hipStream_t s) {
     using C = AttnCfg2<DH, DP, NT>;
     static HirestDevCfg cfg;
     auto kern = attention_kernel_v2<DH, DP, NT>;
     if (int e = hirest_configure(kern, C::LDS_BYTES, cfg)) return e;
-    hipLaunchKernelGGL(kern, dim3(B * H), dim3(512), C::LDS_BYTES, s, qkv, out, N, H, scale * 1.44269504088896340736f, causal, nq);
+    hipLaunchKernelGGL(kern, dim3(B * H), dim3(512), C::LDS_BYTES, s, qkv, out, N, H, scale * 1.44269504088896340736f, causal, nq, lay);
     return hirest_launch_status();
 }
 
@@ -710,12 +716,19 @@
 
 extern "C" int hirest_attention_bf16(const hirest_bf16* qkv, hirest_bf16* out, int32_t B, int32_t N, int32_t H,
                                      int32_t dh, float scale, int32_t causal, void* stream) {
-    return hirest_attention_bf16_rows(qkv, out, B, N, H, dh, scale, causal, N, stream);
+    return hirest_attention_bf16_layout(qkv, out, B, N, H, dh, scale, causal, N, HIREST_QKV_PLANAR, stream);
 }
 
 extern "C" int hirest_attention_bf16_rows(const hirest_bf16* qkv, hirest_bf16* out, int32_t B, int32_t N, int32_t H,
                                           int32_t dh, float scale, int32_t causal, int32_t q_rows, void* stream) {
+    return hirest_attention_bf16_layout(qkv, out, B, N, H, dh, scale, causal, q_rows, HIREST_QKV_PLANAR, stream);
+}
+
+extern "C" int hirest_attention_bf16_layout(const hirest_bf16* qkv, hirest_bf16* out, int32_t B, int32_t N, int32_t H,
+                                            int32_t dh, float scale, int32_t causal, int32_t q_rows, int32_t layout, void* stream) {
     if (!qkv || !out || B <= 0 || N <= 0 || H <= 0 || q_rows <= 0 || q_rows > N) return HIREST_E_BADARG;
+    if (layout != HIREST_QKV_PLANAR && layout != HIREST_QKV_BY_HEAD) return HIREST_E_BADARG;
+    const QkvLayout lay = layout == HIREST_QKV_BY_HEAD ? QkvLayout{3 * dh, dh, 2 * dh} : QkvLayout{dh, H * dh, 2 * H * dh};
     const int nq = q_rows;
     hipStream_t s = reinterpret_cast<hipStream_t>(stream);
     const bf16_t* q = reinterpret_cast<const bf16_t*>(qkv);
@@ -723,27 +736,27 @@
     HirestProfScope prof(HIREST_PROF_ATTENTION, causal, (int64_t)B * H, N, dh, s);
     if (g_attn_variant >= 3 && N > 80 && N <= 272 && B >= 64) {
         const bool fast = !causal && N > 256;
-        if (dh == 88) return fast ? launch3<88, 96, 17, true>(q, o, B, N, H, scale, causal, nq, s)
-                                  : launch3<88, 96, 17, false>(q, o, B, N, H, scale, causal, nq, s);
-        if (dh == 64) return fast ? launch3<64, 64, 17, true>(q, o, B, N, H, scale, causal, nq, s)
-                                  : launch3<64, 64, 17, false>(q, o, B, N, H, scale, causal, nq, s);
+        if (dh == 88) return fast ? launch3<88, 96, 17, true>(q, o, B, N, H, scale, causal, nq, lay, s)
+                                  : launch3<88, 96, 17, false>(q, o, B, N, H, scale, causal, nq, lay, s);
+        if (dh == 64) return fast ? launch3<64, 64, 17, true>(q, o, B, N, H, scale, causal, nq, lay, s)
+                                  : launch3<64, 64, 17, false>(q, o, B, N, H, scale, causal, nq, lay, s);
     }
     if (g_attn_variant >= 2) {
         if (dh == 88) {
-            if (N <= 80) return launch2<88, 96, 5>(q, o, B, N, H, scale, causal, nq, s);
-            if (N <= 272) return launch2<88, 96, 17>(q, o, B, N, H, scale, causal, nq, s);
+            if (N <= 80) return launch2<88, 96, 5>(q, o, B, N, H, scale, causal, nq, lay, s);
+            if (N <= 272) return launch2<88, 96, 17>(q, o, B, N, H, scale, causal, nq, lay, s);
         } else if (dh == 64) {
-            if (N <= 80) return launch2<64, 64, 5>(q, o, B, N, H, scale, causal, nq, s);
-            if (N <= 272) return launch2<64, 64, 17>(q, o, B, N, H, scale, causal, nq, s);
+            if (N <= 80) return launch2<64, 64, 5>(q, o, B, N, H, scale, causal, nq, lay, s);
+            if (N <= 272) return launch2<64, 64, 17>(q, o, B, N, H, scale, causal, nq, lay, s);
         }
         return HIREST_E_SHAPE;
     }
     if (dh == 88) {
-        if (N <= 80) return launch<88, 96, 5>(q, o, B, N, H, scale, causal, nq, s);
-        if (N <= 272) return launch<88, 96, 17>(q, o, B, N, H, scale, causal, nq, s);
+        if (N <= 80) return launch<88, 96, 5>(q, o, B, N, H, scale, causal, nq, lay, s);
+        if (N <= 272) return launch<88, 96, 17>(q, o, B, N, H, scale, causal, nq, lay, s);
     } else if (dh == 64) {
-        if (N <= 80) return launch<64, 64, 5>(q, o, B, N, H, scale, causal, nq, s);
-        if (N <= 272) return launch<64, 64, 17>(q, o, B, N, H, scale, causal, nq, s);
+        if (N <= 80) return launch<64, 64, 5>(q, o, B, N, H, scale, causal, nq, lay, s);
+        if (N <= 272) return launch<64, 64, 17>(q, o, B, N, H, scale, causal, nq, lay, s);
     }
     return HIREST_E_SHAPE;
 }
diff --git a/hirest_amd/csrc/tower.hip b/hirest_amd/csrc/tower.hip
--- a/hirest_amd/csrc/tower.hip
+++ b/hirest_amd/csrc/tower.hip
@@ -57,11 +57,11 @@
 }
 
 int run_block(const hirest_block_weights& w, float* x, hirest_bf16* h, hirest_bf16* big, int B, int T, int D, int heads,
-              int dh, int Dm, float eps, int act, int causal, void* stream) {
+              int dh, int Dm, float eps, int act, int causal, void* stream, int qkv_layout = HIREST_QKV_PLANAR) {
     const int M = B * T;
     CHECK(hirest_layernorm(x, D, nullptr, w.ln1_g, w.ln1_b, eps, h, D, 0, M, D, stream));
     CHECK(gemm(h, D, w.qkv_w, D, w.qkv_b, big, 3 * D, M, 3 * D, D, HIREST_EPI_BIAS_BF16, stream));
-    CHECK(hirest_attention_bf16(big, h, B, T, heads, dh, 1.0f / sqrtf((float)dh), causal, stream));
+    CHECK(hirest_attention_bf16_layout(big, h, B, T, heads, dh, 1.0f / sqrtf((float)dh), causal, T, qkv_layout, stream));
     CHECK(gemm(h, D, w.proj_w, D, w.proj_b, x, D, M, D, D, HIREST_EPI_BIAS_RESID_F32, stream));
     CHECK(hirest_layernorm(x, D, nullptr, w.ln2_g, w.ln2_b, eps, h, D, 0, M, D, stream));
     CHECK(gemm(h, D, w.fc1_w, D, w.fc1_b, big, Dm, M, Dm, D,
@@ -72,13 +72,13 @@
 
 int run_block_lnfold(const hirest_block_weights& w, float* x, hirest_bf16* h, hirest_bf16* big, hirest_bf16* xb, float* part,
                      float* stats, float* guard, int B, int T, int D, int heads, int dh, int Dm, float eps, void* stream,
-                     hirest_bf16* xl = nullptr) {
+                     hirest_bf16* xl = nullptr, int qkv_layout = HIREST_QKV_PLANAR) {
     const int M = B * T, G = (D + 63) / 64;
     void* res = xl ? static_cast<void*>(xl) : static_cast<void*>(x);
     const int epi_res = xl ? HIREST_EPI_BIAS_RESID2_LNSTATS : HIREST_EPI_BIAS_RESID_LNSTATS_F32;
     CHECK(gemm(xb, D, w.qkv_wf, D, w.qkv_bf, big, 3 * D, M, 3 * D, D, HIREST_EPI_LNFOLD_BF16, stream, nullptr, 0, stats,
                const_cast<float*>(w.qkv_s)));
-    CHECK(hirest_attention_bf16(big, h, B, T, heads, dh, 1.0f / sqrtf((float)dh), 0, stream));
+    CHECK(hirest_attention_bf16_layout(big, h, B, T, heads, dh, 1.0f / sqrtf((float)dh), 0, T, qkv_layout, stream));
     CHECK(gemm(h, D, w.proj_w, D, w.proj_b, res, D, M, D, D, epi_res, stream, nullptr, 0, xb, part));
     CHECK(hirest_ln_stats_finalize(part, G, stats, eps, M, D, guard, stream));
     CHECK(gemm(xb, D, w.fc1_wf, D, w.fc1_bf, big, Dm, M, Dm, D, HIREST_EPI_LNFOLD_GELU_BF16, stream, nullptr, 0, stats,
@@ -90,12 +90,13 @@
 
 int run_block_lnfold_cls(const hirest_block_weights& w, float* x, hirest_bf16* h, hirest_bf16* big, hirest_bf16* xb, float* part,
                          float* stats, float* guard, int B, int T, int D, int heads, int dh, int Dm, float eps, void* stream,
-                         hirest_bf16* xl = nullptr, hirest_bf16* cls_hi = nullptr, hirest_bf16* cls_lo = nullptr) {
+                         hirest_bf16* xl = nullptr, hirest_bf16* cls_hi = nullptr, hirest_bf16* cls_lo = nullptr,
+                         int qkv_layout = HIREST_QKV_PLANAR) {
     const int M = B * T, G = (D + 63) / 64;
     const int64_t TD = (int64_t)T * D;
     CHECK(gemm(xb, D, w.qkv_wf, D, w.qkv_bf, big, 3 * D, M, 3 * D, D, HIREST_EPI_LNFOLD_BF16, stream, nullptr, 0, stats,
                const_cast<float*>(w.qkv_s)));
-    CHECK(hirest_attention_bf16_rows(big, h, B, T, heads, dh, 1.0f / sqrtf((float)dh), 0, 1, stream));
+    CHECK(hirest_attention_bf16_layout(big, h, B, T, heads, dh, 1.0f / sqrtf((float)dh), 0, 1, qkv_layout, stream));
     if (xl) {
         hipStream_t s = reinterpret_cast<hipStream_t>(stream);
         if (hipMemcpy2DAsync(cls_hi, (size_t)D * 2, xb, (size_t)TD * 2, (size_t)D * 2, B, hipMemcpyDeviceToDevice, s) != hipSuccess ||
@@ -143,6 +144,7 @@
     if (t->width != t->heads * t->head_dim || t->image_size % t->patch != 0) return HIREST_E_SHAPE;
     const int G = t->image_size / t->patch, P = G * G, T = P + 1, D = t->width;
     const bool can_fold = vision_lnfold(t, B), lnfold = can_fold && !(flags & HIREST_TOWER_NO_LNFOLD);
+    const int qkv_layout = (flags & HIREST_TOWER_QKV_BY_HEAD) ? HIREST_QKV_BY_HEAD : HIREST_QKV_PLANAR;
     const Regions r = plan((int64_t)B * T, D, vision_wide(t), B, can_fold);
     if (workspace_bytes < r.total) return HIREST_E_WORKSPACE;
     char* ws = reinterpret_cast<char*>(workspace);
@@ -171,10 +173,10 @@
         for (int l = 0; l < t->layers; ++l) {
             if (prune && l == t->layers - 1) {
                 CHECK(run_block_lnfold_cls(t->blocks[l], x, h, big, xb, part, stats, guard, B, T, D, t->heads, t->head_dim, t->mlp_dim,
-                                           t->ln_eps, stream, xl, cls_hi, cls_lo));
+                                           t->ln_eps, stream, xl, cls_hi, cls_lo, qkv_layout));
             } else {
                 CHECK(run_block_lnfold(t->blocks[l], x, h, big, xb, part, stats, guard, B, T, D, t->heads, t->head_dim, t->mlp_dim,
-                                       t->ln_eps, stream, xl));
+                                       t->ln_eps, stream, xl, qkv_layout));
             }
         }
         if (xl && !prune) CHECK(hirest_combine_hi_lo_f32(xb, xl, D, x, D, B * T, D, stream));
@@ -184,7 +186,7 @@
         }
     } else {
         for (int l = 0; l < t->layers; ++l)
-            CHECK(run_block(t->blocks[l], x, h, big, B, T, D, t->heads, t->head_dim, t->mlp_dim, t->ln_eps, t->act, 0, stream));
+            CHECK(run_block(t->blocks[l], x, h, big, B, T, D, t->heads, t->head_dim, t->mlp_dim, t->ln_eps, t->act, 0, stream, qkv_layout));
     }
     if (t->out_all_tokens) {
         CHECK(hirest_layernorm(x, D, nullptr, t->norm_g, t->norm_b, t->ln_eps, h, D, 0, B * T, D, stream));
diff --git a/hirest_amd/eva_clip.py b/hirest_amd/eva_clip.py
--- a/hirest_amd/eva_clip.py
+++ b/hirest_amd/eva_clip.py
@@ -142,7 +142,8 @@
             else:
                 scalars = self._scalars()
             desc = _struct(desc_cls, blocks=blocks, **scalars, **self._pointers(self, rows, kind, device, keep))
-            cache[kind] = {"device": device, "desc": desc, "blocks": blocks, "keep": keep}
+            cache[kind] = {"device": device, "desc": desc, "blocks": blocks, "keep": keep,
+                           "qkv_by_head": kind == "bf16" and self._qkv_row_order(device) is not None}
         return cache[kind]
 
     def _pointers(self, owner, rows, kind, device, keep) -> dict:
@@ -172,8 +173,16 @@
                     t = self._f32(p.detach().float().t() if form == "wT" else p)
                     t = ops.split2(t) if form == "split" else t if form == "f32" else cast(t)
             done[field] = t
+        perm = self._qkv_row_order(device) if kind == "bf16" and "qkv_w" in done else None
+        if perm is not None:
+            for field in ("qkv_w", "qkv_b", "qkv_wf", "qkv_bf", "qkv_s"):
+                if done.get(field) is not None:
+                    done[field] = done[field].index_select(0, perm).contiguous()
         keep.extend(t for t in done.values() if t is not None)
         return {f: None if t is None else t.data_ptr() for f, t in done.items()}
+
+    def _qkv_row_order(self, device):
+        return None
 
     def _fold(self, w32, bias, norm, device):
         N, K = w32.shape
@@ -253,9 +262,16 @@
         self.fold_fallbacks = 0
         self.prune_last_block = True
         self.f32_residual = os.environ.get("HIREST_F32_RESIDUAL", "0") == "1"
+        self.qkv_by_head = os.environ.get("HIREST_QKV_BY_HEAD", "1") != "0"
 
     def _blocks(self):
         return self.blocks
+
+    def _qkv_row_order(self, device):
+        if not self.qkv_by_head:
+            return None
+        dh = self.width // self.heads
+        return torch.arange(3 * self.width, device=device).view(3, self.heads, dh).permute(1, 0, 2).reshape(-1)
 
     def _scalars(self):
         P = self.patch_size
@@ -294,7 +310,11 @@
         image = image.contiguous()
         if self.precision in self._EXACT:
             return self._forward_exact(image)
-        desc = C.byref(self._prepared_for("bf16", image.device)["desc"])
+        prep = self._prepared_for("bf16", image.device)
+        if prep["qkv_by_head"] != bool(self.qkv_by_head):
+            del self._prepared["bf16"]
+            prep = self._prepared_for("bf16", image.device)
+        desc = C.byref(prep["desc"])
         lib = _lib.load()
         B = image.shape[0]
         out = torch.empty((B, self.embed_dim), dtype=torch.float32, device=image.device)
@@ -303,7 +323,8 @@
         step = self._call_size(B, self.max_frames_per_call, True)
         code = ops._IN_DTYPES[image.dtype]
         self.last_fold_ratio = 0.0
-        flags = (0 if self.prune_last_block else _lib.TOWER_NO_PRUNE) | (_lib.TOWER_F32_RESIDUAL if self.f32_residual else 0)
+        flags = (0 if self.prune_last_block else _lib.TOWER_NO_PRUNE) | (_lib.TOWER_F32_RESIDUAL if self.f32_residual else 0) | \
+                (_lib.TOWER_QKV_BY_HEAD if prep["qkv_by_head"] else 0)
         goff = lib.hirest_vision_guard_offset(desc, step) if self.fold_guard_ratio is not None else _NO_GUARD
         guards = torch.zeros(-(-B // step), dtype=torch.float32, device=image.device) if goff != _NO_GUARD else None
 
diff --git a/include/hirest_hip.h b/include/hirest_hip.h
--- a/include/hirest_hip.h
+++ b/include/hirest_hip.h
@@ -68,6 +68,10 @@
 int hirest_attention_bf16_rows(const hirest_bf16* qkv, hirest_bf16* out,
                                int32_t B, int32_t N, int32_t H, int32_t dh,
                                float scale, int32_t causal, int32_t q_rows, void* stream);
+enum { HIREST_QKV_PLANAR = 0, HIREST_QKV_BY_HEAD = 1 };
+int hirest_attention_bf16_layout(const hirest_bf16* qkv, hirest_bf16* out,
+                                 int32_t B, int32_t N, int32_t H, int32_t dh,
+                                 float scale, int32_t causal, int32_t q_rows, int32_t layout, void* stream);
 int hirest_attention_select_kernel(int32_t which);
 int hirest_attention_set_mapping(int32_t by_head);
 int hirest_attention_set_pace(int32_t units);
@@ -152,7 +156,8 @@
 size_t hirest_vision_workspace_bytes(const hirest_vision_tower* t, int32_t B);
 enum { HIREST_TOWER_NO_LNFOLD = 1,
        HIREST_TOWER_NO_PRUNE = 2,
-       HIREST_TOWER_F32_RESIDUAL = 4 };
+       HIREST_TOWER_F32_RESIDUAL = 4,
+       HIREST_TOWER_QKV_BY_HEAD = 8 };
 int hirest_vision_forward(const hirest_vision_tower* t, const void* frames, int32_t in_dtype,
                           int32_t B, float* out, void* workspace, size_t workspace_bytes,
                           int32_t flags, void* stream);
```

New measurement: 2162 (median of 6 runs). Within noise of the previous version (+0.2%).
